# wischmcj/pyQSM

Measured on AMD Instinct MI355X. Metric: Mpoints/s DBSCAN (1M-pt synthetic forest, eps=0.1, min_neighbors=10), higher is better.
Workload: dtype f64; 1 GPU; 1000000-point synthetic tree cloud (configs[1]), DBSCAN eps=0.1 min_neighbors=10, 20 clusters; replicas at N>1; points_per_gpu=1000000, parallelism=replicas x1

## Files before the change

include/pyqsm_hip.h:

```cpp
#ifndef PYQSM_HIP_H
#define PYQSM_HIP_H

#include <stddef.h>
#include <stdint.h>

#ifdef __cplusplus
extern "C" {
#endif

#define PYQSM_OK 0
#define PYQSM_EINVAL (-1)
#define PYQSM_EHIP (-2)
#define PYQSM_ENODEV (-3)
#define PYQSM_ERANGE (-4)
#define PYQSM_ENOMEM (-5)
#define PYQSM_ENOCONV (-6)

#define PYQSM_MISS_PRIM 0xFFFFFFFFu


int pyqsm_device_count(void);
int pyqsm_init(int device);
int pyqsm_shutdown(void);
const char* pyqsm_last_error(void);
const char* pyqsm_version(void);
int pyqsm_sync(int device);
void* pyqsm_stream(int device);

int pyqsm_dev_malloc(int device, size_t bytes, void** out);
int pyqsm_dev_free(int device, void* p);
int pyqsm_h2d(int device, void* dst_dev, const void* src_host, size_t bytes);
int pyqsm_d2h(int device, void* dst_host, const void* src_dev, size_t bytes);
void pyqsm_free(void* p);
void* pyqsm_host_alloc(size_t bytes);

int pyqsm_prof_enable(int device, int on);
int pyqsm_prof_reset(int device);
int pyqsm_prof_get(int device, const char* name, double* total_ms, int64_t* launches);

int pyqsm_cast_rays(const float* verts, int64_t V, const int32_t* tris, int64_t T,
                    const float* rays, int64_t R,
                    float* t_hit, uint32_t* prim_id, float* uv, int32_t device);

int pyqsm_expand_tris_dev(const float* verts_dev, int64_t V, const int32_t* tris_dev,
                          int64_t T, float* tri12_dev, int32_t device);
int pyqsm_cast_rays_dev(const float* tri12_dev, int64_t T, const float* rays_dev, int64_t R,
                        float* t_hit_dev, uint32_t* prim_id_dev, float* uv_dev,
                        int32_t device);

int pyqsm_list_intersections(const float* verts, int64_t V, const int32_t* tris, int64_t T,
                             const float* rays, int64_t R, int32_t* counts,
                             uint32_t* ray_ids, uint32_t* prim_ids, float* t, float* uv,
                             int64_t hits_cap, int64_t* n_hits, int32_t device);

int pyqsm_point_mesh_distance(const float* verts, int64_t V, const int32_t* tris, int64_t T,
                              const float* qry, int64_t Q, float* dist, uint32_t* prim,
                              int32_t device);

int pyqsm_cast_rays_multi(const float* verts, int64_t V, const int32_t* tris, int64_t T,
                          const float* rays, int64_t R,
                          float* t_hit, uint32_t* prim_id, float* uv, int32_t n_devices);

int pyqsm_shard_bounds(int64_t n, int32_t world, int32_t rank, int64_t* begin, int64_t* end);

#define PYQSM_COMM_ID_BYTES 128
int pyqsm_comm_unique_id(uint8_t* id);
int pyqsm_comm_init_rank(const uint8_t* id, int32_t world, int32_t rank, int32_t device);
int pyqsm_comm_finalize(void);
int pyqsm_comm_info(int32_t* world, int32_t* rank, int32_t* device);
int pyqsm_comm_broadcast_dev(void* buf_dev, int64_t bytes, int32_t root);
int pyqsm_comm_all_gather_dev(const void* send_dev, void* recv_dev, int64_t bytes_per_rank);
int pyqsm_comm_all_reduce_max(double* value);

int pyqsm_dbscan(const double* xyz, int64_t n, double eps, int32_t min_pts,
                 int64_t* labels, uint8_t* is_core, int32_t device);
int pyqsm_dbscan_dev(const double* xyz_dev, int64_t n, double eps, int32_t min_pts,
                     int64_t* labels_dev, uint8_t* is_core_dev, int64_t* n_clusters,
                     int32_t device);
int pyqsm_dbscan_ex(const double* xyz, int64_t n, double eps, int32_t min_pts,
                    int32_t radius_inclusive, int64_t* labels, uint8_t* is_core, int32_t device);
int pyqsm_dbscan_dev_ex(const double* xyz_dev, int64_t n, double eps, int32_t min_pts,
                        int32_t radius_inclusive, int64_t* labels_dev, uint8_t* is_core_dev,
                        int64_t* n_clusters, int32_t device);
int pyqsm_octant_directory(const double* xyz, int64_t n, double eps, int32_t* dims_out,
                           int32_t* begin_out, int64_t cap, int32_t device);

int pyqsm_knn(const double* xyz, int64_t n, int32_t k, int32_t exclude_self,
              int32_t* idx, double* d2, int32_t device);
int pyqsm_knn_dev(const double* xyz_dev, int64_t n, int32_t k, int32_t exclude_self,
                  int32_t* idx_dev, double* d2_dev, int32_t device);

int pyqsm_ransac(const double* pts, int64_t n, const int64_t* triples, int64_t H,
                 int32_t shape, double thresh, double center[3], double axis[3],
                 double* radius, int64_t* inliers, int64_t* n_inliers, int64_t* best,
                 int32_t device);
int pyqsm_ransac_models(const double* pts, int64_t n, const int64_t* triples, int64_t H,
                        double* models, int32_t device);
int pyqsm_ransac_count(const double* pts, int64_t n, const double* models, int64_t H,
                       int32_t shape, double thresh, int32_t* counts, int32_t device);
int pyqsm_ransac_batch(const double* pts, int64_t n, const int64_t* seg_start, int64_t n_seg,
                       const int64_t* triples, int64_t H, int32_t shape, double thresh,
                       double* centers, double* axes, double* radii, int64_t* inliers,
                       int64_t* n_inliers, int64_t* best, int32_t device);

int pyqsm_plane_models(const double* pts, int64_t n, const int64_t* samples, int64_t H, int32_t m,
                       const double* axis, double cos_limit, double* planes, int32_t device);
int pyqsm_plane_count(const double* pts, int64_t n, const double* planes, int64_t H, double thresh,
                      int32_t* counts, int32_t device);
int pyqsm_segment_plane(const double* pts, int64_t n, const int64_t* samples, int64_t H, int32_t m,
                        double thresh, double probability, const double* axis, double cos_limit,
                        double plane_fit[4], double plane_hyp[4], int64_t* inliers, int64_t* n_inliers,
                        int64_t* best, int64_t* used, int32_t device);
int pyqsm_segment_planes(const double* pts, int64_t n, const uint64_t* draws, int64_t P, int64_t H,
                         int32_t m, double thresh, double probability, int64_t min_inliers,
                         const double* axis, double cos_limit, int32_t* labels, double* planes_fit,
                         double* planes_hyp, int64_t* counts, int64_t* best, int64_t* used,
                         int64_t* n_planes, int32_t device);

int pyqsm_lbc_solve(const int32_t* indptr, const int32_t* indices, const double* vals,
                    int64_t n, const double* wl, const double* wh, const double* pts,
                    double rtol, int32_t max_it, double* out, int32_t* iters,
                    double* resid, int32_t device);
int pyqsm_spmv3(const int32_t* indptr, const int32_t* indices, const double* vals,
                int64_t n, const double* x, double* y, int32_t device);
int pyqsm_clamp(double* pts, int64_t n, const double lo[3], const double hi[3],
                int32_t device);

int pyqsm_ball_query(const double* xyz, int64_t n, const double center[3], double radius,
                     int64_t* out_idx, int64_t* count, int32_t device);
int pyqsm_radius_mark(const double* src, int64_t n, const double* qry, int64_t m, double radius,
                      int32_t k_cap, uint8_t* mark, int32_t* counts, int32_t device);
int pyqsm_radius_knn(const double* src, int64_t n, const double* qry, int64_t m, double radius,
                     int32_t k, int64_t* idx, double* dist, int32_t device);
int pyqsm_radius_reduce(const double* src, int64_t n, const double* qry, int64_t m, double radius, int32_t k,
                        const double* values, int32_t F, int32_t reducer, int64_t empty_row, double* out,
                        int32_t* counts, int32_t device);
int pyqsm_radius_label(const double* src, int64_t n, const double* qry, int64_t m,
                       const int32_t* qry_label, double radius, int32_t k_cap, int32_t* label,
                       int32_t* counts, int32_t device);
int pyqsm_grow_clusters(const double* src, int64_t n, const int32_t* owner_in, const double* seed_xyz,
                        const int32_t* seed_label, int64_t m, int32_t n_clusters, double radius,
                        int32_t k_cap, int32_t cycles, int32_t min_new, int32_t* owner_out,
                        int32_t* cycle_out, int32_t* finished, int64_t* stats, int32_t device);

#define PYQSM_ADJ_SAME_CLOUD 1
#define PYQSM_ADJ_WITNESS 2
#define PYQSM_ADJ_NO_CACHE 4
int pyqsm_cluster_adjacency(const double* src, const int32_t* src_label, int64_t n, int32_t n_src_labels,
                            const double* tgt, const int32_t* tgt_label, int64_t m, int32_t n_tgt_labels,
                            double threshold, int32_t flags, int64_t capacity, int32_t* a, int32_t* b,
                            double* min_d2, int64_t* pairs, int64_t* src_idx, int64_t* tgt_idx, int64_t* count,
                            int64_t* stats, int32_t device);

#define PYQSM_ALPHA_BOUNDARY 1
#define PYQSM_ALPHA_DEFAULT_MAX_TESTS 4000000000000LL
int pyqsm_alpha_area(const int32_t* ij, int64_t n, const int64_t* seg_start, int64_t n_seg, uint64_t a2,
                     int64_t max_tests, int32_t flags, int64_t* twice_area, int64_t* n_live, int64_t* n_boundary,
                     int64_t** edges, int64_t* stats, int32_t device);

#define PYQSM_MESH_PAIRS 1
#define PYQSM_MESH_TILE_ROWS 256
#define PYQSM_MESH_DEFAULT_MAX_TESTS 16000000000000LL
int pyqsm_mesh_topology(const int32_t* tris, int64_t n_tris, int64_t n_verts, const double* verts, int32_t** edges,
                        int32_t** edge_count, uint8_t** edge_flags, int32_t* tri_cluster, int64_t** cluster_n,
                        double** cluster_area, uint8_t* vertex_flags, int64_t* summary, int32_t device);
int pyqsm_mesh_self_intersections(const int32_t* ijk, int64_t n_verts, const int32_t* tris, int64_t n_tris,
                                  int32_t flags, int64_t max_tests, int64_t* n_pairs, int32_t** pairs,
                                  uint8_t* tri_hit, int64_t* stats, int32_t device);

#define PYQSM_RECON_MAX_RHO2 4194304ULL
#define PYQSM_RECON_CHUNK 1024
#define PYQSM_RECON_SLICE 16
#define PYQSM_RECON_DEFAULT_MAX_TESTS 1000000000000LL
int pyqsm_ball_pivot(const int32_t* ijk, const int16_t* normals, int64_t n, const uint64_t* rho2, int32_t n_levels,
                     int64_t max_tests, int64_t* n_tris, int32_t** tris, int64_t* stats, int32_t device);

int pyqsm_fps(const double* xyz, int64_t n, int64_t num_samples, int64_t start_index,
              int32_t* out_idx, int32_t device);

int pyqsm_pc_laplacian(const double* xyz, int64_t n, int32_t k, double moll,
                       int64_t* nnz, int32_t** indptr, int32_t** indices, double** vals,
                       double* mass, int32_t device);
int pyqsm_pc_laplacian_seg(const double* xyz, int64_t n, const int64_t* seg_start, int64_t n_seg,
                           int32_t k, double moll, int64_t* nnz, int32_t** indptr,
                           int32_t** indices, double** vals, double* mass, int32_t device);

int pyqsm_extract_skeleton(const double* xyz, int64_t n, const int64_t* seg_start, int64_t n_seg,
                           int32_t k, double moll, int32_t max_iter, double termination_ratio,
                           double contraction_factor, double attraction_factor,
                           double max_contraction, double max_attraction, const double* lo,
                           const double* hi, double rtol, int32_t solver_max_it, double* out_pts,
                           double* total_shift, double* steps, int32_t* n_steps,
                           int32_t* solve_iters, double* solve_resid, uint8_t* solve_ok,
                           int32_t* n_solves, int32_t device);

int pyqsm_extreme_points(const double* xyz, int64_t n, const double* dirs, int32_t n_dirs,
                         int64_t* idx, int32_t device);
int pyqsm_outside_halfspaces(const double* xyz, int64_t n, const double* eq, int32_t n_planes,
                             double margin, int64_t* idx, int64_t* count, int32_t device);

int pyqsm_mean_f64(const double* v, int64_t n, double* out);

int pyqsm_voxel_down_sample(const double* xyz, int64_t n, const double* colors, double voxel_size,
                            int64_t* m, double** out_xyz, double** out_colors, int64_t* inverse,
                            int64_t* offsets, int64_t* members, int32_t device);
int pyqsm_stat_outlier(const double* xyz, int64_t n, int32_t nb_neighbors, double std_ratio,
                       int64_t* keep, int64_t* n_keep, double* avg, double* stats, int32_t device);
int pyqsm_clean_cloud(const double* xyz, int64_t n, double voxel_size, double neighbors, double ratio,
                      int32_t iters, int64_t* m, double** out_xyz, int32_t device);

int pyqsm_estimate_normals(const double* xyz, int64_t n, double radius, int32_t max_nn,
                           const double* prev_normals, double* normals, int32_t device);
int pyqsm_orient_normals_tangent_plane(const double* xyz, int64_t n, const double* normals, int32_t k,
                                       double* oriented, int32_t* rounds, int32_t device);
int pyqsm_stem_cloud(const double* xyz, int64_t n, const double* prev_normals, double crop_offset,
                     double radius, int32_t max_nn, int32_t orient_k, double angle_cutoff,
                     int64_t* keep, double* normals, int64_t* m, int32_t device);

#define PYQSM_KMEANS_MAX_K 8
#define PYQSM_KMEANS_MAX_Q 4
#define PYQSM_SILHOUETTE_MAX_K 65536
int pyqsm_kmeans(const double* xyz, int64_t m, int32_t k, int32_t iters, const double* init,
                 double* centroids, int32_t* labels, int32_t device);
int pyqsm_silhouette(const double* xyz, int64_t m, const int32_t* labels, int32_t k, double* score,
                     int32_t* n_present, double* samples, int32_t device);
int pyqsm_kmeans_select(const double* xyz, int64_t m, int32_t k0, int32_t nk, int32_t iters,
                        const double* init, int32_t* labels, double* scores, int32_t* present,
                        int32_t device);
int pyqsm_kmeans_select_dev(const double* xyz_dev, int64_t m, int32_t k0, int32_t nk, int32_t iters,
                            const double* init, int32_t* labels, double* scores, int32_t* present,
                            int32_t device);
int pyqsm_ball_excl_dev(const double* xyz_dev, int64_t n, const uint8_t* found_dev, const double center[3],
                        double radius, int64_t* idx_dev, double* out_xyz_dev, int64_t* count,
                        int32_t device);
int pyqsm_mark_found_dev(uint8_t* found_dev, int64_t n, const int64_t* idx, int64_t cnt, int32_t device);

int pyqsm_geometric_features(const double* xyz, int64_t n, double radius, int32_t max_k, int32_t metric,
                             const int32_t* feature_ids, int32_t n_features, double* out, int32_t* counts,
// ... 54 lines not shown
```

pyqsm_amd/_lib.py:

```python
from __future__ import annotations

import ctypes
import os

_HERE = os.path.dirname(os.path.abspath(__file__))
LIB_PATH = os.path.join(_HERE, "libpyqsm_hip.so")

i64, i32, u32, dbl = ctypes.c_int64, ctypes.c_int32, ctypes.c_uint32, ctypes.c_double
vp = ctypes.c_void_p

SIGNATURES = {
    "pyqsm_device_count": (ctypes.c_int, []),
    "pyqsm_init": (ctypes.c_int, [ctypes.c_int]),
    "pyqsm_shutdown": (ctypes.c_int, []),
    "pyqsm_last_error": (ctypes.c_char_p, []),
    "pyqsm_version": (ctypes.c_char_p, []),
    "pyqsm_sync": (ctypes.c_int, [ctypes.c_int]),
    "pyqsm_stream": (vp, [ctypes.c_int]),
    "pyqsm_dev_malloc": (ctypes.c_int, [ctypes.c_int, ctypes.c_size_t, ctypes.POINTER(vp)]),
    "pyqsm_dev_free": (ctypes.c_int, [ctypes.c_int, vp]),
    "pyqsm_h2d": (ctypes.c_int, [ctypes.c_int, vp, vp, ctypes.c_size_t]),
    "pyqsm_d2h": (ctypes.c_int, [ctypes.c_int, vp, vp, ctypes.c_size_t]),
    "pyqsm_free": (None, [vp]),
    "pyqsm_host_alloc": (vp, [ctypes.c_size_t]),
    "pyqsm_prof_enable": (ctypes.c_int, [ctypes.c_int, ctypes.c_int]),
    "pyqsm_prof_reset": (ctypes.c_int, [ctypes.c_int]),
    "pyqsm_prof_get": (ctypes.c_int, [ctypes.c_int, ctypes.c_char_p, ctypes.POINTER(dbl),
                                      ctypes.POINTER(i64)]),
    "pyqsm_cast_rays": (ctypes.c_int, [vp, i64, vp, i64, vp, i64, vp, vp, vp, i32]),
    "pyqsm_expand_tris_dev": (ctypes.c_int, [vp, i64, vp, i64, vp, i32]),
    "pyqsm_cast_rays_dev": (ctypes.c_int, [vp, i64, vp, i64, vp, vp, vp, i32]),
    "pyqsm_list_intersections": (ctypes.c_int, [vp, i64, vp, i64, vp, i64, vp, vp, vp, vp, vp,
                                                i64, ctypes.POINTER(i64), i32]),
    "pyqsm_point_mesh_distance": (ctypes.c_int, [vp, i64, vp, i64, vp, i64, vp, vp, i32]),
    "pyqsm_cast_rays_multi": (ctypes.c_int, [vp, i64, vp, i64, vp, i64, vp, vp, vp, i32]),
    "pyqsm_shard_bounds": (ctypes.c_int, [i64, i32, i32, ctypes.POINTER(i64), ctypes.POINTER(i64)]),
    "pyqsm_comm_unique_id": (ctypes.c_int, [vp]),
    "pyqsm_comm_init_rank": (ctypes.c_int, [vp, i32, i32, i32]),
    "pyqsm_comm_finalize": (ctypes.c_int, []),
    "pyqsm_comm_info": (ctypes.c_int, [ctypes.POINTER(i32), ctypes.POINTER(i32),
                                       ctypes.POINTER(i32)]),
    "pyqsm_comm_broadcast_dev": (ctypes.c_int, [vp, i64, i32]),
    "pyqsm_comm_all_gather_dev": (ctypes.c_int, [vp, vp, i64]),
    "pyqsm_comm_all_reduce_max": (ctypes.c_int, [ctypes.POINTER(dbl)]),
    "pyqsm_dbscan": (ctypes.c_int, [vp, i64, dbl, i32, vp, vp, i32]),
    "pyqsm_dbscan_dev": (ctypes.c_int, [vp, i64, dbl, i32, vp, vp, ctypes.POINTER(i64), i32]),
    "pyqsm_dbscan_ex": (ctypes.c_int, [vp, i64, dbl, i32, i32, vp, vp, i32]),
    "pyqsm_dbscan_dev_ex": (ctypes.c_int, [vp, i64, dbl, i32, i32, vp, vp, ctypes.POINTER(i64), i32]),
    "pyqsm_octant_directory": (ctypes.c_int, [vp, i64, dbl, vp, vp, i64, i32]),
    "pyqsm_knn": (ctypes.c_int, [vp, i64, i32, i32, vp, vp, i32]),
    "pyqsm_knn_dev": (ctypes.c_int, [vp, i64, i32, i32, vp, vp, i32]),
    "pyqsm_ransac": (ctypes.c_int, [vp, i64, vp, i64, i32, dbl, vp, vp, ctypes.POINTER(dbl), vp,
                                    ctypes.POINTER(i64), ctypes.POINTER(i64), i32]),
    "pyqsm_ransac_models": (ctypes.c_int, [vp, i64, vp, i64, vp, i32]),
    "pyqsm_ransac_count": (ctypes.c_int, [vp, i64, vp, i64, i32, dbl, vp, i32]),
    "pyqsm_ransac_batch": (ctypes.c_int, [vp, i64, vp, i64, vp, i64, i32, dbl, vp, vp, vp, vp, vp, vp, i32]),
    "pyqsm_plane_models": (ctypes.c_int, [vp, i64, vp, i64, i32, vp, dbl, vp, i32]),
    "pyqsm_plane_count": (ctypes.c_int, [vp, i64, vp, i64, dbl, vp, i32]),
    "pyqsm_segment_plane": (ctypes.c_int, [vp, i64, vp, i64, i32, dbl, dbl, vp, dbl, vp, vp, vp,
                                           ctypes.POINTER(i64), ctypes.POINTER(i64), ctypes.POINTER(i64), i32]),
    "pyqsm_segment_planes": (ctypes.c_int, [vp, i64, vp, i64, i64, i32, dbl, dbl, i64, vp, dbl, vp, vp, vp, vp,
                                            vp, vp, ctypes.POINTER(i64), i32]),
    "pyqsm_lbc_solve": (ctypes.c_int, [vp, vp, vp, i64, vp, vp, vp, dbl, i32, vp,
                                       ctypes.POINTER(i32), vp, i32]),
    "pyqsm_spmv3": (ctypes.c_int, [vp, vp, vp, i64, vp, vp, i32]),
    "pyqsm_clamp": (ctypes.c_int, [vp, i64, vp, vp, i32]),
    "pyqsm_ball_query": (ctypes.c_int, [vp, i64, vp, dbl, vp, ctypes.POINTER(i64), i32]),
    "pyqsm_radius_mark": (ctypes.c_int, [vp, i64, vp, i64, dbl, i32, vp, vp, i32]),
    "pyqsm_radius_label": (ctypes.c_int, [vp, i64, vp, i64, vp, dbl, i32, vp, vp, i32]),
    "pyqsm_grow_clusters": (ctypes.c_int, [vp, i64, vp, vp, vp, i64, i32, dbl, i32, i32, i32, vp, vp, vp, vp,
                                           i32]),
    "pyqsm_radius_knn": (ctypes.c_int, [vp, i64, vp, i64, dbl, i32, vp, vp, i32]),
    "pyqsm_cluster_adjacency": (ctypes.c_int, [vp, vp, i64, i32, vp, vp, i64, i32, dbl, i32, i64, vp, vp, vp, vp,
                                               vp, vp, ctypes.POINTER(i64), vp, i32]),
    "pyqsm_alpha_area": (ctypes.c_int, [vp, i64, vp, i64, ctypes.c_uint64, i64, i32, vp, vp, vp,
                                        ctypes.POINTER(vp), vp, i32]),
    "pyqsm_pdist_select": (ctypes.c_int, [vp, i64, i32, vp, i64, vp, i32, i64, vp, vp, vp, vp, i32]),
    "pyqsm_mesh_topology": (ctypes.c_int, [vp, i64, i64, vp, ctypes.POINTER(vp), ctypes.POINTER(vp),
                                           ctypes.POINTER(vp), vp, ctypes.POINTER(vp), ctypes.POINTER(vp), vp, vp,
                                           i32]),
    "pyqsm_mesh_self_intersections": (ctypes.c_int, [vp, i64, vp, i64, i32, i64, ctypes.POINTER(i64),
                                                     ctypes.POINTER(vp), vp, vp, i32]),
    "pyqsm_ball_pivot": (ctypes.c_int, [vp, vp, i64, vp, i32, i64, ctypes.POINTER(i64), ctypes.POINTER(vp), vp,
                                        i32]),
    "pyqsm_fps": (ctypes.c_int, [vp, i64, i64, i64, vp, i32]),
    "pyqsm_pc_laplacian": (ctypes.c_int, [vp, i64, i32, dbl, ctypes.POINTER(i64),
                                          ctypes.POINTER(vp), ctypes.POINTER(vp),
                                          ctypes.POINTER(vp), vp, i32]),
    "pyqsm_extract_skeleton": (ctypes.c_int, [vp, i64, vp, i64, i32, dbl, i32, dbl, dbl, dbl, dbl, dbl, vp, vp,
                                              dbl, i32, vp, vp, vp, vp, vp, vp, vp, ctypes.POINTER(i32), i32]),
    "pyqsm_pc_laplacian_seg": (ctypes.c_int, [vp, i64, vp, i64, i32, dbl, ctypes.POINTER(i64),
                                              ctypes.POINTER(vp), ctypes.POINTER(vp),
                                              ctypes.POINTER(vp), vp, i32]),
    "pyqsm_voxel_down_sample": (ctypes.c_int, [vp, i64, vp, dbl, ctypes.POINTER(i64), ctypes.POINTER(vp),
                                               ctypes.POINTER(vp), vp, vp, vp, i32]),
    "pyqsm_stat_outlier": (ctypes.c_int, [vp, i64, i32, dbl, vp, ctypes.POINTER(i64), vp, vp, i32]),
    "pyqsm_clean_cloud": (ctypes.c_int, [vp, i64, dbl, dbl, dbl, i32, ctypes.POINTER(i64),
                                         ctypes.POINTER(vp), i32]),
    "pyqsm_estimate_normals": (ctypes.c_int, [vp, i64, dbl, i32, vp, vp, i32]),
    "pyqsm_orient_normals_tangent_plane": (ctypes.c_int, [vp, i64, vp, i32, vp, ctypes.POINTER(i32), i32]),
    "pyqsm_stem_cloud": (ctypes.c_int, [vp, i64, vp, dbl, dbl, i32, i32, dbl, vp, vp, ctypes.POINTER(i64),
                                        i32]),
    "pyqsm_mean_f64": (ctypes.c_int, [vp, i64, ctypes.POINTER(dbl)]),
    "pyqsm_extreme_points": (ctypes.c_int, [vp, i64, vp, i32, vp, i32]),
    "pyqsm_outside_halfspaces": (ctypes.c_int, [vp, i64, vp, i32, dbl, vp, ctypes.POINTER(i64), i32]),
    "pyqsm_kmeans": (ctypes.c_int, [vp, i64, i32, i32, vp, vp, vp, i32]),
    "pyqsm_silhouette": (ctypes.c_int, [vp, i64, vp, i32, ctypes.POINTER(dbl), ctypes.POINTER(i32), vp, i32]),
    "pyqsm_kmeans_select": (ctypes.c_int, [vp, i64, i32, i32, i32, vp, vp, vp, vp, i32]),
    "pyqsm_kmeans_select_dev": (ctypes.c_int, [vp, i64, i32, i32, i32, vp, vp, vp, vp, i32]),
    "pyqsm_ball_excl_dev": (ctypes.c_int, [vp, i64, vp, vp, dbl, vp, vp, ctypes.POINTER(i64), i32]),
    "pyqsm_mark_found_dev": (ctypes.c_int, [vp, i64, vp, i64, i32]),
    "pyqsm_geometric_features": (ctypes.c_int, [vp, i64, dbl, i32, i32, vp, i32, vp, vp, i32]),
    "pyqsm_smooth_values": (ctypes.c_int, [vp, i64, vp, i64, vp, i32, i32, i32, vp, vp, i32]),
    "pyqsm_forest_create": (ctypes.c_int, [vp, vp, vp, vp, vp, vp, vp, i32, i32, i32, i32, ctypes.POINTER(vp)]),
    "pyqsm_forest_free": (ctypes.c_int, [vp]),
    "pyqsm_forest_info": (ctypes.c_int, [vp, vp]),
    "pyqsm_forest_stage": (ctypes.c_int, [vp, i32]),
    "pyqsm_forest_predict": (ctypes.c_int, [vp, vp, i64, vp, vp, vp]),
    "pyqsm_radius_reduce": (ctypes.c_int, [vp, i64, vp, i64, dbl, i32, vp, i32, i32, i64, vp, vp, i32]),
    "pyqsm_voxel_grid_create": (ctypes.c_int, [vp, i64, vp, dbl, i32, ctypes.POINTER(vp)]),
    "pyqsm_voxel_grid_free": (ctypes.c_int, [vp]),
    "pyqsm_voxel_grid_info": (ctypes.c_int, [vp, vp, ctypes.POINTER(dbl), vp, ctypes.POINTER(i64),
                                             ctypes.POINTER(i64)]),
    "pyqsm_voxel_grid_voxels": (ctypes.c_int, [vp, vp, vp]),
    "pyqsm_voxel_grid_query": (ctypes.c_int, [vp, vp, i64, i32, vp, vp, vp, ctypes.POINTER(i64)]),
    "pyqsm_voxel_grid_query_dev": (ctypes.c_int, [vp, vp, i64, i32, vp, vp, vp, ctypes.POINTER(i64)]),
    "pyqsm_skeletal_forest": (ctypes.c_int, [vp, i64, i32, vp, vp, ctypes.POINTER(i64), ctypes.POINTER(i32), i32]),
    "pyqsm_skeletal_forest_dev": (ctypes.c_int, [vp, i64, i32, vp, vp, ctypes.POINTER(i64), ctypes.POINTER(i32),
                                                 i32]),
    "pyqsm_collapse_chains": (ctypes.c_int, [vp, i64, i64, vp, vp, vp, vp, vp, i32]),
    "pyqsm_collapse_chains_dev": (ctypes.c_int, [vp, i64, i64, vp, vp, vp, vp, vp, i32]),
    "pyqsm_chain_radii": (ctypes.c_int, [vp, i64, vp, i64, vp, vp, i64, vp, i32]),
    "pyqsm_cylinder_surfaces": (ctypes.c_int, [vp, i64, vp, vp, ctypes.POINTER(vp), ctypes.POINTER(i64), i32]),
}

_lib = None


class PyQSMHipError(RuntimeError):

    def __init__(self, code: int, message: str):
        super().__init__(f"libpyqsm_hip error {code}: {message}")
        self.code = code


def load() -> ctypes.CDLL:
    global _lib
    if _lib is not None:
        return _lib
    if not os.path.exists(LIB_PATH):
        raise ImportError(
            f"{LIB_PATH} not found: the HIP library has not been built and there is no CPU "
            "fallback. Build it with `make -C pyqsm_amd/csrc`.")
    lib = ctypes.CDLL(LIB_PATH)
    for name, (res, args) in SIGNATURES.items():
        fn = getattr(lib, name)
        fn.restype = res
        fn.argtypes = args
    _lib = lib
    return lib


def check(code: int) -> None:
    if code != 0:
        msg = load().pyqsm_last_error()
        raise PyQSMHipError(code, msg.decode("utf-8", "replace") if msg else "")


def device_count() -> int:
    return int(load().pyqsm_device_count())


def logical_device_count() -> int:
    fake = os.environ.get("PYQSM_MULTI_FAKE_RANKS", "")
    return int(fake) if fake.isdigit() and int(fake) > 0 else device_count()


def physical_device(logical: int) -> int:
    fake = os.environ.get("PYQSM_MULTI_FAKE_RANKS", "")
    if fake.isdigit() and int(fake) > 0:
        return int(logical) % max(1, device_count())
    return int(logical)


def require_gpu(device: int = 0) -> None:
    check(load().pyqsm_init(int(device)))
```

pyqsm_amd/csrc/dbscan.hip:

```cpp
#include "grid.hpp"

#include <atomic>
#include <cfloat>
#include <chrono>
#include <cmath>
#include <optional>
#include <type_traits>
#include <vector>

namespace pyqsm {

static constexpr int kNoRoot = 0x7FFFFFFF;

__device__ __forceinline__ double sqdist(double ax, double ay, double az, double bx, double by,
                                         double bz) {
  double t0 = ax - bx, t1 = ay - by, t2 = az - bz;
  double d = t0 * t0;
  d = d + t1 * t1;
  d = d + t2 * t2;
  return d;
}


#define FOR_STENCIL(c, st, dir, q, body)                           \
  for (int dz__ = -1; dz__ <= 1; ++dz__)                           \
    for (int dy__ = -1; dy__ <= 1; ++dy__) {                       \
      const int row__ = (c) + dy__ * (st).nx + dz__ * (st).nxy;    \
      const int qb__ = (dir).begin(row__ - 1), qe__ = (dir).begin(row__ + 2); \
      for (int q = qb__; q < qe__; ++q) {                          \
        body                                                       \
      }                                                            \
    }

struct TileLds {
  double x[4][64], y[4][64], z[4][64];
};
struct TileLdsF32 {
  alignas(16) float x[4][64], y[4][64], z[4][64];
};
typedef float float2v __attribute__((ext_vector_type(2)));

struct CoreBand {
  float lo, hi;
  bool usable() const { return lo > 0x1p-100f && std::isfinite(hi); }
};
static CoreBand core_band(double r2) {
  const double a = r2 * (1.0 - 0x1p-20), b = r2 * (1.0 + 0x1p-20);
  CoreBand t{0.0f, INFINITY};
  if (!(a > 0.0) || !(b <= double(FLT_MAX))) return t;
  t.lo = float(a);
  if (double(t.lo) > a) t.lo = nextafterf(t.lo, -INFINITY);
  t.hi = float(b);
  if (double(t.hi) < b) t.hi = nextafterf(t.hi, INFINITY);
  return t;
}

static constexpr int kStragglers = 6;
static constexpr int kMaxChunks = 3;
static constexpr int kRestSegs = 64;
__device__ constexpr int kRunOrder[9] = {4, 3, 5, 1, 7, 0, 2, 6, 8};

__device__ __forceinline__ void stencil_bounds(int c, Stencil st, const CellDir& dir, int (&qb)[9], int (&qe)[9]) {
  int cells[18], q[18];
#pragma unroll
  for (int r = 0; r < 9; ++r) {
    const int row = c + (kRunOrder[r] % 3 - 1) * st.nx + (kRunOrder[r] / 3 - 1) * st.nxy;
    cells[2 * r] = row - 1;
    cells[2 * r + 1] = row + 2;
  }
  dir.begins(cells, q);
#pragma unroll
  for (int r = 0; r < 9; ++r) {
    qb[r] = q[2 * r];
    qe[r] = q[2 * r + 1];
  }
}

template <class CO, bool F32>
__global__ __launch_bounds__(256) void k_core_tiled(int n, const GridPlan* __restrict__ plan,
                                                    const DirWord* __restrict__ dwords,
                                                    const int32_t* __restrict__ dslots,
                                                    const int32_t* __restrict__ cell_of, CO co, double r2,
                                                    float r2_lo, float r2_hi ,
                                                    int min_pts, uint8_t* __restrict__ core,
                                                    int32_t* __restrict__ rest,
                                                    int32_t* __restrict__ rest_cnt , int seg_cap,
                                                    int* __restrict__ parent, int* __restrict__ min_orig,
                                                    uint32_t* __restrict__ bits ,
                                                    int32_t* __restrict__ seam , int seam_cap,
                                                    int max_chunks,
                                                    unsigned long long* __restrict__ tests ,
    unsigned long long* __restrict__ st ) {
  __shared__ TileLds L;
  __shared__ TileLdsF32 LF;
  stamped(st, [&] {
  const CellDir dir{dwords, dslots};
  const int lane = threadIdx.x & 63, w = __builtin_amdgcn_readfirstlane(threadIdx.x >> 6);
  const int p0 = (blockIdx.x * 4 + w) * 64;
  if (p0 >= n || !plan->ok) return;
  const Stencil st = plan_stencil(plan);
  const int ncell = plan->ncell;
  const int p = p0 + lane;
  const bool live = p < n;
  double x = 0.0, y = 0.0, z = 0.0;
  float fx = 0.0f, fy = 0.0f, fz = 0.0f;
  if constexpr (F32) {
    if (live) {
      const float4 v = co.p[p];
      fx = v.x, fy = v.y, fz = v.z;
    }
  } else {
    if (live) co.get(p, x, y, z);
  }
  const Tile t = wave_tile(p0, n, st, ncell, dir, cell_of);
  int cnt = 0;
  int cnt_hi = 0;
  bool deferred = false;
  int chunks = 0;
  int staged = 0;
  int band = 0;
  const auto hand_on = [&](unsigned long long und) {
    if (und != 0) {
      int slot = 0;
      const int lead = __ffsll(und) - 1;
      const int seg = blockIdx.x % kRestSegs;
      if (lane == lead) slot = atomicAdd(rest_cnt + seg, __popcll(und));
      slot = __shfl(slot, lead, 64);
      const bool mine = (und >> lane) & 1ull;
      if constexpr (F32) band += __popcll(__ballot(mine && cnt_hi > cnt));
      if (mine) {
        rest[size_t(seg) * seg_cap + slot + __popcll(und & ((1ull << lane) - 1ull))] = p;
        cnt = -1;
      }
    }
    deferred = true;
  };
  if (t.total > kTileMax) {
    if constexpr (F32) x = double(fx), y = double(fy), z = double(fz);
    const int mycell = live ? cell_of[p] : -1;
    unsigned long long todo = __ballot(live);
    while (todo) {
      const int lead = __ffsll(todo) - 1;
      const int c = __builtin_amdgcn_readlane(mycell, lead);
      const bool mine = mycell == c;
      todo &= ~__ballot(mine);
      int rqb[9], rqe[9];
      stencil_bounds(c, st, dir, rqb, rqe);
#pragma unroll
      for (int r = 0; r < 9; ++r) {
        const int qb = __builtin_amdgcn_readfirstlane(rqb[r]);
        const int qe = __builtin_amdgcn_readfirstlane(rqe[r]);
        for (int base = qb; base < qe; base += 64) {
          const int q = base + lane;
          const int m = qe - base < 64 ? qe - base : 64;
          if (q < qe) co.get(q, L.x[w][lane], L.y[w][lane], L.z[w][lane]);
          __builtin_amdgcn_wave_barrier();
          staged += m;
          if (mine)
            for (int j = 0; j < m; ++j)
              cnt += sqdist(x, y, z, L.x[w][j], L.y[w][j], L.z[w][j]) <= r2;
          __builtin_amdgcn_wave_barrier();
        }
      }
    }
  } else {
    const float2v X = {fx, fx}, Y = {fy, fy}, Z = {fz, fz};
#pragma unroll
    for (int ri = 0; ri < 9; ++ri) {
      const int r = kRunOrder[ri];
      for (int base = t.qb[r]; base < t.qe[r] && !deferred; base += 64) {
        const int q = base + lane;
        const int m = t.qe[r] - base < 64 ? t.qe[r] - base : 64;
        if constexpr (F32) {
          float4 v = make_float4(INFINITY, 0.0f, 0.0f, 0.0f);
          if (q < t.qe[r]) v = co.p[q];
          LF.x[w][lane] = v.x, LF.y[w][lane] = v.y, LF.z[w][lane] = v.z;
          __builtin_amdgcn_wave_barrier();
#pragma unroll 4
          for (int j = 0; j < m; j += 2) {
            const float2v dx = X - *reinterpret_cast<const float2v*>(&LF.x[w][j]);
            const float2v dy = Y - *reinterpret_cast<const float2v*>(&LF.y[w][j]);
            const float2v dz = Z - *reinterpret_cast<const float2v*>(&LF.z[w][j]);
            float2v d = dx * dx;
            d = __builtin_elementwise_fma(dy, dy, d);
            d = __builtin_elementwise_fma(dz, dz, d);
            cnt += d.x <= r2_lo;
            cnt += d.y <= r2_lo;
            cnt_hi += d.x <= r2_hi;
            cnt_hi += d.y <= r2_hi;
          }
        } else {
          if (q < t.qe[r]) co.get(q, L.x[w][lane], L.y[w][lane], L.z[w][lane]);
          __builtin_amdgcn_wave_barrier();
#pragma unroll 4
          for (int j = 0; j < m; ++j)
            cnt += sqdist(x, y, z, L.x[w][j], L.y[w][j], L.z[w][j]) <= r2;
        }
        staged += m;
        __builtin_amdgcn_wave_barrier();
        const unsigned long long und = __ballot(live && cnt < min_pts);
        ++chunks;
        if ((__popcll(und) <= kStragglers || chunks >= max_chunks) &&
            !(ri == 8 && base + 64 >= t.qe[r])) {
          hand_on(und);
          break;
        }
      }
    }
    if constexpr (F32) {
      if (!deferred) hand_on(__ballot(live && cnt < min_pts && cnt_hi >= min_pts));
    }
  }
  if (live && cnt >= 0) {
    core[p] = cnt >= min_pts;
    co.mark_core(p, cnt >= min_pts);
  }
  if (live) {
    parent[p] = p;
    min_orig[p] = 0x7F7F7F7F;
    if (p <= n / 32) bits[p] = 0u;
    if (p == 0) bits[n / 32 + 1] = 0u;
    for (int i = p; i < seam_cap; i += n) seam[i] = 0;
  }
  if (tests && lane == 0) {
    atomicAdd(tests + (blockIdx.x & 255), static_cast<unsigned long long>(staged));
    if (band) atomicAdd(tests + 256 + (blockIdx.x & 255), static_cast<unsigned long long>(band));
  }
  });
}

struct Runs9 {
  int qb[9];
  int pre[10];
  __device__ __forceinline__ int at(int g) const {
    int q = qb[0] + g;
#pragma unroll
    for (int r = 1; r < 9; ++r) q = g >= pre[r] ? qb[r] + (g - pre[r]) : q;
    return q;
  }
};
static constexpr int kRunBatch = 3;
__device__ __forceinline__ int lane_bound(bool act, int c, int j, Stencil st, const CellDir& dir) {
  const int r = int((0x862071534ull >> (4 * (j >> 1))) & 15ull);
  const int cell = c + (r % 3 - 1) * st.nx + (r / 3 - 1) * st.nxy + ((j & 1) ? 2 : -1);
  int b = 0;
  if (act) {
    const DirWord w = dir.words[cell >> 5];
    b = dir.slots[CellDir::slot_of(w, cell)];
  }
  return b;
}
__device__ __forceinline__ Runs9 runs_of_lanes(int bound, int k) {
  Runs9 t;
  t.pre[0] = 0;
#pragma unroll
  for (int r = 0; r < 9; ++r) {
    t.qb[r] = __builtin_amdgcn_readlane(bound, 18 * k + 2 * r);
    t.pre[r + 1] = t.pre[r] + (__builtin_amdgcn_readlane(bound, 18 * k + 2 * r + 1) - t.qb[r]);
  }
  return t;
}

template <class CO>
__global__ __launch_bounds__(256) void k_core_rest(const int32_t* __restrict__ rest,
                                                   const int32_t* __restrict__ rest_cnt ,
                                                   int seg_cap, const GridPlan* __restrict__ plan,
                                                   const DirWord* __restrict__ dwords,
                                                   const int32_t* __restrict__ dslots,
                                                   const int32_t* __restrict__ cell_of, CO co, double r2,
                                                   int min_pts, uint8_t* __restrict__ core,
    unsigned long long* __restrict__ st ) {
  stamped(st, [&] {
  const CellDir dir{dwords, dslots};
  if (!plan->ok) return;
  const Stencil st = plan_stencil(plan);
  const int lane = threadIdx.x & 63;
  const int mine = rest_cnt[lane];
  int incl = mine;
#pragma unroll
  for (int off = 1; off < 64; off <<= 1) {
    const int v = __shfl_up(incl, off, 64);
    if (lane >= off) incl += v;
  }
  const int m = __shfl(incl, 63, 64);
  const int grp = lane / 18, j = lane % 18;
  for (int i0 = (blockIdx.x * 4 + (threadIdx.x >> 6)) * kRunBatch; i0 < m; i0 += gridDim.x * 4 * kRunBatch) {
    int p = 0;
#pragma unroll
    for (int k = 0; k < kRunBatch; ++k) {
      if (i0 + k >= m) break;
      const int seg = __popcll(__ballot(incl <= i0 + k));
      const int before = __shfl(incl - mine, seg, 64);
      const int pk = rest[size_t(seg) * seg_cap + (i0 + k - before)];
      p = grp == k ? pk : p;
    }
    const bool act = grp < kRunBatch && i0 + grp < m;
    double x = 0.0, y = 0.0, z = 0.0;
    int c = 0;
    if (act) {
      co.get(p, x, y, z);
      c = cell_of[p];
    }
    const int bound = lane_bound(act, c, j, st, dir);
#pragma unroll
    for (int k = 0; k < kRunBatch; ++k) {
      if (i0 + k >= m) break;
      const Runs9 t = runs_of_lanes(bound, k);
      const int pk = __builtin_amdgcn_readlane(p, 18 * k);
      const double xk = __shfl(x, 18 * k, 64), yk = __shfl(y, 18 * k, 64), zk = __shfl(z, 18 * k, 64);
      int cnt = 0;
      for (int g0 = 0; g0 < t.pre[9] && cnt < min_pts; g0 += 64) {
        const int g = g0 + lane;
        const bool hit = g < t.pre[9] && co.d2(t.at(g), xk, yk, zk) <= r2;
        cnt += __popcll(__ballot(hit));
      }
      if (lane == 0) {
        core[pk] = cnt >= min_pts;
        co.mark_core(pk, cnt >= min_pts);
      }
    }
  }
  });
}


__device__ __forceinline__ int ld_parent(const int* parent, int i) {
  return __hip_atomic_load(parent + i, __ATOMIC_RELAXED, __HIP_MEMORY_SCOPE_AGENT);
}
__device__ __forceinline__ void st_parent(int* parent, int i, int v) {
  __hip_atomic_store(parent + i, v, __ATOMIC_RELAXED, __HIP_MEMORY_SCOPE_AGENT);
}

__device__ __forceinline__ unsigned link_prio(int x) { return unsigned(x) * 0x9E3779B1u; }

__device__ __forceinline__ int find_root(int* parent, int x) {
  int cur = ld_parent(parent, x);
  if (cur != x) {
    int prev = x, next;
    while (cur != (next = ld_parent(parent, cur))) {
      st_parent(parent, prev, next);
      prev = cur;
      cur = next;
    }
  }
  return cur;
}

__device__ __forceinline__ void unite(int* parent, int a, int b) {
  int ra = find_root(parent, a), rb = find_root(parent, b);
  while (ra != rb) {
    if (link_prio(ra) < link_prio(rb)) {
      int t = ra;
      ra = rb;
      rb = t;
    }
    const int old = atomicCAS(parent + ra, ra, rb);
    if (old == ra) break;
    ra = find_root(parent, old);
    rb = find_root(parent, rb);
  }
}


__global__ __launch_bounds__(1024) void k_sub_rep(int n, const int32_t* __restrict__ sub_of,
                                                 const uint8_t* __restrict__ core,
                                                 const int32_t* __restrict__ order,
                                                 int* __restrict__ parent,
                                                 const int32_t* __restrict__ cell_of,
// ... 627 lines not shown
        k = (static_cast<unsigned long long>(min_orig[r]) << 32) | static_cast<uint32_t>(r);
      }
      key[i] = k;
    }
    __syncthreads();
    for (int k = 2; k <= P; k <<= 1)
      for (int j = k >> 1; j > 0; j >>= 1) {
        for (int i = t; i < P; i += kNumberThreads) {
          const int l = i ^ j;
          if (l > i) {
            const unsigned long long a = key[i], b = key[l];
            if ((a > b) == ((i & k) == 0)) {
              key[i] = b;
              key[l] = a;
            }
          }
        }
        __syncthreads();
      }
    for (int i = t; i < R; i += kNumberThreads) min_orig[static_cast<uint32_t>(key[i])] = i;
    return;
  }
  for (int i = blockIdx.x * kNumberThreads + t; i < R; i += gridDim.x * kNumberThreads) {
    const int v = min_orig[roots[i]];
    __hip_atomic_fetch_or(bits + (v >> 5), 1u << (v & 31), __ATOMIC_RELAXED, __HIP_MEMORY_SCOPE_AGENT);
  }
  __shared__ int last;
  __threadfence();
  __syncthreads();
  if (t == 0) last = atomicAdd(done, 1) == int(gridDim.x) - 1;
  __syncthreads();
  if (!last) return;
  __threadfence();
  __shared__ int wsum[kNumberThreads / 64];
  const int lane = t & 63, wv = t >> 6;
  const int nw = n / 32 + 1;
  int carry = 0;
  for (int w0 = 0; w0 < nw; w0 += 16 * kNumberThreads) {
    const int i0 = w0 + 16 * t;
    int cnt[16], sum = 0;
#pragma unroll
    for (int k = 0; k < 16; ++k) {
      cnt[k] = i0 + k < nw ? __popc(__hip_atomic_load(bits + i0 + k, __ATOMIC_RELAXED, __HIP_MEMORY_SCOPE_AGENT)) : 0;
      sum += cnt[k];
    }
    int incl = sum;
#pragma unroll
    for (int off = 1; off < 64; off <<= 1) {
      const int o = __shfl_up(incl, off, 64);
      if (lane >= off) incl += o;
    }
    if (lane == 63) wsum[wv] = incl;
    __syncthreads();
    int before = carry, total = 0;
    for (int k = 0; k < kNumberThreads / 64; ++k) {
      before += k < wv ? wsum[k] : 0;
      total += wsum[k];
    }
    int run = before + incl - sum;
#pragma unroll
    for (int k = 0; k < 16; ++k)
      if (i0 + k < nw) {
        wpre[i0 + k] = run;
        run += cnt[k];
      }
    carry += total;
    __syncthreads();
  }
  });
}

__device__ __forceinline__ int cluster_number(int v, int n_roots, const uint32_t* __restrict__ bits,
                                              const int32_t* __restrict__ wpre) {
  if (n_roots <= kRankCap) return v;
  return wpre[v >> 5] + __popc(bits[v >> 5] & ((1u << (v & 31)) - 1u));
}

static constexpr int kLabelThreads = 256;
template <class CO>
__global__ __launch_bounds__(kLabelThreads) void k_labels(int n, const int32_t* __restrict__ rest,
                                                          const int32_t* __restrict__ rest_cnt,
                                                          const GridPlan* __restrict__ plan,
                                                          const DirWord* __restrict__ dwords,
                                                          const int32_t* __restrict__ dslots,
                                                          const int32_t* __restrict__ cell_of, CO co, double r2,
                                                          const uint8_t* __restrict__ core,
                                                          const int* __restrict__ parent,
                                                          const int* __restrict__ min_orig,
                                                          const int32_t* __restrict__ roots_cnt,
                                                          const uint32_t* __restrict__ bits,
                                                          const int32_t* __restrict__ wpre,
                                                          const int32_t* __restrict__ order,
                                                          int64_t* __restrict__ labels,
                                                          uint8_t* __restrict__ is_core,
    unsigned long long* __restrict__ st ) {
  stamped(st, [&] {
  const CellDir dir{dwords, dslots};
  if (!plan->ok) return;
  constexpr int kWaves = kLabelThreads / 64;
  const int n_roots = *roots_cnt;
  const int lane = threadIdx.x & 63;
  {
    const int p = blockIdx.x * kLabelThreads + threadIdx.x;
    const bool is_c = p < n && core[p];
    if (is_c) {
      const int v = min_orig[parent[parent[parent[p]]]];
      labels[order[p]] = int64_t(cluster_number(v, n_roots, bits, wpre));
    }
    if (p < n && is_core) is_core[order[p]] = is_c;
  }
  const int m = *rest_cnt;
  const Stencil sten = plan_stencil(plan);
  const int first = (blockIdx.x * kWaves + __builtin_amdgcn_readfirstlane(threadIdx.x >> 6)) * kRunBatch;
  const int grp = lane / 18, j = lane % 18;
  for (int i0 = first; i0 < m; i0 += gridDim.x * kWaves * kRunBatch) {
    const bool act = grp < kRunBatch && i0 + grp < m;
    double x = 0.0, y = 0.0, z = 0.0;
    int p = 0, c = 0;
    if (act) {
      p = rest[i0 + grp];
      co.get(p, x, y, z);
      c = cell_of[p];
    }
    const int bound = lane_bound(act, c, j, sten, dir);
#pragma unroll
    for (int k = 0; k < kRunBatch; ++k) {
      if (i0 + k >= m) break;
      const Runs9 t = runs_of_lanes(bound, k);
      const int pk = __builtin_amdgcn_readlane(p, 18 * k);
      const double xk = __shfl(x, 18 * k, 64), yk = __shfl(y, 18 * k, 64), zk = __shfl(z, 18 * k, 64);
      int best = kNoRoot;
      for (int g0 = 0; g0 < t.pre[9]; g0 += 64) {
        const int g = g0 + lane;
        if (g < t.pre[9]) {
          const int q = t.at(g);
          if (core[q] && co.d2(q, xk, yk, zk) <= r2) {
            const int mo = min_orig[parent[parent[parent[q]]]];
            best = mo < best ? mo : best;
          }
        }
      }
#pragma unroll
      for (int off = 32; off > 0; off >>= 1) {
        const int o = __shfl_xor(best, off, 64);
        best = o < best ? o : best;
      }
      if (lane == 0)
        labels[order[pk]] = best == kNoRoot ? int64_t(-1) : int64_t(cluster_number(best, n_roots, bits, wpre));
    }
  }
  });
}

static int cluster_binned(Ctx* c, int64_t n, double eps, int32_t min_pts, bool radius_inclusive, const DevGrid& g,
                          const SubCells& sub, const GridPlan* d_plan, int64_t* labels, uint8_t* is_core,
                          const int32_t** count_out) {
  const bool fine = g.cell <= eps * (1.0 + 1.0 / 524288.0);
  const int N = int(n);
  const dim3 grid(ceil_div(n, 256)), block(256);
  const Stencil st{g.nx, g.nx * g.ny};
  const CellDir dir = cell_dir(g);
  const double r2 = radius_inclusive ? eps * eps : nextafter(eps * eps, 0.0);
  uint8_t* core;
  int *parent, *min_orig;
  uint32_t* bits;
  PQ_TRY(c->arena.get(size_t(n), &core));
  PQ_TRY(c->arena.get(size_t(n), &parent));
  PQ_TRY(c->arena.get(size_t(n), &min_orig));
  PQ_TRY(c->arena.get(size_t(n / 32) + 2, &bits));
  int32_t* const pre_cnt = reinterpret_cast<int32_t*>(bits + n / 32 + 1);
  const size_t seam_cap = fine ? size_t(n) + size_t(g.start ? g.ncell >> 5 : g.ncell >> 12) + 3 : 0;
  int32_t *seam, *pre;
  PQ_TRY(c->arena.get(seam_cap, &seam));
  PQ_TRY(c->arena.get(size_t(n), &pre));
  if (fine && g.start) PQ_HIP(hipMemsetAsync(seam, 0, seam_cap * 4, c->stream));
  int32_t *roots, *wpre;
  PQ_TRY(c->arena.get(size_t(n), &roots));
  PQ_TRY(c->arena.get(size_t(n / 32) + 1, &wpre));
  int4* list;
  int32_t* list_cnt;
  int* run_min;
  PQ_TRY(c->arena.get(size_t(n), &run_min));
  PQ_TRY(c->arena.get(size_t(n), &list));
  int4* list_xyz;
  PQ_TRY(c->arena.get(size_t(n), &list_xyz));
  int32_t* link2;
  PQ_TRY(c->arena.get(size_t(n), &link2));
  list_cnt = sub.zeroed4;
  int32_t* const roots_cnt = list_cnt + 1;
  int32_t* rest;
  const int core_blocks = int(ceil_div(n, 256));
  const int seg_cap = ceil_div(core_blocks, kRestSegs) * 256;
  PQ_TRY(c->arena.get(std::max<size_t>(size_t(n), size_t(seg_cap) * kRestSegs), &rest));
  int32_t* const rest_segs = list_cnt + 4;
  {
    StampScope ps(c, "dbscan_core");
    unsigned long long* d_tests = nullptr;
    if (c->prof >= 2) {
      PQ_TRY(c->arena.get(512, &d_tests));
      PQ_HIP(hipMemsetAsync(d_tests, 0, 512 * 8, c->stream));
    }
    const int max_chunks = std::min(32, std::max(kMaxChunks, (kMaxChunks * min_pts + 9) / 10));
    {
      const StampKernel pk(c, "k_core_tiled", grid.x);
      const CoreBand cb = core_band(r2);
      const bool f32 = cb.usable();
      on_coords(g, [&](auto co) {
        const auto launch = [&](auto kernel) {
          hipLaunchKernelGGL(kernel, grid, block, 0, c->stream, N, d_plan, dir.words, dir.slots, g.cell_of, co, r2, cb.lo,
                             cb.hi, min_pts, core, rest, rest_segs, seg_cap, parent, min_orig, bits, seam,
                             g.start ? 0 : int(seam_cap), max_chunks, d_tests, pk.slots);
        };
        if constexpr (std::is_same_v<decltype(co), CoordsF32>) {
          if (f32) return launch(k_core_tiled<CoordsF32, true>);
        }
        launch(k_core_tiled<decltype(co), false>);
      });
    }
    if (d_tests) {
      unsigned long long h[512];
      PQ_TRY(fetch(c, h, d_tests, 512));
      unsigned long long tot = 0, band = 0;
      for (int i = 0; i < 256; ++i) tot += h[i], band += h[256 + i];
      c->timers["core_pair_tests"].launches += int64_t(tot) * 64;
      c->timers["core_band_lanes"].launches += int64_t(band);
    }
    const dim3 gr(std::min<int64_t>(8192, ceil_div(n, 64)));
    unsigned long long* const st_rest = stamp_slots(c, gr.x);
    on_coords(g, [&](auto co) {
      hipLaunchKernelGGL(k_core_rest<decltype(co)>, gr, block, 0, c->stream, rest, rest_segs, seg_cap, d_plan, dir.words, dir.slots,
                         g.cell_of, co, r2, min_pts, core, st_rest);
    });
    PQ_HIP(hipGetLastError());
    if (getenv("PYQSM_DBSCAN_TRACE")) {
      int32_t h[kRestSegs];
      PQ_TRY(fetch(c, h, rest_segs, kRestSegs));
      long long tot = 0;
      for (int32_t v : h) tot += v;
      fprintf(stderr, "core pass: %lld stragglers\n", tot);
    }
  }
  {
    StampScope ps(c, "dbscan_union");
    const dim3 gf(ceil_div(n, kFlagsPerBlock));
    if (fine) {
      hipLaunchKernelGGL(k_sub_rep, dim3(ceil_div(n, 1024)), dim3(1024), 0, c->stream, N, sub.sub_of, core,
                         g.order, parent, g.cell_of, sub.rec, run_min, list, list_cnt, d_plan, list_xyz, dir.words,
                         stamp_slots(c, ceil_div(n, 1024)));
      {
        static const bool use_link2 = [] {
          const char* e = getenv("PYQSM_DBSCAN_LINK2");
          return e ? atoi(e) != 0 : true;
        }();
        int per_cu[2] = {use_link2 ? 8 : 16, 32};
        if (const char* e_cu = getenv("PYQSM_UNION_BLOCKS_PER_CU")) {
          per_cu[0] = per_cu[1] = atoi(e_cu);
          if (const char* comma = strchr(e_cu, ',')) per_cu[1] = atoi(comma + 1);
        }
        const int64_t full = ceil_div(n, 4 * kSubPerWave), full_u = ceil_div(n, kSeamThreads);
        const int64_t cu_u = std::max(1, per_cu[1] * 256 / kSeamThreads);
        const dim3 gh(per_cu[0] > 0 ? std::min<int64_t>(full, int64_t(c->cu_count) * per_cu[0]) : full),
            gu(per_cu[1] > 0 ? std::min<int64_t>(full_u, int64_t(c->cu_count) * cu_u) : full_u);
        const bool trace = getenv("PYQSM_DBSCAN_TRACE") != nullptr;
        {
          const StampKernel pk(c, "k_hook_sub", gh.x);
          on_coords(g, [&](auto co) {
            if (use_link2)
              hipLaunchKernelGGL((k_hook_sub<decltype(co), true>), gh, block, 0, c->stream, list, list_xyz, list_cnt,
                                 d_plan, dir.words, dir.slots, sub.rec, co, r2, core, parent, link2, pk.slots);
            else
              hipLaunchKernelGGL((k_hook_sub<decltype(co), false>), gh, block, 0, c->stream, list, list_xyz, list_cnt,
                                 d_plan, dir.words, dir.slots, sub.rec, co, r2, core, parent, link2, pk.slots);
          });
        }
        int32_t tm = 0;
        std::vector<int32_t> hp, root_of;
        std::vector<int4> hl;
        const auto snapshot = [&](std::vector<int64_t>* hist) -> int {
          PQ_TRY(fetch(c, &tm, list_cnt));
          hp.assign(static_cast<size_t>(n), 0);
          hl.assign(static_cast<size_t>(tm), make_int4(0, 0, 0, 0));
          PQ_HIP(hipMemcpy(hp.data(), parent, size_t(n) * 4, hipMemcpyDeviceToHost));
          PQ_HIP(hipMemcpy(hl.data(), list, size_t(tm) * 16, hipMemcpyDeviceToHost));
          root_of.assign(static_cast<size_t>(n), -1);
          for (int32_t s2 = 0; s2 < tm; ++s2) {
            int d = 0, r = hl[size_t(s2)].x;
            while (hp[size_t(r)] != r) {
              r = hp[size_t(r)];
              ++d;
            }
            root_of[size_t(hl[size_t(s2)].x)] = r;
            if (hist) (*hist)[size_t(std::min(d, 65))]++;
          }
          return 0;
        };
        const auto count_roots = [&] {
          int64_t roots = 0;
          for (int32_t s2 = 0; s2 < tm; ++s2) roots += root_of[size_t(hl[size_t(s2)].x)] == hl[size_t(s2)].x;
          return roots;
        };
        int64_t links = 0, crossing = 0;
        if (trace) {
          std::vector<int64_t> hist(66, 0);
          PQ_TRY(snapshot(&hist));
          fprintf(stderr, "hook pass: %d sub-cells, %lld roots; chain depth histogram:", tm, (long long)count_roots());
          for (int d = 0; d < 66; ++d)
            if (hist[size_t(d)]) fprintf(stderr, " %d:%lld", d, (long long)hist[size_t(d)]);
          fprintf(stderr, "\n");
          if (use_link2) {
            std::vector<int32_t> h2(static_cast<size_t>(tm), -1);
            PQ_HIP(hipMemcpy(h2.data(), link2, size_t(tm) * 4, hipMemcpyDeviceToHost));
            for (int32_t s2 = 0; s2 < tm; ++s2) {
              if (h2[size_t(s2)] < 0) continue;
              ++links;
              crossing += root_of[size_t(h2[size_t(s2)])] != root_of[size_t(hl[size_t(s2)].x)];
            }
          }
        }
        static const int jump = [] {
          const char* e = getenv("PYQSM_FLATTEN_JUMP");
          return e ? atoi(e) : 12;
        }();
        const auto flatten = [&](auto mode, int max_steps, bool host_flags) {
          constexpr int threads = kFlagsThreads;
          const int rep_blocks = int(ceil_div(n, threads));
          hipLaunchKernelGGL(k_flatten_reps<decltype(mode)::value>, dim3(rep_blocks + (host_flags ? gf.x : 0)),
                             dim3(threads), 0, c->stream, list, list_cnt, parent, max_steps, link2, seam,
                             pre, pre_cnt, rep_blocks, N, core, rest, list_cnt + 3, d_plan);
        };
        if (jump > 0) flatten(std::integral_constant<FlattenMode, kFlattenJump>{}, jump, false);
        if (use_link2) {
          flatten(std::integral_constant<FlattenMode, kFlattenLink>{}, 0, true);
          if (trace) {
            PQ_TRY(snapshot(nullptr));
            fprintf(stderr, "link pass: %lld recorded, %lld crossed trees, %lld roots left\n", (long long)links,
                    (long long)crossing, (long long)count_roots());
          }
          flatten(std::integral_constant<FlattenMode, kFlattenWords>{}, 0, false);
        } else {
          flatten(std::integral_constant<FlattenMode, kFlattenRoots>{}, 0, true);
        }
        unsigned long long* d_seams = nullptr;
        if (trace) {
          PQ_TRY(c->arena.get(1, &d_seams));
          PQ_HIP(hipMemsetAsync(d_seams, 0, 8, c->stream));
        }
        {
          const int fold_blocks = int(ceil_div(n, kSeamThreads));
          const StampKernel pk(c, "k_union_sub", gu.x + fold_blocks);
          on_coords(g, [&](auto co) {
            hipLaunchKernelGGL(k_union_sub<decltype(co)>, dim3(gu.x + fold_blocks), dim3(kSeamThreads), 0, c->stream, list,
                               list_xyz, list_cnt, d_plan, dir.words, dir.slots, seam, sub.rec, co, r2, core, parent,
                               int(gu.x), run_min, min_orig, d_seams, pk.slots);
          });
        }
        if (trace) {
          unsigned long long h = 0;
          PQ_TRY(fetch(c, &h, d_seams));
          fprintf(stderr, "seam union: %llu sub-cells took the 62-offset path\n", h);
        }
        const dim3 gp(std::min<int64_t>(ceil_div(n, kFoldThreads), int64_t(c->cu_count) * 8));
        hipLaunchKernelGGL(k_fold_roots, gp, dim3(kFoldThreads), 0, c->stream, pre, pre_cnt, parent, min_orig, roots,
                           roots_cnt, d_plan);
      }
      PQ_HIP(hipGetLastError());
    } else {
      PQ_TRY(stamp_mark(c));
      on_coords(g, [&](auto co) {
        hipLaunchKernelGGL(k_union_points<decltype(co)>, grid, block, 0, c->stream, N, st, dir.words, dir.slots, g.cell_of, co,
                           r2, core, parent);
      });
      hipLaunchKernelGGL(k_flatten, grid, block, 0, c->stream, N, core, parent, d_plan);
      hipLaunchKernelGGL(k_point_min, grid, block, 0, c->stream, N, core, parent, g.order, min_orig, roots,
                         roots_cnt, d_plan);
      hipLaunchKernelGGL(k_noncore_list, gf, dim3(kFlagsThreads), 0, c->stream, N, core, rest,
                         list_cnt + 3, d_plan);
    }
    const dim3 gn(std::min<int64_t>(ceil_div(n, kNumberThreads), c->cu_count));
    hipLaunchKernelGGL(k_number, gn, dim3(kNumberThreads), 0, c->stream, N, roots, roots_cnt, min_orig, bits, wpre,
                       list_cnt + 2, d_plan, stamp_slots(c, gn.x));
    PQ_HIP(hipGetLastError());
  }
  {
    StampScope ps(c, "dbscan_label");
    const dim3 gb(ceil_div(n, kLabelThreads));
    unsigned long long* const st_labels = stamp_slots(c, gb.x);
    on_coords(g, [&](auto co) {
      hipLaunchKernelGGL(k_labels<decltype(co)>, gb, dim3(kLabelThreads), 0, c->stream, N, rest, list_cnt + 3, d_plan,
                         dir.words, dir.slots, g.cell_of, co, r2, core, parent, min_orig, roots_cnt, bits, wpre, g.order, labels,
                         is_core, st_labels);
    });
    PQ_HIP(hipGetLastError());
    if (getenv("PYQSM_DBSCAN_TRACE")) {
      int32_t h = 0;
      PQ_TRY(fetch(c, &h, list_cnt + 3));
      fprintf(stderr, "label pass: %d non-core points listed\n", h);
    }
  }
  *count_out = roots_cnt;
  return 0;
}


static constexpr double kPlanPollMs = 20.0;
static int wait_plan(Ctx* c, const GridPlan* h_plan, unsigned seq) {
  const volatile unsigned* const s = &h_plan->seq;
  const auto t0 = std::chrono::steady_clock::now();
  while (*s != seq) {
    if (std::chrono::duration<double, std::milli>(std::chrono::steady_clock::now() - t0).count() > kPlanPollMs) {
      PQ_HIP(hipStreamSynchronize(c->stream));
      if (*s != seq) return fail(PYQSM_EHIP, "DBSCAN: the grid plan was not written (sequence %u)", seq);
      break;
    }
  }
  std::atomic_thread_fence(std::memory_order_acquire);
  return 0;
}

struct DirReadout {
  int64_t cap;
  int32_t* begin_host;
  int32_t dims[3];
};
static int dbscan_device(Ctx* c, const double* xyz, int64_t n, double eps, int32_t min_pts,
                         bool radius_inclusive, int64_t* labels, uint8_t* is_core, int64_t* n_clusters,
                         DirReadout* readout = nullptr) {
  if (!(eps > 0) || !std::isfinite(eps)) return fail(PYQSM_EINVAL, "eps must be positive");
  if (n == 0) {
    if (n_clusters) *n_clusters = 0;
    return 0;
  }
  const double cell = eps * (1.0 + 1.0 / 1048576.0);
  const int64_t max_cells = int64_t(1) << 28;
  if (!c->plan_pinned) {
    PQ_HIP(hipHostMalloc(&c->plan_pinned, 2 * sizeof(GridPlan), hipHostMallocMapped | hipHostMallocCoherent));
    memset(c->plan_pinned, 0, 2 * sizeof(GridPlan));
  }
  GridPlan* const h_plan = static_cast<GridPlan*>(c->plan_pinned);
  GridPlan* h_plan_dev;
  PQ_HIP(hipHostGetDevicePointer(reinterpret_cast<void**>(&h_plan_dev), c->plan_pinned, 0));
  if (++c->plan_seq == 0) c->plan_seq = 1;
  const unsigned seq = c->plan_seq;
  GridPlan* d_plan;
  int32_t* zeroed;
  PQ_TRY(c->arena.get(2, &d_plan));
  PQ_TRY(c->arena.get(size_t(octant_zeroed_ints()), &zeroed));
  const char* plan_env = getenv("PYQSM_DBSCAN_PLAN");
  const char* bin_env = getenv("PYQSM_DBSCAN_BIN");
  const char* f32_env = getenv("PYQSM_COORD_F32");
  const bool speculate = c->plan_hint.valid && !(plan_env && !strcmp(plan_env, "host")) && !bin_env &&
                         !(f32_env && !strcmp(f32_env, "0")) && n <= (int64_t(1) << 25);
  const PlanHint hint = speculate ? c->plan_hint : PlanHint{};
  DevGrid g;
  SubCells sub;
  const int32_t* count = nullptr;
  std::optional<StampScope> bin_scope(std::in_place, c, "dbscan_bin");
  PQ_TRY(plan_grid_device(c, xyz, n, cell, max_cells, hint, d_plan, h_plan_dev, seq, zeroed, octant_zeroed_ints()));
  const Arena::Mark mark = c->arena.mark();
  if (speculate) {
    PQ_TRY(bin_octants_planned(c, xyz, n, cell, hint, d_plan, zeroed, &g, &sub));
    bin_scope.reset();
    if (!readout)
      PQ_TRY(cluster_binned(c, n, eps, min_pts, radius_inclusive, g, sub, d_plan, labels, is_core, &count));
  }
  PQ_TRY(wait_plan(c, h_plan, seq));
  const bool hit = speculate && h_plan[0].ok;
  if (!hit) {
    c->arena.rewind(mark);
    PlanHint next;
    if (!bin_scope) bin_scope.emplace(c, "dbscan_bin");
    PQ_TRY(stamp_mark(c));
    PQ_TRY(bin_octants_host(c, xyz, n, cell, max_cells, h_plan[0], zeroed, &h_plan[1], d_plan + 1, &g, &sub, &next));
    PQ_TRY(stamp_mark(c));
    bin_scope.reset();
    if (next.valid) c->plan_hint = next;
    if (!readout)
      PQ_TRY(cluster_binned(c, n, eps, min_pts, radius_inclusive, g, sub, d_plan + 1, labels, is_core, &count));
  }
  if (c->prof >= 1) {
    c->timers["dbscan_f32_records"].launches += g.p4 ? 1 : 0;
    c->timers[hit ? "dbscan_plan_hit" : "dbscan_plan_miss"].launches += 1;
  }
  if (readout) {
    const GridPlan& pl = hit ? h_plan[0] : h_plan[1];
    readout->dims[0] = pl.nx;
    readout->dims[1] = pl.ny;
    readout->dims[2] = pl.nz;
    const int64_t entries = int64_t(pl.ncell) + 1;
    if (entries > readout->cap)
      return fail(PYQSM_ERANGE, "octant directory: %lld entries, room for %lld", (long long)entries,
                  (long long)readout->cap);
    int32_t* d_begin;
    PQ_TRY(c->arena.get(size_t(entries), &d_begin));
    read_directory(c, g, pl.ncell, d_begin);
    PQ_HIP(hipGetLastError());
    PQ_TRY(fetch(c, readout->begin_host, d_begin, size_t(entries)));
    return 0;
  }
  if (n_clusters) {
    int32_t h = 0;
    PQ_TRY(fetch(c, &h, count));
    *n_clusters = h;
  }
  return 0;
}

}

using namespace pyqsm;

extern "C" {

int pyqsm_dbscan_dev_ex(const double* xyz_dev, int64_t n, double eps, int32_t min_pts,
                        int32_t radius_inclusive, int64_t* labels_dev, uint8_t* is_core_dev,
                        int64_t* n_clusters, int32_t device) {
  PQ_API_RANGE("pyqsm_dbscan_dev");
  if (n < 0) return fail(PYQSM_EINVAL, "negative size");
  if (n > 0 && (!xyz_dev || !labels_dev)) return fail(PYQSM_EINVAL, "pyqsm_dbscan_dev: NULL pointer");
  Call call(device);
  Ctx* c = call.c;
  if (!c) return PYQSM_ENODEV;
  StampScope ps(c, "dbscan_total");
  return dbscan_device(c, xyz_dev, n, eps, min_pts, radius_inclusive != 0, labels_dev, is_core_dev,
                       n_clusters);
}

int pyqsm_dbscan_dev(const double* xyz_dev, int64_t n, double eps, int32_t min_pts,
                     int64_t* labels_dev, uint8_t* is_core_dev, int64_t* n_clusters,
                     int32_t device) {
  return pyqsm_dbscan_dev_ex(xyz_dev, n, eps, min_pts, 1, labels_dev, is_core_dev, n_clusters, device);
}

int pyqsm_dbscan(const double* xyz, int64_t n, double eps, int32_t min_pts, int64_t* labels,
                 uint8_t* is_core, int32_t device) {
  return pyqsm_dbscan_ex(xyz, n, eps, min_pts, 1, labels, is_core, device);
}

int pyqsm_dbscan_ex(const double* xyz, int64_t n, double eps, int32_t min_pts, int32_t radius_inclusive,
                    int64_t* labels, uint8_t* is_core, int32_t device) {
  PQ_API_RANGE("pyqsm_dbscan");
  if (n < 0) return fail(PYQSM_EINVAL, "negative size");
  if (n == 0) return 0;
  if (!xyz || !labels) return fail(PYQSM_EINVAL, "pyqsm_dbscan: NULL pointer");
  Call call(device);
  Ctx* c = call.c;
  if (!c) return PYQSM_ENODEV;
  double* d_xyz;
  int64_t* d_lab;
  uint8_t* d_core;
  PQ_TRY(c->arena.get(size_t(n) * 3, &d_xyz));
  PQ_TRY(c->arena.get(size_t(n), &d_lab));
  PQ_TRY(c->arena.get(size_t(n), &d_core));
  PQ_TRY(copy_in(c, d_xyz, xyz, size_t(n) * 3));
  PQ_TRY(dbscan_device(c, d_xyz, n, eps, min_pts, radius_inclusive != 0, d_lab, d_core, nullptr));
  PQ_TRY(download(c, labels, d_lab, size_t(n)));
  if (is_core) PQ_TRY(download(c, is_core, d_core, size_t(n)));
  PQ_HIP(hipStreamSynchronize(c->stream));
  return 0;
}

int pyqsm_octant_directory(const double* xyz, int64_t n, double eps, int32_t* dims_out, int32_t* begin_out,
                           int64_t cap, int32_t device) {
  PQ_API_RANGE("pyqsm_octant_directory");
  if (n <= 0) return fail(PYQSM_EINVAL, "pyqsm_octant_directory: empty cloud");
  if (!xyz || !dims_out || !begin_out) return fail(PYQSM_EINVAL, "pyqsm_octant_directory: NULL pointer");
  Call call(device);
  Ctx* c = call.c;
  if (!c) return PYQSM_ENODEV;
  double* d_xyz;
  PQ_TRY(upload(c, xyz, size_t(n) * 3, &d_xyz));
  DirReadout ro{cap, begin_out, {0, 0, 0}};
  PQ_TRY(dbscan_device(c, d_xyz, n, eps, 1, true, nullptr, nullptr, nullptr, &ro));
  for (int a = 0; a < 3; ++a) dims_out[a] = ro.dims[a];
  return 0;
}

}
```

pyqsm_amd/csrc/grid.hip:

```cpp
#include "grid.hpp"

#include "block_scan.hpp"

#include <atomic>
#include <cmath>
#include <type_traits>

namespace pyqsm {

__device__ __forceinline__ unsigned long long ord_key(double x) {
  unsigned long long b = static_cast<unsigned long long>(__double_as_longlong(x));
  return (b >> 63) ? ~b : (b | 0x8000000000000000ull);
}
__host__ __device__ static inline double ord_val(unsigned long long k) {
  const unsigned long long b = (k >> 63) ? (k & 0x7FFFFFFFFFFFFFFFull) : ~k;
  double d;
  memcpy(&d, &b, 8);
  return d;
}

static constexpr int kBkMax = 16384;

struct BucketShape {
  int bits;
  int64_t nbk;
};
__host__ __device__ static inline BucketShape bucket_shape(int64_t ncell) {
  const int bits = ncell + 1 <= (int64_t(kBkMax) << 12) ? 12 : 13;
  return BucketShape{bits, (ncell + (int64_t(1) << bits)) >> bits};
}

__host__ __device__ static inline bool interior_slabs(const double* mn, const double* mx, double cell, double border,
                                                      int raw[3], double* tot) {
  bool ok = true;
  double t = 1.0;
  for (int a = 0; a < 3; ++a) {
    const double d = floor((mx[a] - mn[a]) / cell) + 1.0;
    if (!(d < 2.0e9)) ok = false;
    raw[a] = ok ? int(d) : 0;
    t *= d + border;
  }
  *tot = t;
  return ok;
}

static constexpr int kBoxVals = 7;
__global__ __launch_bounds__(256) void k_bbox(const double* __restrict__ xyz, int64_t n,
                                              unsigned long long* __restrict__ part ,
    unsigned long long* __restrict__ st ) {
  __shared__ unsigned long long red[4][6];
  __shared__ int red_f32[4];
  stamped(st, [&] {
  unsigned long long mn[3] = {~0ull, ~0ull, ~0ull}, mx[3] = {0, 0, 0};
  bool f32ok = true;
  for (int64_t i = blockIdx.x * int64_t(blockDim.x) + threadIdx.x; i < n;
       i += int64_t(gridDim.x) * blockDim.x) {
#pragma unroll
    for (int a = 0; a < 3; ++a) {
      const double v = xyz[3 * i + a];
      f32ok = f32ok && double(float(v)) == v;
      unsigned long long k = ord_key(v);
      mn[a] = k < mn[a] ? k : mn[a];
      mx[a] = k > mx[a] ? k : mx[a];
    }
  }
  const bool wave_ok = __all(f32ok);
#pragma unroll
  for (int a = 0; a < 3; ++a) {
#pragma unroll
    for (int off = 32; off > 0; off >>= 1) {
      unsigned long long o1 = __shfl_down(mn[a], off, 64), o2 = __shfl_down(mx[a], off, 64);
      mn[a] = o1 < mn[a] ? o1 : mn[a];
      mx[a] = o2 > mx[a] ? o2 : mx[a];
    }
  }
  const int w = threadIdx.x >> 6;
  if ((threadIdx.x & 63) == 0) {
#pragma unroll
    for (int a = 0; a < 3; ++a) {
      red[w][a] = mn[a];
      red[w][3 + a] = mx[a];
    }
    red_f32[w] = wave_ok;
  }
  __syncthreads();
  if (threadIdx.x < 6) {
    unsigned long long v = red[0][threadIdx.x];
    for (int q = 1; q < 4; ++q) {
      const unsigned long long o = red[q][threadIdx.x];
      v = threadIdx.x < 3 ? (o < v ? o : v) : (o > v ? o : v);
    }
    part[size_t(blockIdx.x) * kBoxVals + threadIdx.x] = v;
  }
  if (threadIdx.x == 6)
    part[size_t(blockIdx.x) * kBoxVals + 6] = (red_f32[0] && red_f32[1] && red_f32[2] && red_f32[3]) ? 1ull : 0ull;
  });
}

struct PlanIn {
  double cell;
  int64_t max_cells;
  PlanHint hint;
  GridPlan* host;
  unsigned seq;
};
__device__ void write_plan(const unsigned long long* box, const PlanIn& in, GridPlan* __restrict__ plan);

__global__ __launch_bounds__(256) void k_bbox_fold(const unsigned long long* __restrict__ part,
                                                   int nblk, unsigned long long* __restrict__ out,
                                                   int32_t* __restrict__ zero_buf, int zero_n,
                                                   PlanIn pin, GridPlan* __restrict__ plan) {
  __shared__ unsigned long long red[4][kBoxVals];
  __shared__ unsigned long long fin[kBoxVals];
  for (int q = threadIdx.x; q < zero_n; q += 256) zero_buf[q] = 0;
  unsigned long long v[kBoxVals] = {~0ull, ~0ull, ~0ull, 0, 0, 0, ~0ull};
  for (int b = threadIdx.x; b < nblk; b += 256)
#pragma unroll
    for (int a = 0; a < kBoxVals; ++a) {
      const unsigned long long o = part[size_t(b) * kBoxVals + a];
      v[a] = (a < 3 || a == 6) ? (o < v[a] ? o : v[a]) : (o > v[a] ? o : v[a]);
    }
#pragma unroll
  for (int a = 0; a < kBoxVals; ++a)
#pragma unroll
    for (int off = 32; off > 0; off >>= 1) {
      const unsigned long long o = __shfl_down(v[a], off, 64);
      v[a] = (a < 3 || a == 6) ? (o < v[a] ? o : v[a]) : (o > v[a] ? o : v[a]);
    }
  if ((threadIdx.x & 63) == 0)
#pragma unroll
    for (int a = 0; a < kBoxVals; ++a) red[threadIdx.x >> 6][a] = v[a];
  __syncthreads();
  if (threadIdx.x < kBoxVals) {
    const bool is_min = threadIdx.x < 3 || threadIdx.x == 6;
    unsigned long long r = red[0][threadIdx.x];
    for (int q = 1; q < 4; ++q) {
      const unsigned long long o = red[q][threadIdx.x];
      r = is_min ? (o < r ? o : r) : (o > r ? o : r);
    }
    out[threadIdx.x] = r;
    fin[threadIdx.x] = r;
  }
  if (plan) {
    __syncthreads();
    if (threadIdx.x == 0) write_plan(fin, pin, plan);
  }
}

__global__ __launch_bounds__(256) void k_cell_count(const double* __restrict__ xyz, int64_t n,
                                                    GridParams g, int32_t* __restrict__ counts,
                                                    int32_t* __restrict__ cell_tmp,
                                                    int32_t* __restrict__ rank_tmp,
                                                    int32_t* __restrict__ occ_part ) {
  __shared__ int wfirst[4];
  int64_t i = blockIdx.x * int64_t(blockDim.x) + threadIdx.x;
  bool first = false;
  if (i < n) {
    int c = cell_index(g, xyz[3 * i], xyz[3 * i + 1], xyz[3 * i + 2]);
    cell_tmp[i] = c;
    const int rank = atomicAdd(&counts[c], 1);
    rank_tmp[i] = rank;
    first = rank == 0;
  }
  const unsigned long long b = __ballot(first);
  if ((threadIdx.x & 63) == 0) wfirst[threadIdx.x >> 6] = __popcll(b);
  __syncthreads();
  if (threadIdx.x == 0) occ_part[blockIdx.x] = (wfirst[0] + wfirst[1]) + (wfirst[2] + wfirst[3]);
}

__global__ __launch_bounds__(256) void k_cell_scatter(const double* __restrict__ xyz, int64_t n,
                                                      const int32_t* __restrict__ start,
                                                      const int32_t* __restrict__ cell_tmp,
                                                      const int32_t* __restrict__ rank_tmp,
                                                      int32_t* __restrict__ order,
                                                      int32_t* __restrict__ cell_of,
                                                      double* __restrict__ sx,
                                                      double* __restrict__ sy,
                                                      double* __restrict__ sz) {
  const SortedStore out{order, cell_of, nullptr, nullptr, sx, sy, sz};
  int64_t i = blockIdx.x * int64_t(blockDim.x) + threadIdx.x;
  if (i >= n) return;
  int c = cell_tmp[i];
  out.put(start[c] + rank_tmp[i], int32_t(i), c, xyz[3 * i], xyz[3 * i + 1], xyz[3 * i + 2]);
}

__device__ __forceinline__ void block_add_i32(int32_t local, int32_t* out) {
  __shared__ int32_t wsum[4];
#pragma unroll
  for (int off = 32; off > 0; off >>= 1) local += __shfl_down(local, off, 64);
  if ((threadIdx.x & 63) == 0) wsum[threadIdx.x >> 6] = local;
  __syncthreads();
  if (threadIdx.x == 0) {
    const int32_t t = (wsum[0] + wsum[1]) + (wsum[2] + wsum[3]);
    if (t) atomicAdd(out, t);
  }
}

__global__ __launch_bounds__(256) void k_count_occupied(const int32_t* __restrict__ start,
                                                        int64_t ncell, int32_t* __restrict__ out) {
  int32_t local = 0;
  for (int64_t i = blockIdx.x * int64_t(blockDim.x) + threadIdx.x; i < ncell;
       i += int64_t(gridDim.x) * blockDim.x)
    local += start[i + 1] > start[i];
  block_add_i32(local, out);
}

__global__ __launch_bounds__(256) void k_probe_count(const double* __restrict__ xyz, int64_t n,
                                                     GridParams g, int32_t* __restrict__ counts) {
  int64_t i = blockIdx.x * int64_t(blockDim.x) + threadIdx.x;
  if (i >= n) return;
  counts[cell_index(g, xyz[3 * i], xyz[3 * i + 1], xyz[3 * i + 2])] = 1;
}

__global__ __launch_bounds__(256) void k_count_nonzero(const int32_t* __restrict__ counts,
                                                       int64_t ncell, int32_t* __restrict__ out) {
  int32_t local = 0;
  for (int64_t i = blockIdx.x * int64_t(blockDim.x) + threadIdx.x; i < ncell;
       i += int64_t(gridDim.x) * blockDim.x)
    local += counts[i] > 0;
  block_add_i32(local, out);
}

int probe_occupancy(Ctx* c, const double* xyz, int64_t n, const double box[6], double cell,
                    double* cell_used, double* per_cell) {
  int dims[3];
  for (;;) {
    double tot = 1.0;
    for (int a = 0; a < 3; ++a) {
      double d = std::floor((box[3 + a] - box[a]) / cell) + 3.0;
      dims[a] = d < 2.0e9 ? int(d) : 0x7FFFFFFF;
      tot *= d;
    }
    if (tot <= double(int64_t(1) << 22)) break;
    cell *= 2.0;
  }
  const int64_t ncell = int64_t(dims[0]) * dims[1] * dims[2];
  int32_t* counts;
  PQ_TRY(c->arena.get(size_t(ncell) + 1, &counts));
  PQ_HIP(hipMemsetAsync(counts, 0, (size_t(ncell) + 1) * 4, c->stream));
  GridParams gp{box[0], box[1], box[2], 1.0 / cell, dims[0], dims[1], dims[2]};
  hipLaunchKernelGGL(k_probe_count, dim3(ceil_div(n, 256)), dim3(256), 0, c->stream, xyz, n, gp,
                     counts);
  const int blocks = int(std::min<int64_t>(ceil_div(ncell, 256), int64_t(c->cu_count) * 8));
  hipLaunchKernelGGL(k_count_nonzero, dim3(blocks), dim3(256), 0, c->stream, counts, ncell,
                     counts + ncell);
  PQ_HIP(hipGetLastError());
  int32_t occ = 0;
  PQ_TRY(fetch(c, &occ, counts + ncell));
  *cell_used = cell;
  *per_cell = double(n) / double(occ > 0 ? occ : 1);
  return 0;
}


static constexpr int kAxisBins = 64;
static constexpr int kAxisBlocks = 512;
static constexpr int kAxisSample = 4;

__global__ __launch_bounds__(256) void k_axis_hist(const double* __restrict__ xyz, int64_t n, double mnx,
                                                   double mny, double mnz, double ix, double iy, double iz,
                                                   int32_t* __restrict__ part ) {
  __shared__ int32_t h[3 * kAxisBins];
  for (int t = threadIdx.x; t < 3 * kAxisBins; t += 256) h[t] = 0;
  __syncthreads();
  for (int64_t i = (blockIdx.x * 256ll + threadIdx.x) * kAxisSample; i < n;
       i += int64_t(gridDim.x) * 256 * kAxisSample) {
    const double bx = floor((xyz[3 * i] - mnx) * ix), by = floor((xyz[3 * i + 1] - mny) * iy),
                 bz = floor((xyz[3 * i + 2] - mnz) * iz);
    atomicAdd(&h[int(fmin(fmax(bx, 0.0), double(kAxisBins - 1)))], kAxisSample);
    atomicAdd(&h[kAxisBins + int(fmin(fmax(by, 0.0), double(kAxisBins - 1)))], kAxisSample);
    atomicAdd(&h[2 * kAxisBins + int(fmin(fmax(bz, 0.0), double(kAxisBins - 1)))], kAxisSample);
  }
  __syncthreads();
  for (int t = threadIdx.x; t < 3 * kAxisBins; t += 256) part[size_t(blockIdx.x) * 3 * kAxisBins + t] = h[t];
}

__global__ __launch_bounds__(64) void k_axis_fold(const int32_t* __restrict__ part, int nblk,
                                                  int32_t* __restrict__ out) {
  const int t = blockIdx.x;
  int32_t s = 0;
  for (int b = threadIdx.x; b < nblk; b += 64) s += part[size_t(b) * 3 * kAxisBins + t];
#pragma unroll
  for (int off = 32; off > 0; off >>= 1) s += __shfl_down(s, off, 64);
  if (threadIdx.x == 0) out[t] = s;
}

int robust_box(Ctx* c, const double* xyz, int64_t n, int budget, double box[6], int64_t* outside) {
  *outside = 0;
  if (budget <= 0 || n < 64) return 0;
  const int blocks = int(std::min<int64_t>(ceil_div(n, 256 * kAxisSample), kAxisBlocks));
  int32_t *d_part = nullptr, *d_hist = nullptr;
  PQ_TRY(c->arena.get(size_t(blocks) * 3 * kAxisBins, &d_part));
  PQ_TRY(c->arena.get(size_t(3 * kAxisBins), &d_hist));
  const int side = budget / 3;
  int64_t lost_axis[3] = {0, 0, 0};
  for (int round = 0; round < 6; ++round) {
    double inv[3];
    for (int a = 0; a < 3; ++a) {
      const double e = box[3 + a] - box[a];
      inv[a] = e > 0 ? double(kAxisBins) / e : 0.0;
    }
    hipLaunchKernelGGL(k_axis_hist, dim3(blocks), dim3(256), 0, c->stream, xyz, n, box[0], box[1], box[2],
                       inv[0], inv[1], inv[2], d_part);
    hipLaunchKernelGGL(k_axis_fold, dim3(3 * kAxisBins), dim3(64), 0, c->stream, d_part, blocks, d_hist);
    PQ_HIP(hipGetLastError());
    int32_t h[3 * kAxisBins];
    PQ_TRY(fetch(c, h, d_hist, 3 * kAxisBins));
    bool cut = false;
    for (int a = 0; a < 3; ++a) {
      const int32_t* ha = h + a * kAxisBins;
      int lo = 0, hi = kAxisBins - 1;
      int64_t acc = 0;
      while (lo < hi && acc + ha[lo] <= side) acc += ha[lo++];
      int64_t lost_a = acc;
      acc = 0;
      while (hi > lo && acc + ha[hi] <= side) acc += ha[hi--];
      lost_a += acc;
      if (hi - lo + 1 > (3 * kAxisBins) / 4 || !(inv[a] > 0)) continue;
      const double w = (box[3 + a] - box[a]) / double(kAxisBins);
      const double mn = box[a];
      box[a] = mn + w * double(lo);
      box[3 + a] = mn + w * double(hi + 1);
      lost_axis[a] = lost_a;
      cut = true;
    }
    if (!cut) break;
    *outside = (lost_axis[0] + lost_axis[1]) + lost_axis[2];
  }
  return 0;
}

int cloud_bbox(Ctx* c, const double* xyz, int64_t n, double mn[3], double mx[3], bool* all_f32,
               int32_t* zero_buf, int zero_n) {
  if (n <= 0) return fail(PYQSM_EINVAL, "bounding box of an empty cloud");
  const int blocks = int(std::min<int64_t>(ceil_div(n, 256), int64_t(c->cu_count) * 4));
  unsigned long long *d_box = nullptr, *d_part = nullptr;
  PQ_TRY(c->arena.get(kBoxVals, &d_box));
  PQ_TRY(c->arena.get(size_t(blocks) * kBoxVals, &d_part));
  hipLaunchKernelGGL(k_bbox, dim3(blocks), dim3(256), 0, c->stream, xyz, n, d_part,
                     static_cast<unsigned long long*>(nullptr));
  hipLaunchKernelGGL(k_bbox_fold, dim3(1), dim3(256), 0, c->stream, d_part, blocks, d_box, zero_buf, zero_n, PlanIn{},
                     static_cast<GridPlan*>(nullptr));
  PQ_HIP(hipGetLastError());
  unsigned long long h_box[kBoxVals];
  PQ_TRY(fetch(c, h_box, d_box, kBoxVals));
  if (all_f32) *all_f32 = h_box[6] != 0;
  for (int a = 0; a < 3; ++a) {
    mn[a] = ord_val(h_box[a]);
    mx[a] = ord_val(h_box[3 + a]);
    if (!std::isfinite(mn[a]) || !std::isfinite(mx[a]))
      return fail(PYQSM_EINVAL, "point coordinates must be finite");
  }
  return 0;
}

static int build_grid_bucketed(Ctx* c, const double* xyz, int64_t n, DevGrid* g);
static bool bucketed_fits(const DevGrid& g);

int build_grid(Ctx* c, const double* xyz, int64_t n, double min_cell, int64_t max_cells,
               DevGrid* g, const double* bbox, bool f32_records) {
  if (n <= 0) return fail(PYQSM_EINVAL, "build_grid: empty cloud");
  if (n > 0x7FFFFF00LL) return fail(PYQSM_ERANGE, "more than 2^31 points per call");
  if (!(min_cell > 0) || !std::isfinite(min_cell))
    return fail(PYQSM_EINVAL, "cell edge must be positive and finite");
  double mn[3], mx[3];
  if (bbox) {
    for (int a = 0; a < 3; ++a) {
      mn[a] = bbox[a];
      mx[a] = bbox[3 + a];
    }
  } else {
    PQ_TRY(cloud_bbox(c, xyz, n, mn, mx));
  }
  double cell = min_cell;
  int dims[3];
  for (;;) {
    double tot;
    const bool ok = interior_slabs(mn, mx, cell, 2.0, dims, &tot);
    if (ok && tot <= double(max_cells)) break;
    cell *= 2.0;
  }
  for (int a = 0; a < 3; ++a) dims[a] += 2;
  g->minx = mn[0];
  g->miny = mn[1];
  g->minz = mn[2];
  g->cell = cell;
  g->inv_cell = 1.0 / cell;
  g->nx = dims[0];
  g->ny = dims[1];
  g->nz = dims[2];
  g->ncell = int64_t(dims[0]) * dims[1] * dims[2];
  int32_t *cell_tmp, *rank_tmp;
  PQ_TRY(c->arena.get(size_t(g->ncell) + 1, &g->start));
  PQ_TRY(c->arena.get(size_t(n), &g->order));
  PQ_TRY(c->arena.get(size_t(n), &g->cell_of));
  const bool bucketed = bucketed_fits(*g);
  g->p4 = nullptr;
  g->sx = g->sy = g->sz = nullptr;
  {
    const char* f32_env = getenv("PYQSM_COORD_F32");
    if (f32_env && !strcmp(f32_env, "0")) f32_records = false;
  }
  if (bucketed && f32_records) {
    PQ_TRY(c->arena.get(size_t(n), &g->p4));
  } else {
    PQ_TRY(c->arena.get(size_t(n), &g->sx));
    PQ_TRY(c->arena.get(size_t(n), &g->sy));
    PQ_TRY(c->arena.get(size_t(n), &g->sz));
  }
  if (bucketed) return build_grid_bucketed(c, xyz, n, g);
  PQ_TRY(c->arena.get(size_t(n), &cell_tmp));
  PQ_TRY(c->arena.get(size_t(n), &rank_tmp));
  PQ_HIP(hipMemsetAsync(g->start, 0, (size_t(g->ncell) + 1) * 4, c->stream));
  const GridParams gp = grid_params(*g);
  const dim3 grid(ceil_div(n, 256));
  g->occ_blocks = int(grid.x);
  PQ_TRY(c->arena.get(size_t(g->occ_blocks), &g->occ_part));
  hipLaunchKernelGGL(k_cell_count, grid, dim3(256), 0, c->stream, xyz, n, gp, g->start, cell_tmp,
                     rank_tmp, g->occ_part);
  PQ_HIP(hipGetLastError());
  PQ_TRY(exclusive_scan_i32(c, g->start, g->ncell + 1));
  hipLaunchKernelGGL(k_cell_scatter, grid, dim3(256), 0, c->stream, xyz, n, g->start, cell_tmp,
                     rank_tmp, g->order, g->cell_of, g->sx, g->sy, g->sz);
  PQ_HIP(hipGetLastError());
  return 0;
}



struct AxisMap {
  const int32_t *x, *y, *z;
};

struct RawCell {
  int cx, cy, cz, oct;
};

__device__ __forceinline__ RawCell raw_cell(const GridParams& g, int rx, int ry, int rz, double x,
                                            double y, double z) {
  int hx = int(floor((x - g.minx) * (2.0 * g.inv_cell)));
  int hy = int(floor((y - g.miny) * (2.0 * g.inv_cell)));
  int hz = int(floor((z - g.minz) * (2.0 * g.inv_cell)));
  int cx = int(floor((x - g.minx) * g.inv_cell));
  int cy = int(floor((y - g.miny) * g.inv_cell));
  int cz = int(floor((z - g.minz) * g.inv_cell));
  cx = cx < 0 ? 0 : (cx > rx - 1 ? rx - 1 : cx);
  cy = cy < 0 ? 0 : (cy > ry - 1 ? ry - 1 : cy);
  cz = cz < 0 ? 0 : (cz > rz - 1 ? rz - 1 : cz);
  const int ox = hx - 2 * cx < 1 ? 0 : 1, oy = hy - 2 * cy < 1 ? 0 : 1, oz = hz - 2 * cz < 1 ? 0 : 1;
  return RawCell{cx, cy, cz, ox | (oy << 1) | (oz << 2)};
}

__global__ __launch_bounds__(256) void k_axis_occ(const double* __restrict__ xyz, int64_t n,
                                                  GridParams g, int rx, int ry, int rz,
                                                  int32_t* __restrict__ ox, int32_t* __restrict__ oy,
                                                  int32_t* __restrict__ oz) {
  int64_t i = blockIdx.x * int64_t(blockDim.x) + threadIdx.x;
  if (i >= n) return;
  const RawCell r = raw_cell(g, rx, ry, rz, xyz[3 * i], xyz[3 * i + 1], xyz[3 * i + 2]);
  ox[r.cx] = 1;
  oy[r.cy] = 1;
  oz[r.cz] = 1;
}

__global__ __launch_bounds__(256) void k_axis_keep(int m, const int32_t* __restrict__ occ,
                                                   int32_t* __restrict__ keep ) {
  int i = blockIdx.x * 256 + threadIdx.x;
  if (i > m) return;
  keep[i] = i < m ? ((occ[i] || (i > 0 && occ[i - 1])) ? 1 : 0) : 0;
}

__global__ __launch_bounds__(256) void k_axis_shift(int m, int32_t* __restrict__ map) {
  int i = blockIdx.x * 256 + threadIdx.x;
  if (i < m) map[i] += 1;
}

template <bool MAPPED>
__global__ __launch_bounds__(256) void k_cell_count_oct(const double* __restrict__ xyz, int64_t n,
                                                        GridParams g, int rx, int ry, int rz, AxisMap am,
                                                        int32_t* __restrict__ counts,
                                                        int32_t* __restrict__ cell_tmp,
                                                        int32_t* __restrict__ rank_tmp) {
  int64_t i = blockIdx.x * int64_t(blockDim.x) + threadIdx.x;
  if (i >= n) return;
  const RawCell r = raw_cell(g, rx, ry, rz, xyz[3 * i], xyz[3 * i + 1], xyz[3 * i + 2]);
  const int cx = MAPPED ? am.x[r.cx] : r.cx + 1, cy = MAPPED ? am.y[r.cy] : r.cy + 1,
            cz = MAPPED ? am.z[r.cz] : r.cz + 1;
  const int c = (cz * g.ny + cy) * g.nx + cx;
  cell_tmp[i] = c;
  rank_tmp[i] = (atomicAdd(&counts[c], 1) << 3) | r.oct;
}

struct alignas(32) PointRec {
  double x, y, z;
  int32_t idx, key;
};

__global__ __launch_bounds__(256) void k_scatter_keys(const double* __restrict__ xyz, int64_t n,
                                                      const int32_t* __restrict__ start,
                                                      const int32_t* __restrict__ cell_tmp,
                                                      const int32_t* __restrict__ rank_tmp,
                                                      PointRec* __restrict__ keyed) {
  int64_t i = blockIdx.x * int64_t(blockDim.x) + threadIdx.x;
  if (i >= n) return;
  const int c = cell_tmp[i], ro = rank_tmp[i];
  PointRec r;
  r.x = xyz[3 * i];
  r.y = xyz[3 * i + 1];
  r.z = xyz[3 * i + 2];
  r.idx = int(i);
  r.key = (c << 3) | (ro & 7);
  keyed[start[c] + (ro >> 3)] = r;
}

static constexpr int kBigCell = 128;

__global__ __launch_bounds__(256) void k_order_cells(int n, const int32_t* __restrict__ start,
                                                     const PointRec* __restrict__ keyed,
                                                     int32_t* __restrict__ order,
                                                     int32_t* __restrict__ cell_of,
                                                     int32_t* __restrict__ sub_of,
                                                     double* __restrict__ sx, double* __restrict__ sy,
                                                     double* __restrict__ sz,
                                                     int4* __restrict__ rec,
                                                     int32_t* __restrict__ big_list,
                                                     int32_t* __restrict__ big_cnt) {
  const SortedStore out{order, cell_of, sub_of, nullptr, sx, sy, sz};
  const int p = blockIdx.x * 256 + threadIdx.x;
  if (p >= n) return;
  const PointRec me = keyed[p];
  const int c = me.key >> 3, o = me.key & 7;
  const int b = start[c], e = start[c + 1];
  if (e - b > kBigCell) {
    if (p == b) big_list[atomicAdd(big_cnt, 1)] = c;
    return;
  }
  int less = 0, same_before = 0;
  int cnt[8] = {0, 0, 0, 0, 0, 0, 0, 0};
  const bool first = p == b;
  for (int q = b; q < e; ++q) {
    const int oq = keyed[q].key & 7;
    less += oq < o;
    same_before += (oq == o) & (q < p);
    if (first) {
#pragma unroll
      for (int k = 0; k < 8; ++k) cnt[k] += oq == k;
    }
  }
  out.put(b + less + same_before, me.idx, c, me.x, me.y, me.z, b * 8 + o);
  if (first) write_sub_records(rec, b, cnt);
}

template <int W>
__device__ __forceinline__ void order_run_by_octant(const PointRec* __restrict__ keyed, int b, int e, int32_t (&tot)[8],
                                                    int32_t (&base)[8], int32_t (&wcnt)[W / 64][8],
                                                    const SortedStore& out, int4* __restrict__ rec) {
  const int t = threadIdx.x, lane = t & 63, w = t >> 6;
  int loc[8] = {0, 0, 0, 0, 0, 0, 0, 0};
  for (int q = b + t; q < e; q += W) {
    const int oq = keyed[q].key & 7;
#pragma unroll
    for (int k = 0; k < 8; ++k) loc[k] += oq == k;
  }
  if (t < 8) tot[t] = 0;
  __syncthreads();
#pragma unroll
  for (int k = 0; k < 8; ++k) {
    int cnt = loc[k];
    for (int off = 32; off > 0; off >>= 1) cnt += __shfl_down(cnt, off, 64);
    if (lane == 0 && cnt) atomicAdd(&tot[k], cnt);
  }
  __syncthreads();
  if (t == 0) {
    int r2 = b;
    for (int k = 0; k < 8; ++k) {
      base[k] = r2;
      r2 += tot[k];
    }
    write_sub_records(rec, b, tot);
  }
  __syncthreads();
  for (int q0 = b; q0 < e; q0 += W) {
    const int q = q0 + t;
    const bool live = q < e;
    PointRec pr;
    pr.key = 0;
    if (live) pr = keyed[q];
    const int o = pr.key & 7;
    int before = 0;
#pragma unroll
    for (int k = 0; k < 8; ++k) {
      const unsigned long long m = __ballot(live && o == k);
      if (lane == 0) wcnt[w][k] = __popcll(m);
      if (o == k) before = __popcll(m & ((1ull << lane) - 1ull));
    }
    __syncthreads();
    if (live) {
      int f = base[o] + before;
      for (int ww = 0; ww < w; ++ww) f += wcnt[ww][o];
      out.put(f, pr.idx, pr.key >> 3, pr.x, pr.y, pr.z, b * 8 + o);
    }
    __syncthreads();
    if (t < 8) {
      int add = 0;
      for (int ww = 0; ww < W / 64; ++ww) add += wcnt[ww][t];
      base[t] += add;
    }
    __syncthreads();
  }
}

__global__ __launch_bounds__(256) void k_order_big(const int32_t* __restrict__ big_list,
                                                   const int32_t* __restrict__ big_cnt,
                                                   const int32_t* __restrict__ start,
                                                   const PointRec* __restrict__ keyed,
                                                   int32_t* __restrict__ order,
                                                   int32_t* __restrict__ cell_of,
                                                   int32_t* __restrict__ sub_of,
                                                   double* __restrict__ sx, double* __restrict__ sy,
                                                   double* __restrict__ sz, float4* __restrict__ p4,
                                                   int4* __restrict__ rec, const GridPlan* __restrict__ plan) {
  __shared__ int32_t tot[8], base[8], wcnt[4][8];
  const SortedStore out{order, cell_of, sub_of, p4, sx, sy, sz};
  if (!plan->ok) return;
  const int nbig = *big_cnt;
  for (int bi = blockIdx.x; bi < nbig; bi += gridDim.x) {
    const int c = big_list[bi];
    order_run_by_octant<256>(keyed, start[c], start[c + 1], tot, base, wcnt, out, rec);
  }
}

static constexpr int kBkBig = 255;
static constexpr int kBkPer = 12;

static constexpr int kBkPts = 2048;

template <bool F32>
struct BkRec;
template <>
struct BkRec<true> {
  using type = float4;
};
template <>
struct BkRec<false> {
  using type = PointRec;
};

template <int MODE>
__global__ __launch_bounds__(256) void k_bk_hist(const double* __restrict__ xyz, int64_t n, GridParams g,
                                                 int rx, int ry, int rz, AxisMap am, int nbk, int bits,
                                                 int32_t* __restrict__ key_tmp,
                                                 int32_t* __restrict__ tot, const GridPlan* __restrict__ plan) {
  extern __shared__ __attribute__((aligned(16))) int32_t h[];
  if (plan) {
    if (!plan->ok) return;
    g = GridParams{plan->mn[0], plan->mn[1], plan->mn[2], plan->inv_cell, plan->nx, plan->ny, plan->nz};
    rx = plan->rx;
    ry = plan->ry;
    rz = plan->rz;
    nbk = plan->nbk;
    bits = plan->bits;
  }
  for (int b = threadIdx.x; b < nbk; b += 256) h[b] = 0;
  __syncthreads();
  const int64_t base = int64_t(blockIdx.x) * kBkPts;
#pragma unroll
  for (int k = 0; k < kBkPts / 256; ++k) {
    const int64_t i = base + k * 256 + threadIdx.x;
    if (i < n) {
      int c, oct = 0;
      if (MODE == 2) {
        c = cell_index(g, xyz[3 * i], xyz[3 * i + 1], xyz[3 * i + 2]);
      } else {
        const RawCell r = raw_cell(g, rx, ry, rz, xyz[3 * i], xyz[3 * i + 1], xyz[3 * i + 2]);
        const int cx = MODE == 1 ? am.x[r.cx] : r.cx + 1, cy = MODE == 1 ? am.y[r.cy] : r.cy + 1,
                  cz = MODE == 1 ? am.z[r.cz] : r.cz + 1;
        c = (cz * g.ny + cy) * g.nx + cx;
        oct = r.oct;
      }
      key_tmp[i] = (c << 3) | oct;
      atomicAdd(&h[c >> bits], 1);
    }
  }
  __syncthreads();
  for (int b = threadIdx.x; b < nbk; b += 256) {
    const int v = h[b];
    if (v) atomicAdd(&tot[b], v);
  }
}

static constexpr int kBkFusedScan = 4096;
__global__ __launch_bounds__(1024) void k_bk_scan(int nbk, const int32_t* __restrict__ tot,
                                                  int32_t* __restrict__ bstart, const GridPlan* __restrict__ plan) {
  __shared__ int32_t wsum[16];
  if (plan) {
    if (!plan->ok) return;
    nbk = plan->nbk;
  }
  const int per = (nbk + 1023) / 1024;
  const int b0 = threadIdx.x * per;
  int32_t v[16], s = 0;
  for (int k = 0; k < per; ++k) {
    v[k] = b0 + k < nbk ? tot[b0 + k] : 0;
    s += v[k];
  }
  int32_t run = block_excl_scan<1024>(s, wsum);
  for (int k = 0; k < per; ++k) {
    if (b0 + k < nbk) bstart[b0 + k] = run;
    run += v[k];
  }
  if (threadIdx.x == 1023) bstart[nbk] = run;
}

template <bool F32>
__global__ __launch_bounds__(256) void k_bk_scatter(const double* __restrict__ xyz, int64_t n, int nbk,
                                                    int bits, const int32_t* __restrict__ key_tmp,
                                                    const int32_t* __restrict__ tot,
                                                    int32_t* __restrict__ cursor ,
                                                    int32_t* __restrict__ bstart ,
                                                    int fused,
                                                    typename BkRec<F32>::type* __restrict__ bucketed,
                                                    int32_t* __restrict__ keyb ,
                                                    const GridPlan* __restrict__ plan) {
  extern __shared__ __attribute__((aligned(16))) int32_t h[];
  const int64_t base = int64_t(blockIdx.x) * kBkPts;
  using Coord = typename std::conditional<F32, float, double>::type;
  int key[kBkPts / 256], lr[kBkPts / 256];
  Coord px[kBkPts / 256], py[kBkPts / 256], pz[kBkPts / 256];
#pragma unroll
  for (int k = 0; k < kBkPts / 256; ++k) {
    const int64_t i = base + k * 256 + threadIdx.x;
    key[k] = -1;
    px[k] = py[k] = pz[k] = Coord(0);
    if (i < n) {
      key[k] = key_tmp[i];
      px[k] = Coord(xyz[3 * i]);
      py[k] = Coord(xyz[3 * i + 1]);
      pz[k] = Coord(xyz[3 * i + 2]);
    }
  }
  if (plan) {
    if (!plan->ok) return;
    nbk = plan->nbk;
    bits = plan->bits;
  }
  int32_t* pre = h + nbk;
  __shared__ int32_t wsum[4];
  for (int b = threadIdx.x; b < nbk; b += 256) h[b] = 0;
  if (fused) {
    constexpr int kPer = kBkFusedScan / 256;
    const int b0 = threadIdx.x * kPer;
    int32_t v[kPer], s = 0;
#pragma unroll
    for (int k = 0; k < kPer; ++k) {
      v[k] = b0 + k < nbk ? tot[b0 + k] : 0;
      s += v[k];
    }
    int32_t run = block_excl_scan<256>(s, wsum);
#pragma unroll
    for (int k = 0; k < kPer; ++k) {
      if (b0 + k < nbk) {
        pre[b0 + k] = run;
        if (blockIdx.x == 0) bstart[b0 + k] = run;
      }
      run += v[k];
    }
    if (blockIdx.x == 0 && threadIdx.x == 255) bstart[nbk] = run;
  }
  __syncthreads();
#pragma unroll
  for (int k = 0; k < kBkPts / 256; ++k) {
    lr[k] = key[k] >= 0 ? atomicAdd(&h[key[k] >> (3 + bits)], 1) : 0;
  }
  __syncthreads();
  for (int bb = 0; bb < nbk; bb += 16 * 256) {
    int32_t v[16], a[16];
#pragma unroll
    for (int k = 0; k < 16; ++k) {
      const int b = bb + k * 256 + threadIdx.x;
      v[k] = b < nbk ? h[b] : 0;
    }
#pragma unroll
    for (int k = 0; k < 16; ++k) {
      a[k] = 0;
      if (v[k]) a[k] = atomicAdd(&cursor[bb + k * 256 + threadIdx.x], v[k]);
    }
#pragma unroll
    for (int k = 0; k < 16; ++k) {
      const int b = bb + k * 256 + threadIdx.x;
      if (v[k]) h[b] = (fused ? pre[b] : bstart[b]) + a[k];
    }
  }
  __syncthreads();
#pragma unroll
  for (int k = 0; k < kBkPts / 256; ++k) {
    if (key[k] < 0) continue;
    const int64_t i = base + k * 256 + threadIdx.x;
    const int pos = h[key[k] >> (3 + bits)] + lr[k];
    keyb[pos] = key[k];
    if constexpr (F32) {
      bucketed[pos] = make_float4(px[k], py[k], pz[k], __int_as_float(int(i)));
    } else {
      PointRec r;
      r.x = px[k];
      r.y = py[k];
      r.z = pz[k];
      r.idx = int(i);
      r.key = key[k];
      bucketed[pos] = r;
    }
  }
}

template <bool F32>
static constexpr int kBkGrp = F32 ? 2 : 1;

__device__ __forceinline__ int rec_idx(const float4& p) { return __float_as_int(p.w); }
__device__ __forceinline__ int rec_idx(const PointRec& p) { return p.idx; }

template <int BITS, bool F32, class Policy>
__device__ __forceinline__ void bk_two_sweeps(Policy& P, int s, int e,
                                              const typename BkRec<F32>::type* __restrict__ bucketed,
                                              const int32_t* __restrict__ keyb, uint32_t* __restrict__ word_tmp) {
  constexpr int CELLS = 1 << BITS, T = CELLS / 8, CAP = T * kBkPer, G = kBkGrp<F32>;
  using Rec = typename BkRec<F32>::type;
  static_assert(kBkPer % G == 0, "whole groups");
  const int t = threadIdx.x;
// ... 266 lines not shown
        slots[sb + __popcll(hm)] = e;
        L.wsum[0] = __popcll(hm);
      }
    }
    __syncthreads();
    if (t < WORDS) {
      const int nd = L.wsum[0];
      uint32_t bits = 0u, before = 0u;
      for (int q = 0; q < nd; ++q) {
        const int c = dcell[q];
        before += c < 32 * t ? 1u : 0u;
        bits |= (c >> 5) == t ? 1u << (c & 31) : 0u;
      }
      wds[t] = DirWord{bits, sb + before};
    }
    return;
  }
  BkOctants<BITS, F32> P{L, s, e, c0, wds, slots, sb, rec, keyed, rank_tmp, out, 0u, 0, 0};
  bk_two_sweeps<BITS, F32>(P, s, e, bucketed, keyb, word_tmp);
  __syncthreads();
  if (!L.any_big) return;
  for (int wd = 0; wd < CELLS / 32; ++wd) {
    for (uint32_t bm = L.big[wd]; bm; bm &= bm - 1u) {
      const int cl = wd * 32 + __ffs(bm) - 1;
      order_run_by_octant<T>(keyed, s + L.cnt[cl], s + (cl + 1 < CELLS ? L.cnt[cl + 1] : e - s), L.btot, L.bbase,
                             L.bw, out, rec);
    }
  }
  });
}

template <int BITS>
struct BkPlainLds {
  int32_t cnt[1 << BITS];
  int32_t wsum[16], wocc[16];
};

template <int BITS, bool F32>
struct BkPlain {
  static constexpr int CELLS = 1 << BITS, T = CELLS / 8, RB = 32 - BITS, RMAX = (1 << RB) - 1;
  using Rec = typename BkRec<F32>::type;
  BkPlainLds<BITS>& L;
  const int s, bk;
  const int64_t c0, ncell1;
  int32_t* const start;
  int32_t* const occ;
  int32_t* const rank_tmp;
  const SortedStore& out;

  __device__ __forceinline__ int32_t* cnt() const { return L.cnt; }
  __device__ __forceinline__ void clear(int t) const {
#pragma unroll
    for (int k = 0; k < 8; ++k) L.cnt[k * T + t] = 0;
  }
  __device__ __forceinline__ uint32_t rank_of(uint32_t ky, int j) const {
    const int cl = int(ky >> 3) & (CELLS - 1);
    const int rr = atomicAdd(&L.cnt[cl], 1);
    if (rr >= RMAX) rank_tmp[j] = rr;
    return (uint32_t(cl) << RB) | uint32_t(rr < RMAX ? rr : RMAX);
  }
  __device__ __forceinline__ int32_t scan(const int32_t (&v)[8], int32_t tot, int t) const {
    int32_t nocc = 0;
#pragma unroll
    for (int k = 0; k < 8; ++k) nocc += v[k] > 0;
#pragma unroll
    for (int off = 32; off > 0; off >>= 1) nocc += __shfl_down(nocc, off, 64);
    if ((t & 63) == 0) L.wocc[t >> 6] = nocc;
    const int32_t run = block_excl_scan<T>(tot, L.wsum);
    if (t == 0) {
      int o = 0;
      for (int q = 0; q < T / 64; ++q) o += L.wocc[q];
      occ[bk] = o;
    }
    return run;
  }
  __device__ __forceinline__ void directory(const int32_t (&)[8], const int32_t (&pre)[8], int t) const {
    const int64_t cidx = c0 + 8 * t;
    if (cidx + 7 < ncell1) {
      *reinterpret_cast<int4*>(start + cidx) = make_int4(s + pre[0], s + pre[1], s + pre[2], s + pre[3]);
      *reinterpret_cast<int4*>(start + cidx + 4) = make_int4(s + pre[4], s + pre[5], s + pre[6], s + pre[7]);
    } else {
#pragma unroll
      for (int k = 0; k < 8; ++k)
        if (cidx + k < ncell1) start[cidx + k] = s + pre[k];
    }
#pragma unroll
    for (int k = 0; k < 8; ++k) L.cnt[8 * t + k] = pre[k];
  }
  __device__ __forceinline__ void place(const Rec& p, uint32_t w, int j) const {
    const int cl = int(w >> RB), arr = int(w & uint32_t(RMAX));
    out.put(s + L.cnt[cl] + (arr < RMAX ? arr : rank_tmp[j]), rec_idx(p), int(c0) + cl, p.x, p.y, p.z);
  }
};

template <int BITS, bool F32>
__global__ __launch_bounds__((1 << BITS) / 8, BITS == 12 ? 6 : 4) void k_bk_sort_plain(
    int64_t ncell1, const int32_t* __restrict__ bstart, const typename BkRec<F32>::type* __restrict__ bucketed,
    const int32_t* __restrict__ keyb, uint32_t* __restrict__ word_tmp, int32_t* __restrict__ rank_tmp,
    int32_t* __restrict__ start, int32_t* __restrict__ order,
    int32_t* __restrict__ cell_of, double* __restrict__ sx, double* __restrict__ sy, double* __restrict__ sz,
    float4* __restrict__ p4 , int32_t* __restrict__ occ) {
  constexpr int T = (1 << BITS) / 8;
  __shared__ BkPlainLds<BITS> L;
  const SortedStore out{order, cell_of, nullptr, F32 ? p4 : nullptr, sx, sy, sz};
  const int bk = blockIdx.x, t = threadIdx.x;
  const int s = bstart[bk], e = bstart[bk + 1];
  const int64_t c0 = int64_t(bk) << BITS;
  if (s == e) {
#pragma unroll
    for (int k = 0; k < 2; ++k) {
      const int64_t cidx = c0 + int64_t(k * T + t) * 4;
      if (cidx + 3 < ncell1) {
        *reinterpret_cast<int4*>(start + cidx) = make_int4(s, s, s, s);
      } else {
        for (int u = 0; u < 4; ++u)
          if (cidx + u < ncell1) start[cidx + u] = s;
      }
    }
    if (t == 0) occ[bk] = 0;
    return;
  }
  BkPlain<BITS, F32> P{L, s, bk, c0, ncell1, start, occ, rank_tmp, out};
  bk_two_sweeps<BITS, F32>(P, s, e, bucketed, keyb, word_tmp);
}

static bool bucketed_fits(const DevGrid& g) {
  const char* env = getenv("PYQSM_GRID_BIN");
  return bucket_shape(g.ncell).nbk <= kBkMax && !(env && !strcmp(env, "atomic"));
}

template <int BITS_, bool F32_>
struct Sort {
  static constexpr int BITS = BITS_;
  static constexpr bool F32 = F32_;
  using Rec = typename BkRec<F32_>::type;
};
template <class F>
static void on_sort_shape(int bits, bool f32, F&& launch) {
  if (bits == 12) {
    if (f32)
      launch(Sort<12, true>{});
    else
      launch(Sort<12, false>{});
  } else {
    if (f32)
      launch(Sort<13, true>{});
    else
      launch(Sort<13, false>{});
  }
}

static void enqueue_bk_a(Ctx* c, int mode, bool f32, const double* xyz, int64_t n, const GridParams& gp,
                         const int raw[3], AxisMap am, int64_t nbk, int bits, int32_t* key_tmp, int32_t* tot,
                         int32_t* cursor, int32_t* bstart, void* bucketed, int32_t* keyb, const GridPlan* d_plan) {
  const dim3 ga(ceil_div(n, kBkPts)), blk(256);
  const size_t lds = size_t(nbk) * 4;
  const int fused = nbk <= kBkFusedScan;
#define PQ_BK_HIST(MODE)                                                                                         \
  hipLaunchKernelGGL(k_bk_hist<MODE>, ga, blk, lds, c->stream, xyz, n, gp, raw[0], raw[1], raw[2], am, int(nbk), \
                     bits, key_tmp, tot, d_plan)
  if (mode == 0)
    PQ_BK_HIST(0);
  else if (mode == 1)
    PQ_BK_HIST(1);
  else
    PQ_BK_HIST(2);
#undef PQ_BK_HIST
  if (!fused) hipLaunchKernelGGL(k_bk_scan, dim3(1), dim3(1024), 0, c->stream, int(nbk), tot, bstart, d_plan);
  if (f32)
    hipLaunchKernelGGL(k_bk_scatter<true>, ga, blk, fused ? 2 * lds : lds, c->stream, xyz, n, int(nbk), bits,
                       key_tmp, tot, cursor, bstart, fused, static_cast<float4*>(bucketed), keyb, d_plan);
  else
    hipLaunchKernelGGL(k_bk_scatter<false>, ga, blk, fused ? 2 * lds : lds, c->stream, xyz, n, int(nbk), bits,
                       key_tmp, tot, cursor, bstart, fused, static_cast<PointRec*>(bucketed), keyb, d_plan);
}

static int build_grid_bucketed(Ctx* c, const double* xyz, int64_t n, DevGrid* g) {
  const int bits = bucket_shape(g->ncell).bits;
  const int64_t nbk = bucket_shape(g->ncell).nbk;
  const bool f32 = g->p4 != nullptr;
  int32_t *tot, *bstart, *cursor, *key_tmp, *keyb, *rank_tmp;
  uint32_t* word_tmp;
  void* bucketed;
  PQ_TRY(c->arena.get(size_t(nbk) * 2, &tot));
  cursor = tot + nbk;
  PQ_TRY(c->arena.get(size_t(nbk) + 1, &bstart));
  PQ_TRY(c->arena.get(size_t(n), &key_tmp));
  PQ_TRY(c->arena.get(size_t(n), &keyb));
  PQ_TRY(c->arena.get(size_t(n), &word_tmp));
  PQ_TRY(c->arena.get(size_t(n), &rank_tmp));
  if (f32) {
    float4* b4;
    PQ_TRY(c->arena.get(size_t(n), &b4));
    bucketed = b4;
  } else {
    PointRec* b8;
    PQ_TRY(c->arena.get(size_t(n), &b8));
    bucketed = b8;
  }
  g->occ_blocks = int(nbk);
  PQ_TRY(c->arena.get(size_t(nbk), &g->occ_part));
  PQ_HIP(hipMemsetAsync(tot, 0, size_t(nbk) * 8, c->stream));
  const int raw[3] = {0, 0, 0};
  enqueue_bk_a(c, 2, f32, xyz, n, grid_params(*g), raw, AxisMap{nullptr, nullptr, nullptr}, nbk, bits, key_tmp, tot,
               cursor, bstart, bucketed, keyb, nullptr);
  on_sort_shape(bits, f32, [&](auto S) {
    using K = decltype(S);
    hipLaunchKernelGGL((k_bk_sort_plain<K::BITS, K::F32>), dim3(unsigned(nbk)), dim3((1 << K::BITS) / 8), 0, c->stream,
                       g->ncell + 1, bstart, static_cast<const typename K::Rec*>(bucketed), keyb, word_tmp, rank_tmp,
                       g->start, g->order, g->cell_of, g->sx, g->sy, g->sz, g->p4, g->occ_part);
  });
  PQ_HIP(hipGetLastError());
  return 0;
}


__device__ void write_plan(const unsigned long long* box, const PlanIn& in, GridPlan* __restrict__ plan) {
  GridPlan p;
  bool ok = in.hint.valid != 0;
  for (int a = 0; a < 3; ++a) {
    p.mn[a] = ord_val(box[a]);
    p.mx[a] = ord_val(box[3 + a]);
    ok = ok && isfinite(p.mn[a]) && isfinite(p.mx[a]);
  }
  p.all_f32 = box[6] != 0 ? 1 : 0;
  ok = ok && p.all_f32;
  double tot;
  int raw[3];
  ok = interior_slabs(p.mn, p.mx, in.cell, 2.0, raw, &tot) && ok;
  ok = ok && tot <= double(in.max_cells);
  p.inv_cell = 1.0 / in.cell;
  p.rx = raw[0];
  p.ry = raw[1];
  p.rz = raw[2];
  p.nx = raw[0] + 2;
  p.ny = raw[1] + 2;
  p.nz = raw[2] + 2;
  const int64_t ncell = ok ? int64_t(p.nx) * p.ny * p.nz : 0;
  const BucketShape bs = bucket_shape(ncell);
  const int64_t nbk = bs.nbk;
  ok = ok && bs.bits == 12 && ncell <= in.hint.ncell && nbk <= in.hint.nbk &&
       (nbk <= kBkFusedScan) == (in.hint.fused != 0);
  p.ncell = ok ? int(ncell) : 0;
  p.nbk = ok ? int(nbk) : 0;
  p.bits = 12;
  p.ok = ok ? 1 : 0;
  p.seq = in.seq;
  *plan = p;
  if (in.host) {
    p.seq = 0;
    *in.host = p;
    __threadfence_system();
    *reinterpret_cast<volatile unsigned*>(&in.host->seq) = in.seq;
  }
}

int plan_grid_device(Ctx* c, const double* xyz, int64_t n, double cell, int64_t max_cells, const PlanHint& hint,
                     GridPlan* d_plan, GridPlan* h_plan, unsigned seq, int32_t* zero_buf, int zero_n) {
  if (n <= 0) return fail(PYQSM_EINVAL, "bounding box of an empty cloud");
  const int blocks = int(std::min<int64_t>(ceil_div(n, 256), int64_t(c->cu_count) * 4));
  unsigned long long *d_box = nullptr, *d_part = nullptr;
  PQ_TRY(c->arena.get(kBoxVals, &d_box));
  PQ_TRY(c->arena.get(size_t(blocks) * kBoxVals, &d_part));
  hipLaunchKernelGGL(k_bbox, dim3(blocks), dim3(256), 0, c->stream, xyz, n, d_part, stamp_slots(c, blocks));
  hipLaunchKernelGGL(k_bbox_fold, dim3(1), dim3(256), 0, c->stream, d_part, blocks, d_box, zero_buf, zero_n,
                     PlanIn{cell, max_cells, hint, h_plan, seq}, d_plan);
  PQ_HIP(hipGetLastError());
  return 0;
}

int octant_zeroed_ints() { return 2 * kBkMax + 5 + kZeroedExtra; }

static int enqueue_bucketed(Ctx* c, const double* xyz, int64_t n, const GridParams& gp, const int raw[3],
                            AxisMap am, bool mapped, int64_t nbk, int bits, bool f32,
                            int32_t* zeroed, const GridPlan* d_plan, DevGrid* g, SubCells* sub) {
  int32_t *cell_tmp, *keyb, *rank_tmp, *bstart;
  uint32_t* word_tmp;
  int32_t *tot = zeroed, *cursor = zeroed + kBkMax;
  PointRec* keyed;
  void* bucketed;
  g->p4 = nullptr;
  g->sx = g->sy = g->sz = nullptr;
  g->start = nullptr;
  PQ_TRY(c->arena.get(size_t(nbk) << (bits - 5), &g->dir_words));
  PQ_TRY(c->arena.get(size_t(n) + size_t(nbk) + 1, &g->dir_slots));
  PQ_TRY(c->arena.get(size_t(n), &g->order));
  PQ_TRY(c->arena.get(size_t(n), &g->cell_of));
  if (f32) {
    float4* b4;
    PQ_TRY(c->arena.get(size_t(n), &g->p4));
    PQ_TRY(c->arena.get(size_t(n), &b4));
    bucketed = b4;
  } else {
    PointRec* b8;
    PQ_TRY(c->arena.get(size_t(n), &g->sx));
    PQ_TRY(c->arena.get(size_t(n), &g->sy));
    PQ_TRY(c->arena.get(size_t(n), &g->sz));
    PQ_TRY(c->arena.get(size_t(n), &b8));
    bucketed = b8;
  }
  PQ_TRY(c->arena.get(size_t(n), &cell_tmp));
  PQ_TRY(c->arena.get(size_t(n), &keyb));
  PQ_TRY(c->arena.get(size_t(n), &word_tmp));
  PQ_TRY(c->arena.get(size_t(n), &rank_tmp));
  PQ_TRY(c->arena.get(size_t(n), &keyed));
  PQ_TRY(c->arena.get(size_t(n), &sub->sub_of));
  PQ_TRY(c->arena.get(size_t(n) * 8, &sub->rec));
  PQ_TRY(c->arena.get(size_t(nbk) + 1, &bstart));
  enqueue_bk_a(c, mapped ? 1 : 0, f32, xyz, n, gp, raw, am, nbk, bits, cell_tmp, tot, cursor, bstart, bucketed, keyb,
               d_plan);
  on_sort_shape(bits, f32, [&](auto S) {
    using K = decltype(S);
    unsigned long long* const st_sort = stamp_slots(c, nbk);
    hipLaunchKernelGGL((k_bk_sort<K::BITS, K::F32>), dim3(unsigned(nbk)), dim3((1 << K::BITS) / 8), 0, c->stream,
                       bstart, static_cast<const typename K::Rec*>(bucketed), keyb, word_tmp, rank_tmp, g->dir_words,
                       g->dir_slots, g->order, g->cell_of, sub->sub_of, g->sx, g->sy, g->sz, g->p4, sub->rec, keyed,
                       d_plan, st_sort);
  });
  PQ_HIP(hipGetLastError());
  return 0;
}

__global__ __launch_bounds__(256) void k_dir_from_dense(int64_t ncell, const int32_t* __restrict__ start,
                                                        DirWord* __restrict__ words, int32_t* __restrict__ slots) {
  const int64_t c = int64_t(blockIdx.x) * 256 + threadIdx.x;
  const int lane = threadIdx.x & 63, half = lane >> 5;
  const int a = start[c < ncell ? c : ncell];
  const int b = start[c + 1 < ncell ? c + 1 : ncell];
  const uint32_t bits = uint32_t(__ballot(b != a) >> (32 * half));
  const int64_t w = c >> 5;
  const uint32_t base = uint32_t(__shfl(a, half * 32, 64)) + uint32_t(w);
  if (w > (ncell >> 5)) return;
  if (b != a) slots[base + __popc(bits & ((1u << (lane & 31)) - 1u))] = a;
  if ((lane & 31) == 31) slots[base + __popc(bits)] = b;
  if ((lane & 31) == 0) words[w] = DirWord{bits, base};
}

static int dir_from_dense(Ctx* c, int64_t n, DevGrid* g) {
  const int64_t nwords = (g->ncell >> 5) + 1;
  PQ_TRY(c->arena.get(size_t(nwords), &g->dir_words));
  PQ_TRY(c->arena.get(size_t(n) + size_t(nwords) + 1, &g->dir_slots));
  hipLaunchKernelGGL(k_dir_from_dense, dim3(unsigned(ceil_div(nwords * 32, 256))), dim3(256), 0, c->stream, g->ncell,
                     g->start, g->dir_words, g->dir_slots);
  PQ_HIP(hipGetLastError());
  return 0;
}

__global__ __launch_bounds__(256) void k_read_directory(int64_t ncell, const CellDir dir,
                                                        int32_t* __restrict__ out) {
  const int64_t c = int64_t(blockIdx.x) * 256 + threadIdx.x;
  if (c <= ncell) out[c] = dir.begin(int(c));
}

void read_directory(Ctx* c, const DevGrid& g, int64_t ncell, int32_t* begin_out) {
  hipLaunchKernelGGL(k_read_directory, dim3(unsigned(ceil_div(ncell + 1, 256))), dim3(256), 0, c->stream, ncell,
                     cell_dir(g), begin_out);
}

int bin_octants_planned(Ctx* c, const double* xyz, int64_t n, double cell, const PlanHint& hint,
                        const GridPlan* d_plan, int32_t* zeroed, DevGrid* g, SubCells* sub) {
  g->minx = g->miny = g->minz = 0.0;
  g->cell = cell;
  g->inv_cell = 1.0 / cell;
  g->nx = g->ny = g->nz = 0;
  g->ncell = hint.ncell;
  sub->zeroed4 = zeroed + 2 * kBkMax + 1;
  const int raw[3] = {0, 0, 0};
  return enqueue_bucketed(c, xyz, n, GridParams{}, raw, AxisMap{nullptr, nullptr, nullptr}, false, hint.nbk, 12,
                          true, zeroed, d_plan, g, sub);
}

static int upload_plan(Ctx* c, const GridPlan& p, GridPlan* h_up, GridPlan* d_plan) {
  *h_up = p;
  PQ_TRY(copy_in(c, d_plan, h_up, 1));
  return 0;
}

int bin_octants_host(Ctx* c, const double* xyz, int64_t n, double min_cell, int64_t max_cells, const GridPlan& box,
                     int32_t* zeroed, GridPlan* h_up, GridPlan* d_plan, DevGrid* g, SubCells* sub,
                     PlanHint* hint_out) {
  *hint_out = PlanHint{};
  if (n <= 0) return fail(PYQSM_EINVAL, "build_grid_octants: empty cloud");
  if (n > (int64_t(1) << 27)) return fail(PYQSM_ERANGE, "octant sub-cells: more than 2^27 points");
  if (max_cells > (int64_t(1) << 28)) max_cells = int64_t(1) << 28;
  if (!(min_cell > 0) || !std::isfinite(min_cell))
    return fail(PYQSM_EINVAL, "cell edge must be positive and finite");
  double mn[3], mx[3];
  for (int a = 0; a < 3; ++a) {
    mn[a] = box.mn[a];
    mx[a] = box.mx[a];
    if (!std::isfinite(mn[a]) || !std::isfinite(mx[a])) return fail(PYQSM_EINVAL, "point coordinates must be finite");
  }
  bool all_f32 = box.all_f32 != 0;
  sub->zeroed4 = zeroed + 2 * kBkMax + 1;
  GridPlan hp{};
  {
    const char* f32_env = getenv("PYQSM_COORD_F32");
    if (f32_env && !strcmp(f32_env, "0")) all_f32 = false;
  }
  const char* bin_env = getenv("PYQSM_DBSCAN_BIN");
  const dim3 grid(ceil_div(n, 256)), blk(256);
  double cell = min_cell;
  int raw[3], dims[3];
  AxisMap am{nullptr, nullptr, nullptr};
  bool mapped = false;
  for (;;) {
    double tot;
    const bool ok = interior_slabs(mn, mx, cell, 2.0, raw, &tot);
    for (int a = 0; a < 3; ++a) dims[a] = raw[a] + 2;
    if (ok && tot <= double(max_cells)) break;
    const int64_t raw_sum = ok ? int64_t(raw[0]) + raw[1] + raw[2] : int64_t(1) << 40;
    if (raw_sum <= (int64_t(1) << 27)) {
      GridParams gp{mn[0], mn[1], mn[2], 1.0 / cell, 0, 0, 0};
      int32_t* occ[3];
      int32_t* map[3];
      for (int a = 0; a < 3; ++a) {
        PQ_TRY(c->arena.get(size_t(raw[a]) + 1, &occ[a]));
        PQ_TRY(c->arena.get(size_t(raw[a]) + 1, &map[a]));
        PQ_HIP(hipMemsetAsync(occ[a], 0, (size_t(raw[a]) + 1) * 4, c->stream));
      }
      hipLaunchKernelGGL(k_axis_occ, grid, blk, 0, c->stream, xyz, n, gp, raw[0], raw[1], raw[2], occ[0],
                         occ[1], occ[2]);
      double ctot = 1.0;
      for (int a = 0; a < 3; ++a) {
        hipLaunchKernelGGL(k_axis_keep, dim3(ceil_div(raw[a] + 1, 256)), blk, 0, c->stream, raw[a], occ[a],
                           map[a]);
        PQ_HIP(hipGetLastError());
        PQ_TRY(exclusive_scan_i32(c, map[a], int64_t(raw[a]) + 1));
        int32_t kept = 0;
        PQ_TRY(fetch(c, &kept, map[a] + raw[a]));
        hipLaunchKernelGGL(k_axis_shift, dim3(ceil_div(raw[a], 256)), blk, 0, c->stream, raw[a], map[a]);
        dims[a] = kept + 2;
        ctot *= double(dims[a]);
      }
      PQ_HIP(hipGetLastError());
      if (ctot <= double(max_cells)) {
        am = AxisMap{map[0], map[1], map[2]};
        mapped = true;
        break;
      }
    }
    cell *= 2.0;
  }
  g->minx = mn[0];
  g->miny = mn[1];
  g->minz = mn[2];
  g->cell = cell;
  g->inv_cell = 1.0 / cell;
  g->nx = dims[0];
  g->ny = dims[1];
  g->nz = dims[2];
  g->ncell = int64_t(dims[0]) * dims[1] * dims[2];
  const int bits = bucket_shape(g->ncell).bits;
  const int64_t nbk = bucket_shape(g->ncell).nbk;
  const bool bucketed_path = nbk <= kBkMax && !(bin_env && !strcmp(bin_env, "atomic"));
  for (int a = 0; a < 3; ++a) {
    hp.mn[a] = mn[a];
    hp.mx[a] = mx[a];
  }
  hp.inv_cell = g->inv_cell;
  hp.nx = dims[0];
  hp.ny = dims[1];
  hp.nz = dims[2];
  hp.rx = raw[0];
  hp.ry = raw[1];
  hp.rz = raw[2];
  hp.ncell = int(g->ncell);
  hp.nbk = int(nbk);
  hp.bits = bits;
  hp.all_f32 = all_f32 && bucketed_path;
  hp.ok = 1;
  PQ_TRY(upload_plan(c, hp, h_up, d_plan));
  const GridParams gp = grid_params(*g);
  if (bucketed_path) {
    PQ_TRY(enqueue_bucketed(c, xyz, n, gp, raw, am, mapped, nbk, bits, hp.all_f32, zeroed, d_plan, g, sub));
    if (!mapped && cell == min_cell && bits == 12 && hp.all_f32) {
      int64_t ncell_h = std::min<int64_t>(g->ncell + g->ncell / 16, (int64_t(kBkMax) << 12) - 1);
      if (nbk <= kBkFusedScan) ncell_h = std::min<int64_t>(ncell_h, (int64_t(kBkFusedScan) << 12) - 1);
      hint_out->valid = 1;
      hint_out->ncell = int(ncell_h);
      hint_out->nbk = int(bucket_shape(ncell_h).nbk);
      hint_out->fused = nbk <= kBkFusedScan;
    }
    return 0;
  }
  int32_t *cell_tmp, *rank_tmp, *big_list, *big_cnt = zeroed + 2 * kBkMax;
  PointRec* keyed;
  g->p4 = nullptr;
  PQ_TRY(c->arena.get(size_t(g->ncell) + 1, &g->start));
  PQ_TRY(c->arena.get(size_t(n), &g->order));
  PQ_TRY(c->arena.get(size_t(n), &g->cell_of));
  PQ_TRY(c->arena.get(size_t(n), &g->sx));
  PQ_TRY(c->arena.get(size_t(n), &g->sy));
  PQ_TRY(c->arena.get(size_t(n), &g->sz));
  PQ_TRY(c->arena.get(size_t(n), &cell_tmp));
  PQ_TRY(c->arena.get(size_t(n), &rank_tmp));
  PQ_TRY(c->arena.get(size_t(n), &keyed));
  PQ_TRY(c->arena.get(size_t(n), &sub->sub_of));
  PQ_TRY(c->arena.get(size_t(n) * 8, &sub->rec));
  PQ_TRY(c->arena.get(size_t(n) / kBigCell + 2, &big_list));
  PQ_HIP(hipMemsetAsync(g->start, 0, (size_t(g->ncell) + 1) * 4, c->stream));
  if (mapped)
    hipLaunchKernelGGL(k_cell_count_oct<true>, grid, blk, 0, c->stream, xyz, n, gp, raw[0], raw[1], raw[2],
                       am, g->start, cell_tmp, rank_tmp);
  else
    hipLaunchKernelGGL(k_cell_count_oct<false>, grid, blk, 0, c->stream, xyz, n, gp, raw[0], raw[1], raw[2],
                       am, g->start, cell_tmp, rank_tmp);
  PQ_HIP(hipGetLastError());
  PQ_TRY(exclusive_scan_i32(c, g->start, g->ncell + 1));
  hipLaunchKernelGGL(k_scatter_keys, grid, blk, 0, c->stream, xyz, n, g->start, cell_tmp, rank_tmp, keyed);
  hipLaunchKernelGGL(k_order_cells, grid, blk, 0, c->stream, int(n), g->start, keyed, g->order,
                     g->cell_of, sub->sub_of, g->sx, g->sy, g->sz, sub->rec, big_list, big_cnt);
  PQ_HIP(hipGetLastError());
  hipLaunchKernelGGL(k_order_big, dim3(unsigned(std::min<int64_t>(n / kBigCell + 1, 2048))), blk, 0,
                     c->stream, big_list, big_cnt, g->start, keyed, g->order, g->cell_of, sub->sub_of,
                     g->sx, g->sy, g->sz, g->p4, sub->rec, d_plan);
  PQ_HIP(hipGetLastError());
  return dir_from_dense(c, n, g);
}


struct Pyr {
// ... 228 lines not shown
```

pyqsm_amd/csrc/grid.hpp:

```cpp
#pragma once
#include "common.hpp"

namespace pyqsm {

struct alignas(8) DirWord {
  uint32_t bits, base;
};
struct CellDir {
  const DirWord* words;
  const int32_t* slots;
  __device__ __forceinline__ static int slot_of(const DirWord w, int c) {
    return int(w.base) + __popc(w.bits & ((1u << (c & 31)) - 1u));
  }
  __device__ __forceinline__ int begin(int c) const { return slots[slot_of(words[c >> 5], c)]; }
  template <int N>
  __device__ __forceinline__ void begins(const int (&c)[N], int (&out)[N]) const {
    DirWord w[N];
#pragma unroll
    for (int i = 0; i < N; ++i) w[i] = words[c[i] >> 5];
#pragma unroll
    for (int i = 0; i < N; ++i) out[i] = slots[slot_of(w[i], c[i])];
  }
};

// ... 100 lines not shown
  float4* p;
  __device__ __forceinline__ void get(int q, double& a, double& b, double& c) const {
    const float4 v = p[q];
    a = double(v.x);
    b = double(v.y);
    c = double(v.z);
  }
  __device__ __forceinline__ double d2(int q, double px, double py, double pz) const {
    const float4 v = p[q];
    return sqdist3(px, py, pz, double(v.x), double(v.y), double(v.z));
  }
  __device__ __forceinline__ double d2(int a, int q) const {
    const float4 u = p[a], v = p[q];
    return sqdist3(double(u.x), double(u.y), double(u.z), double(v.x), double(v.y), double(v.z));
  }
  __device__ __forceinline__ void mark_core(int q, bool is_core) const {
    reinterpret_cast<float*>(p)[size_t(q) * 4 + 3] = is_core ? 1.0f : 0.0f;
  }
  __device__ __forceinline__ bool core_pair_within(int a, int q, const uint8_t* __restrict__, double r2) const {
    const float4 u = p[a], v = p[q];
    return u.w != 0.0f && v.w != 0.0f &&
           sqdist3(double(u.x), double(u.y), double(u.z), double(v.x), double(v.y), double(v.z)) <= r2;
  }
};


static constexpr int kTileMax = 16384;

struct Tile {
  int qb[9], qe[9];
  int total;
};

__device__ __forceinline__ Tile wave_tile(int p0, int n, Stencil st, int ncell, const CellDir& dir,
                                          const int32_t* __restrict__ cell_of) {
  Tile t;
  const int plast = p0 + 63 < n ? p0 + 63 : n - 1;
  const int c_first = __builtin_amdgcn_readfirstlane(cell_of[p0]);
  const int c_last = __builtin_amdgcn_readfirstlane(cell_of[plast]);
  int lo[9], hi[9];
#pragma unroll
  for (int w = 0; w < 9; ++w) {
    const int o = (w % 3 - 1) * st.nx + (w / 3 - 1) * st.nxy;
    const int a = c_first + o - 1, b = c_last + o + 1;
    lo[w] = a < 0 ? 0 : a;
    hi[w] = b > ncell - 1 ? ncell - 1 : b;
  }
#pragma unroll
  for (int i = 1; i < 9; ++i)
#pragma unroll
    for (int k = i; k > 0; --k) {
      const bool sw = lo[k - 1] > lo[k];
      const int l0 = lo[k - 1], h0 = hi[k - 1];
      lo[k - 1] = sw ? lo[k] : l0;
      hi[k - 1] = sw ? hi[k] : h0;
      lo[k] = sw ? l0 : lo[k];
      hi[k] = sw ? h0 : hi[k];
    }
  int cells[18], q[18];
  int prev_hi = -1;
#pragma unroll
  for (int r = 0; r < 9; ++r) {
    const int a = lo[r] <= prev_hi ? prev_hi + 1 : lo[r];
    cells[2 * r] = cells[2 * r + 1] = 0;
    if (a <= hi[r]) {
      cells[2 * r] = a;
      cells[2 * r + 1] = hi[r] + 1;
      prev_hi = hi[r];
    }
  }
  dir.begins(cells, q);
  t.total = 0;
#pragma unroll
  for (int r = 0; r < 9; ++r) {
    t.qb[r] = __builtin_amdgcn_readfirstlane(q[2 * r]);
    t.qe[r] = __builtin_amdgcn_readfirstlane(q[2 * r + 1]);
    t.total += t.qe[r] - t.qb[r];
  }
  return t;
}

template <class F>
inline void on_coords(const DevGrid& g, F&& fn) {
  if (g.p4)
    fn(CoordsF32{g.p4});
  else
    fn(CoordsF64{g.sx, g.sy, g.sz});
}

struct SortedStore {
  int32_t* order;
  int32_t* cell_of;
  int32_t* sub_of;
  float4* p4;
  double *sx, *sy, *sz;
  __device__ __forceinline__ void put(int f, int idx, int cell, double x, double y, double z, int sub = 0) const {
    if (cell_of) cell_of[f] = cell;
    if (sub_of) sub_of[f] = sub;
    order[f] = idx;
    if (p4) {
      p4[f] = make_float4(float(x), float(y), float(z), 0.f);
    } else {
      sx[f] = x;
      sy[f] = y;
      sz[f] = z;
    }
  }
  __device__ __forceinline__ void put(int f, int idx, int cell, float x, float y, float z, int sub = 0) const {
    if (cell_of) cell_of[f] = cell;
    if (sub_of) sub_of[f] = sub;
    order[f] = idx;
    p4[f] = make_float4(x, y, z, 0.f);
  }
};

struct SubCells {
  int32_t* sub_of;
  int4* rec;
  int32_t* zeroed4 = nullptr;
};
static constexpr int kZeroedExtra = 64;

template <class CountOf>
__device__ __forceinline__ void write_sub_records_of(int4* __restrict__ rec, int b, CountOf&& count_of) {
  int run = b;
#pragma unroll
  for (int o = 0; o < 8; ++o) {
    const int cnt = count_of(o);
    rec[size_t(b) * 8 + o] = make_int4(run, cnt, -1, 0);
    run += cnt;
  }
}
__device__ __forceinline__ void write_sub_records(int4* __restrict__ rec, int b, const int (&cnt)[8]) {
  write_sub_records_of(rec, b, [&](int o) { return cnt[o]; });
}
__device__ __forceinline__ void write_sub_records(int4* __restrict__ rec, int b, unsigned long long packed) {
  write_sub_records_of(rec, b, [&](int o) { return int((packed >> (8 * o)) & 255ull); });
}


struct GridPlan {
  double mn[3], mx[3];
  double inv_cell;
  int nx, ny, nz;
  int rx, ry, rz;
  int ncell;
  int nbk, bits;
  int all_f32;
  int ok;
  unsigned seq;
};
__device__ __forceinline__ Stencil plan_stencil(const GridPlan* p) { return Stencil{p->nx, p->nx * p->ny}; }

int plan_grid_device(Ctx* c, const double* xyz, int64_t n, double cell, int64_t max_cells, const PlanHint& hint,
                     GridPlan* d_plan, GridPlan* h_plan, unsigned seq, int32_t* zero_buf, int zero_n);
int octant_zeroed_ints();
int bin_octants_planned(Ctx* c, const double* xyz, int64_t n, double cell, const PlanHint& hint,
                        const GridPlan* d_plan, int32_t* zeroed, DevGrid* g, SubCells* sub);
int bin_octants_host(Ctx* c, const double* xyz, int64_t n, double min_cell, int64_t max_cells, const GridPlan& box,
                     int32_t* zeroed, GridPlan* h_up, GridPlan* d_plan, DevGrid* g, SubCells* sub,
                     PlanHint* hint_out);

void read_directory(Ctx* c, const DevGrid& g, int64_t ncell, int32_t* begin_out);

int coarsen_grid(Ctx* c, const DevGrid& fine, int64_t n, int factor, DevGrid* coarse);

int ball_grid(Ctx* c, const double* d_src, int64_t n, double radius, DevGrid* g, double* cloud_box = nullptr);
int radius_grid(Ctx* c, const double* d_src, int64_t n, double radius, DevGrid* g);
int query_order(Ctx* c, const double* d_qry, int64_t m, const GridParams& rg, int64_t ncell, int32_t** perm);

int count_occupied(Ctx* c, const DevGrid& g, int64_t* occupied);

}
```

pyqsm_amd/hip.py:

```python
from __future__ import annotations

import ctypes
import weakref
from typing import NamedTuple

import numpy as np

from . import _lib
from ._lib import check, i64, i32, dbl, vp

MISS_PRIM = np.uint32(0xFFFFFFFF)


def _p(a):
    return None if a is None else a.ctypes.data_as(ctypes.c_void_p)


def _points(points) -> np.ndarray:
    pts = np.ascontiguousarray(np.asarray(points), dtype=np.float64)
    if pts.ndim != 2 or pts.shape[1] != 3:
        raise ValueError(f"expected points of shape [n,3], got {pts.shape}")
    return pts


# ... 33 lines not shown
            self.ptr = None

    def __del__(self):
        try:
            self.free()
        except Exception:
            pass


def sync(device: int = 0) -> None:
    check(_lib.load().pyqsm_sync(int(device)))


def prof_enable(on, device: int = 0) -> None:
    check(_lib.load().pyqsm_prof_enable(int(device), int(on)))


def prof_reset(device: int = 0) -> None:
    check(_lib.load().pyqsm_prof_reset(int(device)))


def prof_get(name: str, device: int = 0):
    ms, cnt = dbl(0.0), i64(0)
    check(_lib.load().pyqsm_prof_get(int(device), name.encode(), ctypes.byref(ms),
                                     ctypes.byref(cnt)))
    return ms.value, cnt.value



def _mesh(verts, tris):
    v = np.ascontiguousarray(np.asarray(verts), dtype=np.float32).reshape(-1, 3)
    t = np.ascontiguousarray(np.asarray(tris), dtype=np.int32).reshape(-1, 3)
    return v, t


def cast_rays(verts, tris, rays, device: int = 0):
    v, t = _mesh(verts, tris)
    r = np.ascontiguousarray(np.asarray(rays), dtype=np.float32)
    if r.shape[-1] != 6:
        raise ValueError(f"rays must have last dimension 6, got {r.shape}")
    lead = r.shape[:-1]
    r2 = r.reshape(-1, 6)
    R = r2.shape[0]
    t_hit = np.empty(R, dtype=np.float32)
    prim = np.empty(R, dtype=np.uint32)
    uv = np.empty((R, 2), dtype=np.float32)
    check(_lib.load().pyqsm_cast_rays(_p(v), v.shape[0], _p(t), t.shape[0], _p(r2), R,
                                      _p(t_hit), _p(prim), _p(uv), int(device)))
    return t_hit.reshape(lead), prim.reshape(lead), uv.reshape(lead + (2,))


def cast_rays_multi(verts, tris, rays, n_devices: int = 0, with_uv: bool = True):
    v, t = _mesh(verts, tris)
    r = np.ascontiguousarray(np.asarray(rays), dtype=np.float32)
    if r.shape[-1] != 6:
        raise ValueError(f"rays must have last dimension 6, got {r.shape}")
    lead = r.shape[:-1]
    r2 = r.reshape(-1, 6)
    R = r2.shape[0]
    t_hit = np.empty(R, dtype=np.float32)
    prim = np.empty(R, dtype=np.uint32)
    uv = np.empty((R, 2), dtype=np.float32) if with_uv else None
    check(_lib.load().pyqsm_cast_rays_multi(_p(v), v.shape[0], _p(t), t.shape[0], _p(r2), R,
                                            _p(t_hit), _p(prim), _p(uv) if with_uv else None,
                                            int(n_devices)))
    return t_hit.reshape(lead), prim.reshape(lead), uv.reshape(lead + (2,)) if with_uv else None


def list_intersections(verts, tris, rays, device: int = 0):
    v, t = _mesh(verts, tris)
    r = np.ascontiguousarray(np.asarray(rays), dtype=np.float32).reshape(-1, 6)
    R = r.shape[0]
    lib = _lib.load()
    counts = np.zeros(R, dtype=np.int32)
    total = i64(0)
    check(lib.pyqsm_list_intersections(_p(v), v.shape[0], _p(t), t.shape[0], _p(r), R, _p(counts),
                                       None, None, None, None, 0, ctypes.byref(total),
                                       int(device)))
    n = int(total.value)
    ray_ids = np.empty(n, dtype=np.uint32)
    prim = np.empty(n, dtype=np.uint32)
    ts = np.empty(n, dtype=np.float32)
    uv = np.empty((n, 2), dtype=np.float32)
    if n:
        check(lib.pyqsm_list_intersections(_p(v), v.shape[0], _p(t), t.shape[0], _p(r), R,
                                           _p(counts), _p(ray_ids), _p(prim), _p(ts), _p(uv), n,
                                           ctypes.byref(total), int(device)))
    return {"ray_ids": ray_ids, "primitive_ids": prim, "t_hit": ts, "primitive_uvs": uv,
            "counts": counts}


def point_mesh_distance(verts, tris, queries, device: int = 0):
    v, t = _mesh(verts, tris)
    q = np.ascontiguousarray(queries, dtype=np.float32).reshape(-1, 3)
    dist = np.empty(q.shape[0], dtype=np.float32)
    prim = np.empty(q.shape[0], dtype=np.uint32)
    check(_lib.load().pyqsm_point_mesh_distance(_p(v), v.shape[0], _p(t), t.shape[0], _p(q), q.shape[0],
                                                _p(dist), _p(prim), int(device)))
    return dist, prim


class DeviceMesh:

    def __init__(self, verts, tris, device: int = 0):
        v, t = _mesh(verts, tris)
        self.device = int(device)
        self.n_tris = t.shape[0]
        dv = DeviceBuffer.from_array(v, device) if v.size else None
        dt = DeviceBuffer.from_array(t, device) if t.size else None
        self.records = DeviceBuffer(max(1, self.n_tris) * 48, device)
        if self.n_tris:
            check(_lib.load().pyqsm_expand_tris_dev(dv.ptr, v.shape[0], dt.ptr, self.n_tris,
                                                    self.records.ptr, self.device))
            sync(device)
        for b in (dv, dt):
            if b is not None:
                b.free()


def cast_rays_dev(mesh: DeviceMesh, rays_ptr: int, n_rays: int, t_hit_ptr: int, prim_ptr: int,
                  uv_ptr: int | None = None) -> None:
    check(_lib.load().pyqsm_cast_rays_dev(mesh.records.ptr, mesh.n_tris, rays_ptr, int(n_rays),
                                          t_hit_ptr, prim_ptr, uv_ptr, mesh.device))



def dbscan(points, eps: float, min_pts: int, device: int = 0, radius_inclusive: bool = True):
    pts = _points(points)
    n = pts.shape[0]
    labels = np.empty(n, dtype=np.int64)
    core = np.zeros(n, dtype=np.uint8)
    check(_lib.load().pyqsm_dbscan_ex(_p(pts), n, float(eps), int(min_pts), int(bool(radius_inclusive)),
                                      _p(labels), _p(core), int(device)))
    return labels, core.astype(bool)


def dbscan_dev(xyz_ptr: int, n: int, eps: float, min_pts: int, labels_ptr: int,
               core_ptr: int | None = None, device: int = 0, want_count: bool = False,
               radius_inclusive: bool = True):
    cnt = i64(0)
    check(_lib.load().pyqsm_dbscan_dev_ex(xyz_ptr, int(n), float(eps), int(min_pts),
                                          int(bool(radius_inclusive)), labels_ptr, core_ptr,
                                          ctypes.byref(cnt) if want_count else None, int(device)))
    return int(cnt.value) if want_count else None


def octant_directory(points, eps: float, device: int = 0, cap: int = 1 << 25):
    pts = _points(points)
    dims = np.zeros(3, dtype=np.int32)
    begin = np.empty(int(cap), dtype=np.int32)
    check(_lib.load().pyqsm_octant_directory(_p(pts), pts.shape[0], float(eps), _p(dims), _p(begin), int(cap),
                                             int(device)))
    return dims, begin[: int(np.prod(dims.astype(np.int64))) + 1].copy()


def knn(points, k: int, exclude_self: bool = True, device: int = 0):
    pts = _points(points)
    n = pts.shape[0]
    idx = np.empty((n, int(k)), dtype=np.int32)
    d2 = np.empty((n, int(k)), dtype=np.float64)
    check(_lib.load().pyqsm_knn(_p(pts), n, int(k), int(bool(exclude_self)), _p(idx), _p(d2),
                                int(device)))
    return idx, d2


def knn_dev(xyz_ptr: int, n: int, k: int, exclude_self: bool, idx_ptr: int, d2_ptr: int,
            device: int = 0) -> None:
    check(_lib.load().pyqsm_knn_dev(xyz_ptr, int(n), int(k), int(bool(exclude_self)), idx_ptr,
                                    d2_ptr, int(device)))



SHAPES = {"circle": 0, "cylinder": 1}


def ransac(points, triples, shape: str = "circle", thresh: float = 0.2, device: int = 0):
    pts = _points(points)
    tri = np.ascontiguousarray(np.asarray(triples), dtype=np.int64).reshape(-1, 3)
    n, H = pts.shape[0], tri.shape[0]
    if H and (tri.min() < 0 or tri.max() >= n):
        raise ValueError("sample index outside the point set")
    center = np.zeros(3)
    axis = np.zeros(3)
    radius = dbl(0.0)
    inl = np.empty(max(n, 1), dtype=np.int64)
    n_in, best = i64(0), i64(-1)
    check(_lib.load().pyqsm_ransac(_p(pts), n, _p(tri), H, SHAPES[shape], float(thresh),
                                   _p(center), _p(axis), ctypes.byref(radius), _p(inl),
                                   ctypes.byref(n_in), ctypes.byref(best), int(device)))
    return center, axis, radius.value, inl[:n_in.value].copy(), int(best.value)


def ransac_batch(points, seg_start, triples, shape: str = "circle", thresh: float = 0.2, device: int = 0):
    pts = _points(points)
    ss = np.ascontiguousarray(seg_start, dtype=np.int64)
    S = len(ss) - 1
    tri = np.ascontiguousarray(np.asarray(triples), dtype=np.int64).reshape(S, -1, 3)
    H = tri.shape[1]
    sizes = np.diff(ss)
    if H and S:
        ok = (tri >= 0).all(axis=(1, 2)) | (sizes < 3)
        if not ok.all() or (tri.max(axis=(1, 2)) >= np.maximum(sizes, 1))[sizes >= 3].any():
            raise ValueError("sample index outside its point set")
    centers = np.zeros((S, 3))
    axes = np.zeros((S, 3))
    radii = np.zeros(S)
    inl = np.empty(max(pts.shape[0], 1), dtype=np.int64)
    n_in = np.zeros(S, dtype=np.int64)
    best = np.full(S, -1, dtype=np.int64)
    check(_lib.load().pyqsm_ransac_batch(_p(pts), pts.shape[0], _p(ss), S, _p(tri), H, SHAPES[shape],
                                         float(thresh), _p(centers), _p(axes), _p(radii), _p(inl), _p(n_in),
                                         _p(best), int(device)))
    ends = np.cumsum(n_in)
    inliers = [inl[e - c:e].copy() for c, e in zip(n_in, ends)]
    return centers, axes, radii, inliers, best


def ransac_models(points, triples, device: int = 0):
    pts = _points(points)
    tri = np.ascontiguousarray(np.asarray(triples), dtype=np.int64).reshape(-1, 3)
    models = np.zeros((tri.shape[0], 8))
    check(_lib.load().pyqsm_ransac_models(_p(pts), pts.shape[0], _p(tri), tri.shape[0],
                                          _p(models), int(device)))
    return models


def ransac_count(points, models, shape: str = "circle", thresh: float = 0.2, device: int = 0):
    pts = _points(points)
    m = np.ascontiguousarray(models, dtype=np.float64).reshape(-1, 8)
    counts = np.zeros(m.shape[0], dtype=np.int32)
    check(_lib.load().pyqsm_ransac_count(_p(pts), pts.shape[0], _p(m), m.shape[0], SHAPES[shape],
                                         float(thresh), _p(counts), int(device)))
    return counts



def _plane_samples(samples) -> np.ndarray:
    smp = np.ascontiguousarray(np.asarray(samples), dtype=np.int64)
    if smp.ndim != 2:
        raise ValueError(f"expected samples of shape [H,m], got {smp.shape}")
    return smp


def _plane_axis(axis):
    if axis is None:
        return None
    ax = np.ascontiguousarray(np.asarray(axis, dtype=np.float64).reshape(3))
    return ax


def plane_models(points, samples, axis=None, cos_limit: float = 0.0, device: int = 0):
    pts = _points(points)
    smp = _plane_samples(samples)
    H, m = smp.shape
    ax = _plane_axis(axis)
    planes = np.zeros((H, 4))
    check(_lib.load().pyqsm_plane_models(_p(pts), pts.shape[0], _p(smp), H, m, _p(ax), float(cos_limit),
                                         _p(planes), int(device)))
    return planes


def plane_count(points, planes, thresh: float, device: int = 0):
    pts = _points(points)
    pl = np.ascontiguousarray(planes, dtype=np.float64).reshape(-1, 4)
    counts = np.zeros(pl.shape[0], dtype=np.int32)
    check(_lib.load().pyqsm_plane_count(_p(pts), pts.shape[0], _p(pl), pl.shape[0], float(thresh), _p(counts),
                                        int(device)))
    return counts


def segment_plane(points, samples, thresh: float, probability: float = 0.99999999, axis=None,
                  cos_limit: float = 0.0, device: int = 0):
    pts = _points(points)
    smp = _plane_samples(samples)
    H, m = smp.shape
    ax = _plane_axis(axis)
    fit, hyp = np.zeros(4), np.zeros(4)
    inl = np.empty(max(pts.shape[0], 1), dtype=np.int64)
    n_in, best, used = i64(0), i64(-1), i64(0)
    check(_lib.load().pyqsm_segment_plane(_p(pts), pts.shape[0], _p(smp), H, m, float(thresh), float(probability),
                                          _p(ax), float(cos_limit), _p(fit), _p(hyp), _p(inl), ctypes.byref(n_in),
                                          ctypes.byref(best), ctypes.byref(used), int(device)))
    return fit, hyp, inl[:n_in.value].copy(), int(best.value), int(used.value)


class PlaneSegments:

    def __init__(self, planes, hypothesis_planes, labels, counts, best, used):
        self.planes = planes
        self.hypothesis_planes = hypothesis_planes
        self.labels = labels
        self.counts = counts
        self.best = best
        self.used = used

    def __len__(self):
        return len(self.planes)

    def indices(self, i: int) -> np.ndarray:
        return np.flatnonzero(self.labels == int(i)).astype(np.int64)

    def rest(self) -> np.ndarray:
        return np.flatnonzero(self.labels < 0).astype(np.int64)

    def __repr__(self):
        return f"PlaneSegments with {len(self.planes)} planes over {len(self.labels)} points."
# ... 1268 lines not shown
```

Measured before the change: 3765 Mpoints/s.

## Count core neighbors with clamped packed-FMA ramp and fold bbox plan into histogram

The f32 core-counting loop now turns each squared distance into a 0/1 indicator using a clamped v_pk_fma (d*-K + A, saturated), and sums those indicators in packed float accumulators. This replaces the scalar compare-and-add pairs, and LDS is read as float4 so the inner loop is unrolled by 8. Separately, the bbox fold kernel is removed on the speculative path: its reduction is fused into an extra block of the bucket histogram kernel, and the zero-fill moves into k_bbox, which also gets fewer blocks. Test-probe APIs for the ramp constants are added as well. The risks are exactness of the float-ramp threshold near the band edges and the added complexity of the kernel fusion.

```diff
diff --git a/include/pyqsm_hip.h b/include/pyqsm_hip.h
--- a/include/pyqsm_hip.h
+++ b/include/pyqsm_hip.h
@@ -84,6 +84,9 @@
                         int64_t* n_clusters, int32_t device);
 int pyqsm_octant_directory(const double* xyz, int64_t n, double eps, int32_t* dims_out,
                            int32_t* begin_out, int64_t cap, int32_t device);
+int pyqsm_core_ramp_constants(double eps, int32_t radius_inclusive, float* out);
+int pyqsm_core_ramp_probe(const float* d, int64_t n, double eps, int32_t radius_inclusive,
+                          float* s_in_out, float* s_hi_out, int32_t device);
 
 int pyqsm_knn(const double* xyz, int64_t n, int32_t k, int32_t exclude_self,
               int32_t* idx, double* d2, int32_t device);
diff --git a/pyqsm_amd/_lib.py b/pyqsm_amd/_lib.py
--- a/pyqsm_amd/_lib.py
+++ b/pyqsm_amd/_lib.py
@@ -48,6 +48,8 @@
     "pyqsm_dbscan_ex": (ctypes.c_int, [vp, i64, dbl, i32, i32, vp, vp, i32]),
     "pyqsm_dbscan_dev_ex": (ctypes.c_int, [vp, i64, dbl, i32, i32, vp, vp, ctypes.POINTER(i64), i32]),
     "pyqsm_octant_directory": (ctypes.c_int, [vp, i64, dbl, vp, vp, i64, i32]),
+    "pyqsm_core_ramp_constants": (ctypes.c_int, [dbl, i32, vp]),
+    "pyqsm_core_ramp_probe": (ctypes.c_int, [vp, i64, dbl, i32, vp, vp, i32]),
     "pyqsm_knn": (ctypes.c_int, [vp, i64, i32, i32, vp, vp, i32]),
     "pyqsm_knn_dev": (ctypes.c_int, [vp, i64, i32, i32, vp, vp, i32]),
     "pyqsm_ransac": (ctypes.c_int, [vp, i64, vp, i64, i32, dbl, vp, vp, ctypes.POINTER(dbl), vp,
diff --git a/pyqsm_amd/csrc/dbscan.hip b/pyqsm_amd/csrc/dbscan.hip
--- a/pyqsm_amd/csrc/dbscan.hip
+++ b/pyqsm_amd/csrc/dbscan.hip
@@ -39,6 +39,7 @@
   alignas(16) float x[4][64], y[4][64], z[4][64];
 };
 typedef float float2v __attribute__((ext_vector_type(2)));
+typedef float float4v __attribute__((ext_vector_type(4)));
 
 struct CoreBand {
   float lo, hi;
@@ -55,6 +56,49 @@
   return t;
 }
 
+struct CoreRamp {
+  float lo, hi;
+  float K, A, B;
+  bool usable(int min_pts = 1) const {
+    return CoreBand{lo, hi}.usable() && std::isnormal(K) && std::isnormal(A) && std::isnormal(B) &&
+           min_pts <= (1 << 20);
+  }
+};
+static CoreRamp core_ramp(double r2) {
+  const CoreBand cb = core_band(r2);
+  CoreRamp t{cb.lo, cb.hi, 0.0f, 0.0f, 0.0f};
+  if (!cb.usable()) return t;
+  int x;
+  const double m = frexp(r2, &x);
+  const int e = m == 0.5 ? x - 21 : x - 20;
+  if (e < -126 || e > 126) return t;
+  t.K = float(ldexp(1.0, -e));
+  const double a = ldexp(double(cb.lo), -e), b = 1.0 + ldexp(double(cb.hi), -e);
+  t.A = float(a);
+  if (double(t.A) > a) t.A = nextafterf(t.A, -INFINITY);
+  t.B = float(b);
+  if (double(t.B) < b) t.B = nextafterf(t.B, INFINITY);
+  return t;
+}
+__device__ __forceinline__ float2v core_ramp_sat(float2v d, float2v neg_k, float2v c) {
+  float2v s;
+  asm("v_pk_fma_f32 %0, %1, %2, %3 clamp" : "=v"(s) : "v"(d), "v"(neg_k), "v"(c));
+  return s;
+}
+
+__global__ __launch_bounds__(256) void k_core_ramp_probe(const float* __restrict__ d, int64_t n, float neg_k,
+                                                         float ramp_a, float ramp_b, float* __restrict__ s_in,
+                                                         float* __restrict__ s_hi) {
+  const int64_t i = 2 * (int64_t(blockIdx.x) * blockDim.x + threadIdx.x);
+  if (i >= n) return;
+  const bool two = i + 1 < n;
+  const float2v v = {d[i], two ? d[i + 1] : INFINITY};
+  const float2v a = core_ramp_sat(v, float2v{neg_k, neg_k}, float2v{ramp_a, ramp_a});
+  const float2v b = core_ramp_sat(v, float2v{neg_k, neg_k}, float2v{ramp_b, ramp_b});
+  s_in[i] = a.x, s_hi[i] = b.x;
+  if (two) s_in[i + 1] = a.y, s_hi[i + 1] = b.y;
+}
+
 static constexpr int kStragglers = 6;
 static constexpr int kMaxChunks = 3;
 static constexpr int kRestSegs = 64;
@@ -81,7 +125,7 @@
                                                     const DirWord* __restrict__ dwords,
                                                     const int32_t* __restrict__ dslots,
                                                     const int32_t* __restrict__ cell_of, CO co, double r2,
-                                                    float r2_lo, float r2_hi ,
+                                                    float neg_k, float ramp_a, float ramp_b ,
                                                     int min_pts, uint8_t* __restrict__ core,
                                                     int32_t* __restrict__ rest,
                                                     int32_t* __restrict__ rest_cnt , int seg_cap,
@@ -114,7 +158,8 @@
   }
   const Tile t = wave_tile(p0, n, st, ncell, dir, cell_of);
   int cnt = 0;
-  int cnt_hi = 0;
+  float2v acc_in = {0.0f, 0.0f}, acc_hi = {0.0f, 0.0f};
+  const float fmin_pts = float(min_pts);
   bool deferred = false;
   int chunks = 0;
   int staged = 0;
@@ -127,7 +172,7 @@
       if (lane == lead) slot = atomicAdd(rest_cnt + seg, __popcll(und));
       slot = __shfl(slot, lead, 64);
       const bool mine = (und >> lane) & 1ull;
-      if constexpr (F32) band += __popcll(__ballot(mine && cnt_hi > cnt));
+      if constexpr (F32) band += __popcll(__ballot(mine && acc_hi.x + acc_hi.y > acc_in.x + acc_in.y));
       if (mine) {
         rest[size_t(seg) * seg_cap + slot + __popcll(und & ((1ull << lane) - 1ull))] = p;
         cnt = -1;
@@ -135,6 +180,7 @@
     }
     deferred = true;
   };
+  const bool ramped = F32 && t.total <= kTileMax;
   if (t.total > kTileMax) {
     if constexpr (F32) x = double(fx), y = double(fy), z = double(fz);
     const int mycell = live ? cell_of[p] : -1;
@@ -165,6 +211,7 @@
     }
   } else {
     const float2v X = {fx, fx}, Y = {fy, fy}, Z = {fz, fz};
+    const float2v NK = {neg_k, neg_k}, RA = {ramp_a, ramp_a}, RB = {ramp_b, ramp_b};
 #pragma unroll
     for (int ri = 0; ri < 9; ++ri) {
       const int r = kRunOrder[ri];
@@ -176,19 +223,28 @@
           if (q < t.qe[r]) v = co.p[q];
           LF.x[w][lane] = v.x, LF.y[w][lane] = v.y, LF.z[w][lane] = v.z;
           __builtin_amdgcn_wave_barrier();
-#pragma unroll 4
-          for (int j = 0; j < m; j += 2) {
-            const float2v dx = X - *reinterpret_cast<const float2v*>(&LF.x[w][j]);
-            const float2v dy = Y - *reinterpret_cast<const float2v*>(&LF.y[w][j]);
-            const float2v dz = Z - *reinterpret_cast<const float2v*>(&LF.z[w][j]);
+          const auto pair = [&](float2v cx, float2v cy, float2v cz) {
+            const float2v dx = X - cx, dy = Y - cy, dz = Z - cz;
             float2v d = dx * dx;
             d = __builtin_elementwise_fma(dy, dy, d);
             d = __builtin_elementwise_fma(dz, dz, d);
-            cnt += d.x <= r2_lo;
-            cnt += d.y <= r2_lo;
-            cnt_hi += d.x <= r2_hi;
-            cnt_hi += d.y <= r2_hi;
+            acc_in += core_ramp_sat(d, NK, RA);
+            acc_hi += core_ramp_sat(d, NK, RB);
+          };
+          int j = 0;
+          for (; j + 8 <= m; j += 8) {
+            const float4v* const lx = reinterpret_cast<const float4v*>(&LF.x[w][j]);
+            const float4v* const ly = reinterpret_cast<const float4v*>(&LF.y[w][j]);
+            const float4v* const lz = reinterpret_cast<const float4v*>(&LF.z[w][j]);
+            const float4v x0 = lx[0], x1 = lx[1], y0 = ly[0], y1 = ly[1], z0 = lz[0], z1 = lz[1];
+            pair(x0.lo, y0.lo, z0.lo);
+            pair(x0.hi, y0.hi, z0.hi);
+            pair(x1.lo, y1.lo, z1.lo);
+            pair(x1.hi, y1.hi, z1.hi);
           }
+          for (; j < m; j += 2)
+            pair(*reinterpret_cast<const float2v*>(&LF.x[w][j]), *reinterpret_cast<const float2v*>(&LF.y[w][j]),
+                 *reinterpret_cast<const float2v*>(&LF.z[w][j]));
         } else {
           if (q < t.qe[r]) co.get(q, L.x[w][lane], L.y[w][lane], L.z[w][lane]);
           __builtin_amdgcn_wave_barrier();
@@ -198,7 +254,8 @@
         }
         staged += m;
         __builtin_amdgcn_wave_barrier();
-        const unsigned long long und = __ballot(live && cnt < min_pts);
+        const unsigned long long und =
+            F32 ? __ballot(live && acc_in.x + acc_in.y < fmin_pts) : __ballot(live && cnt < min_pts);
         ++chunks;
         if ((__popcll(und) <= kStragglers || chunks >= max_chunks) &&
             !(ri == 8 && base + 64 >= t.qe[r])) {
@@ -208,12 +265,14 @@
       }
     }
     if constexpr (F32) {
-      if (!deferred) hand_on(__ballot(live && cnt < min_pts && cnt_hi >= min_pts));
+      if (!deferred)
+        hand_on(__ballot(live && acc_in.x + acc_in.y < fmin_pts && acc_hi.x + acc_hi.y >= fmin_pts));
     }
   }
   if (live && cnt >= 0) {
-    core[p] = cnt >= min_pts;
-    co.mark_core(p, cnt >= min_pts);
+    const bool is_core = ramped ? acc_in.x + acc_in.y >= fmin_pts : cnt >= min_pts;
+    core[p] = is_core;
+    co.mark_core(p, is_core);
   }
   if (live) {
     parent[p] = p;
@@ -1147,6 +1206,10 @@
   });
 }
 
+static double dbscan_r2(double eps, bool radius_inclusive) {
+  return radius_inclusive ? eps * eps : nextafter(eps * eps, 0.0);
+}
+
 static int cluster_binned(Ctx* c, int64_t n, double eps, int32_t min_pts, bool radius_inclusive, const DevGrid& g,
                           const SubCells& sub, const GridPlan* d_plan, int64_t* labels, uint8_t* is_core,
                           const int32_t** count_out) {
@@ -1155,7 +1218,7 @@
   const dim3 grid(ceil_div(n, 256)), block(256);
   const Stencil st{g.nx, g.nx * g.ny};
   const CellDir dir = cell_dir(g);
-  const double r2 = radius_inclusive ? eps * eps : nextafter(eps * eps, 0.0);
+  const double r2 = dbscan_r2(eps, radius_inclusive);
   uint8_t* core;
   int *parent, *min_orig;
   uint32_t* bits;
@@ -1198,12 +1261,12 @@
     const int max_chunks = std::min(32, std::max(kMaxChunks, (kMaxChunks * min_pts + 9) / 10));
     {
       const StampKernel pk(c, "k_core_tiled", grid.x);
-      const CoreBand cb = core_band(r2);
-      const bool f32 = cb.usable();
+      const CoreRamp cr = core_ramp(r2);
+      const bool f32 = cr.usable(min_pts);
       on_coords(g, [&](auto co) {
         const auto launch = [&](auto kernel) {
-          hipLaunchKernelGGL(kernel, grid, block, 0, c->stream, N, d_plan, dir.words, dir.slots, g.cell_of, co, r2, cb.lo,
-                             cb.hi, min_pts, core, rest, rest_segs, seg_cap, parent, min_orig, bits, seam,
+          hipLaunchKernelGGL(kernel, grid, block, 0, c->stream, N, d_plan, dir.words, dir.slots, g.cell_of, co, r2, -cr.K,
+                             cr.A, cr.B, min_pts, core, rest, rest_segs, seg_cap, parent, min_orig, bits, seam,
                              g.start ? 0 : int(seam_cap), max_chunks, d_tests, pk.slots);
         };
         if constexpr (std::is_same_v<decltype(co), CoordsF32>) {
@@ -1450,10 +1513,12 @@
   SubCells sub;
   const int32_t* count = nullptr;
   std::optional<StampScope> bin_scope(std::in_place, c, "dbscan_bin");
-  PQ_TRY(plan_grid_device(c, xyz, n, cell, max_cells, hint, d_plan, h_plan_dev, seq, zeroed, octant_zeroed_ints()));
+  PlanRecords rec{};
+  PQ_TRY(plan_grid_device(c, xyz, n, cell, max_cells, hint, d_plan, h_plan_dev, seq, zeroed, octant_zeroed_ints(),
+                          speculate ? &rec : nullptr));
   const Arena::Mark mark = c->arena.mark();
   if (speculate) {
-    PQ_TRY(bin_octants_planned(c, xyz, n, cell, hint, d_plan, zeroed, &g, &sub));
+    PQ_TRY(bin_octants_planned(c, xyz, n, cell, hint, rec, d_plan, zeroed, &g, &sub));
     bin_scope.reset();
     if (!readout)
       PQ_TRY(cluster_binned(c, n, eps, min_pts, radius_inclusive, g, sub, d_plan, labels, is_core, &count));
@@ -1570,4 +1635,35 @@
   return 0;
 }
 
-}
+int pyqsm_core_ramp_constants(double eps, int32_t radius_inclusive, float* out) {
+  if (!out) return fail(PYQSM_EINVAL, "pyqsm_core_ramp_constants: NULL pointer");
+  const CoreRamp cr = core_ramp(dbscan_r2(eps, radius_inclusive != 0));
+  out[0] = cr.lo, out[1] = cr.hi, out[2] = cr.K, out[3] = cr.A, out[4] = cr.B;
+  out[5] = cr.usable() ? 1.0f : 0.0f;
+  return 0;
+}
+
+int pyqsm_core_ramp_probe(const float* d, int64_t n, double eps, int32_t radius_inclusive, float* s_in_out,
+                          float* s_hi_out, int32_t device) {
+  PQ_API_RANGE("pyqsm_core_ramp_probe");
+  if (n < 0) return fail(PYQSM_EINVAL, "negative size");
+  const CoreRamp cr = core_ramp(dbscan_r2(eps, radius_inclusive != 0));
+  if (!cr.usable()) return fail(PYQSM_EINVAL, "pyqsm_core_ramp_probe: no ramp form at this eps");
+  if (n == 0) return 0;
+  if (!d || !s_in_out || !s_hi_out) return fail(PYQSM_EINVAL, "pyqsm_core_ramp_probe: NULL pointer");
+  Call call(device);
+  Ctx* c = call.c;
+  if (!c) return PYQSM_ENODEV;
+  float *d_d, *d_in, *d_hi;
+  PQ_TRY(upload(c, d, size_t(n), &d_d));
+  PQ_TRY(c->arena.get(size_t(n), &d_in));
+  PQ_TRY(c->arena.get(size_t(n), &d_hi));
+  hipLaunchKernelGGL(k_core_ramp_probe, dim3(ceil_div(ceil_div(n, 2), 256)), dim3(256), 0, c->stream, d_d, n, -cr.K,
+                     cr.A, cr.B, d_in, d_hi);
+  PQ_HIP(hipGetLastError());
+  PQ_TRY(fetch(c, s_in_out, d_in, size_t(n)));
+  PQ_TRY(fetch(c, s_hi_out, d_hi, size_t(n)));
+  return 0;
+}
+
+}
diff --git a/pyqsm_amd/csrc/grid.hip b/pyqsm_amd/csrc/grid.hip
--- a/pyqsm_amd/csrc/grid.hip
+++ b/pyqsm_amd/csrc/grid.hip
@@ -45,16 +45,20 @@
 }
 
 static constexpr int kBoxVals = 7;
+static int bbox_blocks(const Ctx* c, int64_t n) {
+  return int(std::min<int64_t>(ceil_div(n, 256), int64_t(c->cu_count) * 2));
+}
 __global__ __launch_bounds__(256) void k_bbox(const double* __restrict__ xyz, int64_t n,
                                               unsigned long long* __restrict__ part ,
+                                              int32_t* __restrict__ zero_buf, int zero_n,
     unsigned long long* __restrict__ st ) {
   __shared__ unsigned long long red[4][6];
   __shared__ int red_f32[4];
   stamped(st, [&] {
   unsigned long long mn[3] = {~0ull, ~0ull, ~0ull}, mx[3] = {0, 0, 0};
   bool f32ok = true;
-  for (int64_t i = blockIdx.x * int64_t(blockDim.x) + threadIdx.x; i < n;
-       i += int64_t(gridDim.x) * blockDim.x) {
+  const int64_t stride = int64_t(gridDim.x) * blockDim.x;
+  for (int64_t i = blockIdx.x * int64_t(blockDim.x) + threadIdx.x; i < n; i += stride) {
 #pragma unroll
     for (int a = 0; a < 3; ++a) {
       const double v = xyz[3 * i + a];
@@ -64,6 +68,7 @@
       mx[a] = k > mx[a] ? k : mx[a];
     }
   }
+  for (int64_t q = blockIdx.x * int64_t(blockDim.x) + threadIdx.x; q < zero_n; q += stride) zero_buf[q] = 0;
   const bool wave_ok = __all(f32ok);
 #pragma unroll
   for (int a = 0; a < 3; ++a) {
@@ -104,47 +109,53 @@
   GridPlan* host;
   unsigned seq;
 };
-__device__ void write_plan(const unsigned long long* box, const PlanIn& in, GridPlan* __restrict__ plan);
+__device__ GridPlan make_plan(const unsigned long long* box, const PlanIn& in);
+__device__ void store_plan(GridPlan p, const PlanIn& in, GridPlan* __restrict__ plan);
+
+__device__ __forceinline__ void fold_box_records(const unsigned long long* __restrict__ part, int nblk,
+                                                 unsigned long long (*red)[kBoxVals] ,
+                                                 unsigned long long* fin ) {
+  const auto fold = [](int a, unsigned long long o, unsigned long long v) {
+    return (a < 3 || a == 6) ? (o < v ? o : v) : (o > v ? o : v);
+  };
+  unsigned long long v[kBoxVals] = {~0ull, ~0ull, ~0ull, 0, 0, 0, ~0ull};
+  for (int b0 = threadIdx.x; b0 < nblk; b0 += 512) {
+    unsigned long long o[2][kBoxVals];
+#pragma unroll
+    for (int u = 0; u < 2; ++u) {
+      const int b = b0 + 256 * u < nblk ? b0 + 256 * u : nblk - 1;
+#pragma unroll
+      for (int a = 0; a < kBoxVals; ++a) o[u][a] = part[size_t(b) * kBoxVals + a];
+    }
+#pragma unroll
+    for (int u = 0; u < 2; ++u)
+#pragma unroll
+      for (int a = 0; a < kBoxVals; ++a) v[a] = fold(a, o[u][a], v[a]);
+  }
+#pragma unroll
+  for (int a = 0; a < kBoxVals; ++a)
+#pragma unroll
+    for (int off = 32; off > 0; off >>= 1) v[a] = fold(a, __shfl_down(v[a], off, 64), v[a]);
+  if ((threadIdx.x & 63) == 0)
+#pragma unroll
+    for (int a = 0; a < kBoxVals; ++a) red[threadIdx.x >> 6][a] = v[a];
+  __syncthreads();
+  if (threadIdx.x < kBoxVals) {
+    unsigned long long r = red[0][threadIdx.x];
+    for (int q = 1; q < 4; ++q) r = fold(int(threadIdx.x), red[q][threadIdx.x], r);
+    fin[threadIdx.x] = r;
+  }
+  __syncthreads();
+}
 
 __global__ __launch_bounds__(256) void k_bbox_fold(const unsigned long long* __restrict__ part,
                                                    int nblk, unsigned long long* __restrict__ out,
-                                                   int32_t* __restrict__ zero_buf, int zero_n,
                                                    PlanIn pin, GridPlan* __restrict__ plan) {
   __shared__ unsigned long long red[4][kBoxVals];
   __shared__ unsigned long long fin[kBoxVals];
-  for (int q = threadIdx.x; q < zero_n; q += 256) zero_buf[q] = 0;
-  unsigned long long v[kBoxVals] = {~0ull, ~0ull, ~0ull, 0, 0, 0, ~0ull};
-  for (int b = threadIdx.x; b < nblk; b += 256)
-#pragma unroll
-    for (int a = 0; a < kBoxVals; ++a) {
-      const unsigned long long o = part[size_t(b) * kBoxVals + a];
-      v[a] = (a < 3 || a == 6) ? (o < v[a] ? o : v[a]) : (o > v[a] ? o : v[a]);
-    }
-#pragma unroll
-  for (int a = 0; a < kBoxVals; ++a)
-#pragma unroll
-    for (int off = 32; off > 0; off >>= 1) {
-      const unsigned long long o = __shfl_down(v[a], off, 64);
-      v[a] = (a < 3 || a == 6) ? (o < v[a] ? o : v[a]) : (o > v[a] ? o : v[a]);
-    }
-  if ((threadIdx.x & 63) == 0)
-#pragma unroll
-    for (int a = 0; a < kBoxVals; ++a) red[threadIdx.x >> 6][a] = v[a];
-  __syncthreads();
-  if (threadIdx.x < kBoxVals) {
-    const bool is_min = threadIdx.x < 3 || threadIdx.x == 6;
-    unsigned long long r = red[0][threadIdx.x];
-    for (int q = 1; q < 4; ++q) {
-      const unsigned long long o = red[q][threadIdx.x];
-      r = is_min ? (o < r ? o : r) : (o > r ? o : r);
-    }
-    out[threadIdx.x] = r;
-    fin[threadIdx.x] = r;
-  }
-  if (plan) {
-    __syncthreads();
-    if (threadIdx.x == 0) write_plan(fin, pin, plan);
-  }
+  fold_box_records(part, nblk, red, fin);
+  if (threadIdx.x < kBoxVals) out[threadIdx.x] = fin[threadIdx.x];
+  if (plan && threadIdx.x == 0) store_plan(make_plan(fin, pin), pin, plan);
 }
 
 __global__ __launch_bounds__(256) void k_cell_count(const double* __restrict__ xyz, int64_t n,
@@ -333,13 +344,13 @@
 int cloud_bbox(Ctx* c, const double* xyz, int64_t n, double mn[3], double mx[3], bool* all_f32,
                int32_t* zero_buf, int zero_n) {
   if (n <= 0) return fail(PYQSM_EINVAL, "bounding box of an empty cloud");
-  const int blocks = int(std::min<int64_t>(ceil_div(n, 256), int64_t(c->cu_count) * 4));
+  const int blocks = bbox_blocks(c, n);
   unsigned long long *d_box = nullptr, *d_part = nullptr;
   PQ_TRY(c->arena.get(kBoxVals, &d_box));
   PQ_TRY(c->arena.get(size_t(blocks) * kBoxVals, &d_part));
-  hipLaunchKernelGGL(k_bbox, dim3(blocks), dim3(256), 0, c->stream, xyz, n, d_part,
+  hipLaunchKernelGGL(k_bbox, dim3(blocks), dim3(256), 0, c->stream, xyz, n, d_part, zero_buf, zero_n,
                      static_cast<unsigned long long*>(nullptr));
-  hipLaunchKernelGGL(k_bbox_fold, dim3(1), dim3(256), 0, c->stream, d_part, blocks, d_box, zero_buf, zero_n, PlanIn{},
+  hipLaunchKernelGGL(k_bbox_fold, dim3(1), dim3(256), 0, c->stream, d_part, blocks, d_box, PlanIn{},
                      static_cast<GridPlan*>(nullptr));
   PQ_HIP(hipGetLastError());
   unsigned long long h_box[kBoxVals];
@@ -646,33 +657,68 @@
   using type = PointRec;
 };
 
+struct PlanFold {
+  const unsigned long long* part = nullptr;
+  int nblk = 0;
+  PlanIn in{};
+  GridPlan* out = nullptr;
+};
+
 template <int MODE>
 __global__ __launch_bounds__(256) void k_bk_hist(const double* __restrict__ xyz, int64_t n, GridParams g,
                                                  int rx, int ry, int rz, AxisMap am, int nbk, int bits,
                                                  int32_t* __restrict__ key_tmp,
-                                                 int32_t* __restrict__ tot, const GridPlan* __restrict__ plan) {
+                                                 int32_t* __restrict__ tot, const GridPlan* __restrict__ plan,
+                                                 PlanFold pf) {
   extern __shared__ __attribute__((aligned(16))) int32_t h[];
-  if (plan) {
-    if (!plan->ok) return;
-    g = GridParams{plan->mn[0], plan->mn[1], plan->mn[2], plan->inv_cell, plan->nx, plan->ny, plan->nz};
-    rx = plan->rx;
-    ry = plan->ry;
-    rz = plan->rz;
-    nbk = plan->nbk;
-    bits = plan->bits;
+  __shared__ unsigned long long red[4][kBoxVals];
+  __shared__ unsigned long long fin[kBoxVals];
+  const bool folds = MODE == 0 && pf.part != nullptr;
+  const bool stores = folds && blockIdx.x + 1 == gridDim.x;
+  const int64_t base = int64_t(blockIdx.x) * kBkPts;
+  double px[kBkPts / 256], py[kBkPts / 256], pz[kBkPts / 256];
+#pragma unroll
+  for (int k = 0; k < kBkPts / 256; ++k) {
+    const int64_t i = base + k * 256 + threadIdx.x;
+    px[k] = py[k] = pz[k] = 0.0;
+    if (MODE == 0 && i < n) {
+      px[k] = xyz[3 * i];
+      py[k] = xyz[3 * i + 1];
+      pz[k] = xyz[3 * i + 2];
+    }
+  }
+  if (folds || plan) {
+    GridPlan pl;
+    if (folds) {
+      fold_box_records(pf.part, pf.nblk, red, fin);
+      pl = make_plan(fin, pf.in);
+      if (stores) {
+        if (threadIdx.x == 0) store_plan(pl, pf.in, pf.out);
+        return;
+      }
+    } else {
+      pl = *plan;
+    }
+    if (!pl.ok) return;
+    g = GridParams{pl.mn[0], pl.mn[1], pl.mn[2], pl.inv_cell, pl.nx, pl.ny, pl.nz};
+    rx = pl.rx;
+    ry = pl.ry;
+    rz = pl.rz;
+    nbk = pl.nbk;
+    bits = pl.bits;
   }
   for (int b = threadIdx.x; b < nbk; b += 256) h[b] = 0;
   __syncthreads();
-  const int64_t base = int64_t(blockIdx.x) * kBkPts;
 #pragma unroll
   for (int k = 0; k < kBkPts / 256; ++k) {
     const int64_t i = base + k * 256 + threadIdx.x;
     if (i < n) {
       int c, oct = 0;
+      if (MODE != 0) px[k] = xyz[3 * i], py[k] = xyz[3 * i + 1], pz[k] = xyz[3 * i + 2];
       if (MODE == 2) {
-        c = cell_index(g, xyz[3 * i], xyz[3 * i + 1], xyz[3 * i + 2]);
+        c = cell_index(g, px[k], py[k], pz[k]);
       } else {
-        const RawCell r = raw_cell(g, rx, ry, rz, xyz[3 * i], xyz[3 * i + 1], xyz[3 * i + 2]);
+        const RawCell r = raw_cell(g, rx, ry, rz, px[k], py[k], pz[k]);
         const int cx = MODE == 1 ? am.x[r.cx] : r.cx + 1, cy = MODE == 1 ? am.y[r.cy] : r.cy + 1,
                   cz = MODE == 1 ? am.z[r.cz] : r.cz + 1;
         c = (cz * g.ny + cy) * g.nx + cx;
@@ -1245,13 +1291,15 @@
 
 static void enqueue_bk_a(Ctx* c, int mode, bool f32, const double* xyz, int64_t n, const GridParams& gp,
                          const int raw[3], AxisMap am, int64_t nbk, int bits, int32_t* key_tmp, int32_t* tot,
-                         int32_t* cursor, int32_t* bstart, void* bucketed, int32_t* keyb, const GridPlan* d_plan) {
+                         int32_t* cursor, int32_t* bstart, void* bucketed, int32_t* keyb, const GridPlan* d_plan,
+                         const PlanFold& pf = PlanFold{}) {
   const dim3 ga(ceil_div(n, kBkPts)), blk(256);
+  const dim3 gh(ga.x + (pf.part ? 1 : 0));
   const size_t lds = size_t(nbk) * 4;
   const int fused = nbk <= kBkFusedScan;
 #define PQ_BK_HIST(MODE)                                                                                         \
-  hipLaunchKernelGGL(k_bk_hist<MODE>, ga, blk, lds, c->stream, xyz, n, gp, raw[0], raw[1], raw[2], am, int(nbk), \
-                     bits, key_tmp, tot, d_plan)
+  hipLaunchKernelGGL(k_bk_hist<MODE>, gh, blk, lds, c->stream, xyz, n, gp, raw[0], raw[1], raw[2], am, int(nbk), \
+                     bits, key_tmp, tot, d_plan, pf)
   if (mode == 0)
     PQ_BK_HIST(0);
   else if (mode == 1)
@@ -1308,7 +1356,7 @@
 }
 
 
-__device__ void write_plan(const unsigned long long* box, const PlanIn& in, GridPlan* __restrict__ plan) {
+__device__ GridPlan make_plan(const unsigned long long* box, const PlanIn& in) {
   GridPlan p;
   bool ok = in.hint.valid != 0;
   for (int a = 0; a < 3; ++a) {
@@ -1339,6 +1387,10 @@
   p.bits = 12;
   p.ok = ok ? 1 : 0;
   p.seq = in.seq;
+  return p;
+}
+
+__device__ void store_plan(GridPlan p, const PlanIn& in, GridPlan* __restrict__ plan) {
   *plan = p;
   if (in.host) {
     p.seq = 0;
@@ -1349,15 +1401,20 @@
 }
 
 int plan_grid_device(Ctx* c, const double* xyz, int64_t n, double cell, int64_t max_cells, const PlanHint& hint,
-                     GridPlan* d_plan, GridPlan* h_plan, unsigned seq, int32_t* zero_buf, int zero_n) {
+                     GridPlan* d_plan, GridPlan* h_plan, unsigned seq, int32_t* zero_buf, int zero_n,
+                     PlanRecords* speculated) {
   if (n <= 0) return fail(PYQSM_EINVAL, "bounding box of an empty cloud");
-  const int blocks = int(std::min<int64_t>(ceil_div(n, 256), int64_t(c->cu_count) * 4));
+  const int blocks = bbox_blocks(c, n);
   unsigned long long *d_box = nullptr, *d_part = nullptr;
   PQ_TRY(c->arena.get(kBoxVals, &d_box));
   PQ_TRY(c->arena.get(size_t(blocks) * kBoxVals, &d_part));
-  hipLaunchKernelGGL(k_bbox, dim3(blocks), dim3(256), 0, c->stream, xyz, n, d_part, stamp_slots(c, blocks));
-  hipLaunchKernelGGL(k_bbox_fold, dim3(1), dim3(256), 0, c->stream, d_part, blocks, d_box, zero_buf, zero_n,
-                     PlanIn{cell, max_cells, hint, h_plan, seq}, d_plan);
+  hipLaunchKernelGGL(k_bbox, dim3(blocks), dim3(256), 0, c->stream, xyz, n, d_part, zero_buf, zero_n,
+                     stamp_slots(c, blocks));
+  if (speculated)
+    *speculated = PlanRecords{d_part, blocks, max_cells, h_plan, seq};
+  else
+    hipLaunchKernelGGL(k_bbox_fold, dim3(1), dim3(256), 0, c->stream, d_part, blocks, d_box,
+                       PlanIn{cell, max_cells, hint, h_plan, seq}, d_plan);
   PQ_HIP(hipGetLastError());
   return 0;
 }
@@ -1366,7 +1423,8 @@
 
 static int enqueue_bucketed(Ctx* c, const double* xyz, int64_t n, const GridParams& gp, const int raw[3],
                             AxisMap am, bool mapped, int64_t nbk, int bits, bool f32,
-                            int32_t* zeroed, const GridPlan* d_plan, DevGrid* g, SubCells* sub) {
+                            int32_t* zeroed, const GridPlan* d_plan, DevGrid* g, SubCells* sub,
+                            const PlanFold& pf = PlanFold{}) {
   int32_t *cell_tmp, *keyb, *rank_tmp, *bstart;
   uint32_t* word_tmp;
   int32_t *tot = zeroed, *cursor = zeroed + kBkMax;
@@ -1401,7 +1459,7 @@
   PQ_TRY(c->arena.get(size_t(n) * 8, &sub->rec));
   PQ_TRY(c->arena.get(size_t(nbk) + 1, &bstart));
   enqueue_bk_a(c, mapped ? 1 : 0, f32, xyz, n, gp, raw, am, nbk, bits, cell_tmp, tot, cursor, bstart, bucketed, keyb,
-               d_plan);
+               d_plan, pf);
   on_sort_shape(bits, f32, [&](auto S) {
     using K = decltype(S);
     unsigned long long* const st_sort = stamp_slots(c, nbk);
@@ -1451,7 +1509,7 @@
 }
 
 int bin_octants_planned(Ctx* c, const double* xyz, int64_t n, double cell, const PlanHint& hint,
-                        const GridPlan* d_plan, int32_t* zeroed, DevGrid* g, SubCells* sub) {
+                        const PlanRecords& rec, GridPlan* d_plan, int32_t* zeroed, DevGrid* g, SubCells* sub) {
   g->minx = g->miny = g->minz = 0.0;
   g->cell = cell;
   g->inv_cell = 1.0 / cell;
@@ -1460,7 +1518,8 @@
   sub->zeroed4 = zeroed + 2 * kBkMax + 1;
   const int raw[3] = {0, 0, 0};
   return enqueue_bucketed(c, xyz, n, GridParams{}, raw, AxisMap{nullptr, nullptr, nullptr}, false, hint.nbk, 12,
-                          true, zeroed, d_plan, g, sub);
+                          true, zeroed, d_plan, g, sub,
+                          PlanFold{rec.part, rec.blocks, PlanIn{cell, rec.max_cells, hint, rec.h_plan, rec.seq}, d_plan});
 }
 
 static int upload_plan(Ctx* c, const GridPlan& p, GridPlan* h_up, GridPlan* d_plan) {
diff --git a/pyqsm_amd/csrc/grid.hpp b/pyqsm_amd/csrc/grid.hpp
--- a/pyqsm_amd/csrc/grid.hpp
+++ b/pyqsm_amd/csrc/grid.hpp
@@ -276,11 +276,19 @@
 };
 __device__ __forceinline__ Stencil plan_stencil(const GridPlan* p) { return Stencil{p->nx, p->nx * p->ny}; }
 
+struct PlanRecords {
+  const unsigned long long* part;
+  int blocks;
+  int64_t max_cells;
+  GridPlan* h_plan;
+  unsigned seq;
+};
 int plan_grid_device(Ctx* c, const double* xyz, int64_t n, double cell, int64_t max_cells, const PlanHint& hint,
-                     GridPlan* d_plan, GridPlan* h_plan, unsigned seq, int32_t* zero_buf, int zero_n);
+                     GridPlan* d_plan, GridPlan* h_plan, unsigned seq, int32_t* zero_buf, int zero_n,
+                     PlanRecords* speculated = nullptr);
 int octant_zeroed_ints();
 int bin_octants_planned(Ctx* c, const double* xyz, int64_t n, double cell, const PlanHint& hint,
-                        const GridPlan* d_plan, int32_t* zeroed, DevGrid* g, SubCells* sub);
+                        const PlanRecords& rec, GridPlan* d_plan, int32_t* zeroed, DevGrid* g, SubCells* sub);
 int bin_octants_host(Ctx* c, const double* xyz, int64_t n, double min_cell, int64_t max_cells, const GridPlan& box,
                      int32_t* zeroed, GridPlan* h_up, GridPlan* d_plan, DevGrid* g, SubCells* sub,
                      PlanHint* hint_out);
diff --git a/pyqsm_amd/hip.py b/pyqsm_amd/hip.py
--- a/pyqsm_amd/hip.py
+++ b/pyqsm_amd/hip.py
@@ -209,6 +209,30 @@
     check(_lib.load().pyqsm_octant_directory(_p(pts), pts.shape[0], float(eps), _p(dims), _p(begin), int(cap),
                                              int(device)))
     return dims, begin[: int(np.prod(dims.astype(np.int64))) + 1].copy()
+
+
+class CoreRamp(NamedTuple):
+    lo: np.float32
+    hi: np.float32
+    K: np.float32
+    A: np.float32
+    B: np.float32
+    usable: bool
+
+
+def core_ramp_constants(eps: float, radius_inclusive: bool = True) -> CoreRamp:
+    out = np.zeros(6, dtype=np.float32)
+    check(_lib.load().pyqsm_core_ramp_constants(float(eps), int(bool(radius_inclusive)), _p(out)))
+    return CoreRamp(out[0], out[1], out[2], out[3], out[4], bool(out[5] != 0))
+
+
+def core_ramp_probe(d, eps: float, radius_inclusive: bool = True, device: int = 0):
+    d = np.ascontiguousarray(np.asarray(d), dtype=np.float32).reshape(-1)
+    s_in = np.empty_like(d)
+    s_hi = np.empty_like(d)
+    check(_lib.load().pyqsm_core_ramp_probe(_p(d), d.shape[0], float(eps), int(bool(radius_inclusive)),
+                                            _p(s_in), _p(s_hi), int(device)))
+    return s_in, s_hi
 
 
 def knn(points, k: int, exclude_self: bool = True, device: int = 0):
```

Result: faster. 3912 Mpoints/s (median of 6 runs) (+3.9%).
